# CenterForMedicalGeneticsGhent/WisecondorX

Measured on AMD Instinct MI355X. Metric: newref+predict throughput @15kb bins (bins x refs per second), higher is better.
Workload: dtype f64

## Files before the change

wisecondorx_amd/csrc/api.hip:

```cpp
#include "wcx_common.h"

#include <cstring>
#include <thread>

static thread_local char g_err[1024] = "";

void wcx_set_error(const char *fmt, ...) {
  va_list ap;
  va_start(ap, fmt);
  vsnprintf(g_err, sizeof(g_err), fmt, ap);
  va_end(ap);
}

int wcx_scratch(wcx_ctx *ctx, size_t bytes, void **out) {
  if (bytes > ctx->scratch_bytes) {
    if (ctx->scratch) {
      WCX_HIP(hipStreamSynchronize(ctx->stream));
      WCX_HIP(hipFree(ctx->scratch));
      ctx->scratch = nullptr;
      ctx->scratch_bytes = 0;
    }
    hipError_t e = hipMalloc(&ctx->scratch, bytes);
    if (e != hipSuccess) {
      wcx_set_error("hipMalloc(%zu bytes scratch) failed: %s", bytes, hipGetErrorString(e));
      return WCX_ERR_NOMEM;
    }
    ctx->scratch_bytes = bytes;
  }
  *out = ctx->scratch;
  return WCX_OK;
}

int wcx_host_scratch(wcx_ctx *ctx, size_t bytes, void **out) {
  if (bytes > ctx->host_scratch_bytes) {
    if (ctx->host_scratch) {
      WCX_HIP(hipStreamSynchronize(ctx->stream));
      WCX_HIP(hipHostFree(ctx->host_scratch));
      ctx->host_scratch = nullptr;
      ctx->host_scratch_bytes = 0;
    }
    const size_t grown = bytes + bytes / 4;
    hipError_t e = hipHostMalloc(&ctx->host_scratch, grown, hipHostMallocDefault);
    if (e != hipSuccess) {
      wcx_set_error("hipHostMalloc(%zu bytes) failed: %s", grown, hipGetErrorString(e));
      return WCX_ERR_NOMEM;
    }
    ctx->host_scratch_bytes = grown;
  }
  *out = ctx->host_scratch;
  return WCX_OK;
}

int wcx_scratch2(wcx_ctx *ctx, size_t bytes, void **out) {
  if (bytes > ctx->scratch2_bytes) {
    if (ctx->scratch2) {
      WCX_HIP(hipStreamSynchronize(ctx->stream));
      WCX_HIP(hipFree(ctx->scratch2));
      ctx->scratch2 = nullptr;
      ctx->scratch2_bytes = 0;
    }
    hipError_t e = hipMalloc(&ctx->scratch2, bytes);
    if (e != hipSuccess) {
      wcx_set_error("hipMalloc(%zu bytes scratch2) failed: %s", bytes, hipGetErrorString(e));
      return WCX_ERR_NOMEM;
    }
    ctx->scratch2_bytes = bytes;
  }
  *out = ctx->scratch2;
  return WCX_OK;
}

int wcx_upload_small(wcx_ctx *ctx, void *dst_dev, const void *src_host, size_t bytes) {
  if (ctx->stage.size() > 64) {
    WCX_HIP(hipStreamSynchronize(ctx->stream));
    ctx->stage.clear();
  }
  ctx->stage.emplace_back((const unsigned char *)src_host, (const unsigned char *)src_host + bytes);
  WCX_HIP(hipMemcpyAsync(dst_dev, ctx->stage.back().data(), bytes, hipMemcpyHostToDevice,
                         ctx->stream));
  return WCX_OK;
}

int wcx_timer_begin(wcx_ctx *ctx, const char *name) {
  KernelTimer &t = ctx->timers[ctx->timer_tag + name];
  if (!t.start) {
    WCX_HIP(hipEventCreate(&t.start));
    WCX_HIP(hipEventCreate(&t.stop));
  }
  WCX_HIP(hipEventRecord(t.start, ctx->stream));
  return WCX_OK;
}

int wcx_timer_end(wcx_ctx *ctx, const char *name) {
  KernelTimer &t = ctx->timers[ctx->timer_tag + name];
  WCX_HIP(hipEventRecord(t.stop, ctx->stream));
  t.used = true;
  return WCX_OK;
}

namespace {
constexpr size_t STAGED_MIN = (size_t)32 << 20;
constexpr size_t STAGED_CHUNK = (size_t)32 << 20;
constexpr int COPY_THREADS = 8;

void host_copy_mt(char *dst, const char *src, size_t n) {
  const size_t per = ((n + COPY_THREADS - 1) / COPY_THREADS + 4095) & ~(size_t)4095;
  std::thread th[COPY_THREADS];
  int used = 0;
  for (size_t o = per; o < n; o += per)
    th[used++] = std::thread([=] { memcpy(dst + o, src + o, o + per <= n ? per : n - o); });
  memcpy(dst, src, per <= n ? per : n);
  for (int i = 0; i < used; ++i) th[i].join();
}

int staged_copy(wcx_ctx *ctx, void *dst, const void *src, size_t bytes, bool to_host) {
  void *pin = nullptr;
  int rc = wcx_host_scratch(ctx, 2 * STAGED_CHUNK, &pin);
  if (rc) return rc;
  char *half[2] = {reinterpret_cast<char *>(pin), reinterpret_cast<char *>(pin) + STAGED_CHUNK};
  char *d = reinterpret_cast<char *>(dst);
  const char *s = reinterpret_cast<const char *>(src);
  hipStream_t st = ctx->stream;
  const size_t n_chunks = (bytes + STAGED_CHUNK - 1) / STAGED_CHUNK;
  auto len = [&](size_t i) { return i + 1 < n_chunks ? STAGED_CHUNK : bytes - i * STAGED_CHUNK; };
  if (to_host) {
    WCX_HIP(hipMemcpyAsync(half[0], s, len(0), hipMemcpyDeviceToHost, st));
    WCX_HIP(hipStreamSynchronize(st));
    for (size_t i = 0; i < n_chunks; ++i) {
      if (i + 1 < n_chunks)
        WCX_HIP(hipMemcpyAsync(half[(i + 1) & 1], s + (i + 1) * STAGED_CHUNK, len(i + 1),
                               hipMemcpyDeviceToHost, st));
      host_copy_mt(d + i * STAGED_CHUNK, half[i & 1], len(i));
      WCX_HIP(hipStreamSynchronize(st));
    }
  } else {
    host_copy_mt(half[0], s, len(0));
    for (size_t i = 0; i < n_chunks; ++i) {
      WCX_HIP(hipMemcpyAsync(d + i * STAGED_CHUNK, half[i & 1], len(i), hipMemcpyHostToDevice, st));
      if (i + 1 < n_chunks) host_copy_mt(half[(i + 1) & 1], s + (i + 1) * STAGED_CHUNK, len(i + 1));
      WCX_HIP(hipStreamSynchronize(st));
    }
  }
  return WCX_OK;
}
}

extern "C" {

int wcx_version(void) { return 100; }

int wcx_sweep_event(wcx_ctx *ctx, void **out_event) {
  WCX_ARG(ctx && out_event, "NULL argument");
  WCX_HIP(hipSetDevice(ctx->device));
  if (!ctx->ev_after_sweep) WCX_HIP(hipEventCreateWithFlags(&ctx->ev_after_sweep, hipEventDisableTiming));
  *out_event = ctx->ev_after_sweep;
  return WCX_OK;
}

int wcx_wait_event(wcx_ctx *ctx, void *event) {
  WCX_ARG(ctx && event, "NULL argument");
  WCX_HIP(hipSetDevice(ctx->device));
  WCX_HIP(hipStreamWaitEvent(ctx->stream, reinterpret_cast<hipEvent_t>(event), 0));
  return WCX_OK;
}

int wcx_debug_flags(wcx_ctx *ctx, int flags) {
  if (!ctx) return 0;
  const int old = ctx->debug_flags;
  ctx->debug_flags = flags;
  return old;
}

const char *wcx_last_error(void) { return g_err; }

int wcx_timer_tag(wcx_ctx *ctx, const char *tag) {
  WCX_ARG(ctx, "ctx is NULL");
  ctx->timer_tag = tag ? tag : "";
  return WCX_OK;
}

int wcx_ctx_create(int device, void *stream, wcx_ctx **out) {
  WCX_ARG(out != nullptr, "out is NULL");
  int n = 0;
  hipError_t e = hipGetDeviceCount(&n);
  if (e != hipSuccess || n <= 0) {
    wcx_set_error("no HIP device available (%s); libwcx_hip.so has no CPU fallback",
                  e != hipSuccess ? hipGetErrorString(e) : "device count 0");
    return WCX_ERR_HIP;
  }
  WCX_ARG(device >= 0 && device < n, "device index out of range");
  WCX_HIP(hipSetDevice(device));
  wcx_ctx *ctx = new wcx_ctx();
  ctx->device = device;
  if (stream == WCX_STREAM_DEFAULT) {
    ctx->stream = nullptr;
    ctx->own_stream = false;
  } else if (stream) {
    ctx->stream = reinterpret_cast<hipStream_t>(stream);
    ctx->own_stream = false;
  } else {
    WCX_HIP(hipStreamCreateWithFlags(&ctx->stream, hipStreamNonBlocking));
    ctx->own_stream = true;
  }
  WCX_HIP(hipMalloc(reinterpret_cast<void **>(&ctx->d_stats), 256));
  WCX_HIP(hipMemsetAsync(ctx->d_stats, 0, 256, ctx->stream));
  WCX_HIP(hipMalloc(&ctx->d_small, 8192));
  *out = ctx;
  return WCX_OK;
}

int wcx_ctx_destroy(wcx_ctx *ctx) {
  if (!ctx) return WCX_OK;
  hipSetDevice(ctx->device);
  hipStreamSynchronize(ctx->stream);
  for (auto &kv : ctx->timers) {
    if (kv.second.start) hipEventDestroy(kv.second.start);
    if (kv.second.stop) hipEventDestroy(kv.second.stop);
  }
  wcx_sym_state_free(ctx);
  if (ctx->scratch) hipFree(ctx->scratch);
  if (ctx->host_scratch) hipHostFree(ctx->host_scratch);
  for (auto &sl : ctx->sel_pool)
    if (sl.p) hipFree(sl.p);
  if (ctx->host_scratch2) hipHostFree(ctx->host_scratch2);
  if (ctx->scratch2) hipFree(ctx->scratch2);
  if (ctx->d_stats) hipFree(ctx->d_stats);
  if (ctx->d_small) hipFree(ctx->d_small);
  if (ctx->d_nullm) hipFree(ctx->d_nullm);
  if (ctx->d_nullsrc) hipFree(ctx->d_nullsrc);
  if (ctx->d_pca) hipFree(ctx->d_pca);
  if (ctx->sweep_stream) {
    hipStreamSynchronize(ctx->sweep_stream);
    hipStreamDestroy(ctx->sweep_stream);
    hipEventDestroy(ctx->ev_sweep0);
    hipEventDestroy(ctx->ev_sweep1);
  }
  if (ctx->ev_after_sweep) hipEventDestroy(ctx->ev_after_sweep);
  if (ctx->copy_stream) {
    hipStreamSynchronize(ctx->copy_stream);
    hipStreamDestroy(ctx->copy_stream);
    hipEventDestroy(ctx->ev_cbs_fill);
    hipEventDestroy(ctx->ev_cbs_xw);
  }
  if (ctx->aux_stream) {
    hipStreamSynchronize(ctx->aux_stream);
    hipStreamDestroy(ctx->aux_stream);
    hipEventDestroy(ctx->ev_main);
    hipEventDestroy(ctx->ev_rank);
  }
  if (ctx->d_rank) hipFree(ctx->d_rank);
  if (ctx->own_stream) hipStreamDestroy(ctx->stream);
  delete ctx;
  return WCX_OK;
}

int wcx_sync(wcx_ctx *ctx) {
  WCX_ARG(ctx, "ctx is NULL");
  WCX_HIP(hipStreamSynchronize(ctx->stream));
  return WCX_OK;
}

int wcx_malloc(wcx_ctx *ctx, size_t bytes, void **dptr) {
  WCX_ARG(ctx && dptr, "NULL argument");
  WCX_HIP(hipSetDevice(ctx->device));
  hipError_t e = hipMalloc(dptr, bytes ? bytes : 1);
  if (e != hipSuccess) {
    wcx_set_error("hipMalloc(%zu) failed: %s", bytes, hipGetErrorString(e));
    return WCX_ERR_NOMEM;
  }
  return WCX_OK;
}

int wcx_free(wcx_ctx *ctx, void *dptr) {
  WCX_ARG(ctx, "ctx is NULL");
  if (dptr) {
    WCX_HIP(hipStreamSynchronize(ctx->stream));
    WCX_HIP(hipFree(dptr));
  }
  return WCX_OK;
}

int wcx_memcpy_h2d(wcx_ctx *ctx, void *dst, const void *src, size_t bytes) {
  WCX_ARG(ctx && dst && src, "NULL argument");
  WCX_HIP(hipSetDevice(ctx->device));
  if (bytes >= STAGED_MIN) return staged_copy(ctx, dst, src, bytes, false);
  WCX_HIP(hipMemcpyAsync(dst, src, bytes, hipMemcpyHostToDevice, ctx->stream));
  WCX_HIP(hipStreamSynchronize(ctx->stream));
  return WCX_OK;
}

int wcx_memcpy_d2h(wcx_ctx *ctx, void *dst, const void *src, size_t bytes) {
  WCX_ARG(ctx && dst && src, "NULL argument");
  WCX_HIP(hipSetDevice(ctx->device));
  if (bytes >= STAGED_MIN) return staged_copy(ctx, dst, src, bytes, true);
  WCX_HIP(hipMemcpyAsync(dst, src, bytes, hipMemcpyDeviceToHost, ctx->stream));
  WCX_HIP(hipStreamSynchronize(ctx->stream));
  return WCX_OK;
}

double wcx_last_kernel_ms(wcx_ctx *ctx, const char *name) {
  if (!ctx || !name) return -1.0;
  auto it = ctx->timers.find(name);
  if (it == ctx->timers.end() || !it->second.used) return -1.0;
  if (hipEventSynchronize(it->second.stop) != hipSuccess) return -1.0;
  float ms = 0.f;
  if (hipEventElapsedTime(&ms, it->second.start, it->second.stop) != hipSuccess) return -1.0;
  return (double)ms;
}

int wcx_transpose_dev(wcx_ctx *ctx, const double *d_src, int64_t rows, int64_t cols,
                      double *d_dst) {
  WCX_ARG(ctx && d_src && d_dst, "NULL argument");
  WCX_ARG(rows > 0 && cols > 0 && rows < (1ll << 31) && (rows + 31) / 32 < 65536, "bad sizes");
  WCX_HIP(hipSetDevice(ctx->device));
  return wcx_transpose_launch(ctx, d_src, rows, cols, d_dst);
}

int wcx_last_topk_stats(wcx_ctx *ctx, int64_t out[24]) {
  WCX_ARG(ctx && out, "NULL argument");
  unsigned long long h[24] = {0};
  WCX_HIP(hipMemcpyAsync(h, ctx->d_stats, 24 * 8, hipMemcpyDeviceToHost, ctx->stream));
  WCX_HIP(hipStreamSynchronize(ctx->stream));
  out[0] = ctx->topk_stats[0];
  out[1] = ctx->topk_stats[1];
  out[2] = (int64_t)h[2];
  out[3] = (int64_t)h[3];
  for (int i = 4; i < 24; ++i) out[i] = (int64_t)h[i];
  return WCX_OK;
}

int wcx_newref_sym_sweep_dev(wcx_ctx *ctx, const double *dXs, int64_t B, int S, const int64_t *chr_cum,
                             int n_chr, int k, int part, int n_parts, const int64_t *row_bounds,
                             int64_t *counts_out) {
  WCX_ARG(ctx && dXs && chr_cum && row_bounds && counts_out, "NULL argument");
  WCX_ARG(B > 0 && S > 0 && n_chr > 0 && k > 0, "B, S, n_chr, k must be positive");
  WCX_ARG(chr_cum[n_chr - 1] == B, "chr_cum[n_chr-1] must equal B");
  WCX_ARG(n_parts >= 1 && part >= 0 && part < n_parts, "bad part");
  WCX_ARG(B < (int64_t)0x7fffffff, "B must fit in int32 (indices are int32)");
  if (n_chr > 22) {
    wcx_set_error("the sharded symmetric sweep searches every row: not a gonosomal pass (n_chr = %d)", n_chr);
    return WCX_ERR_UNSUPPORTED;
  }
  WCX_HIP(hipSetDevice(ctx->device));
  if (ctx->rank_X && !ctx->rank_pending) ctx->rank_X = nullptr;
  const int64_t r0 = row_bounds[part], r1 = row_bounds[part + 1];
  WCX_ARG(0 <= r0 && r0 <= r1 && r1 <= B, "bad row bounds");
  int64_t pairs = 0;
  for (int c = 0; c < n_chr; ++c) {
    const int64_t cs = c ? chr_cum[c - 1] : 0, ce = chr_cum[c];
    const int64_t lo = cs > r0 ? cs : r0, hi = ce < r1 ? ce : r1;
    if (lo < hi) pairs += (hi - lo) * (B - (ce - cs));
  }
  ctx->topk_stats[0] = r1 - r0;
  ctx->topk_stats[1] = pairs;
  wcx_aux_cancel_if_few_rows(ctx, B, r1 - r0);
  return wcx_sym_shard_sweep(ctx, dXs, B, S, chr_cum, n_chr, k, part, n_parts, row_bounds, counts_out);
}

int wcx_newref_sym_records_dev(wcx_ctx *ctx, void *d_send) {
// ... 103 lines not shown
```

wisecondorx_amd/csrc/cbs_seg.hip:

```cpp
#include <algorithm>
#include <chrono>
#include <cmath>
#include <cstdio>
#include <functional>
#include <map>
#include <mutex>
#include <thread>
#include <vector>

#include "wave_sort.h"
#include "wcx_common.h"

namespace {

constexpr int NTP = 1024;
constexpr int KMAXC = 25;
constexpr int QC_W = 32;
constexpr int PCHUNK = 256;
constexpr int NCH = 64;
constexpr int STAGE_A = 512;
typedef float f32x2 __attribute__((ext_vector_type(2)));

__host__ __device__ __forceinline__ unsigned long long mix64(unsigned long long z) {
  z += 0x9e3779b97f4a7c15ull;
// ... 1213 lines not shown
    std::vector<int> hc(nsc + 1);
    WCX_HIP(hipMemcpyAsync(hc.data(), d_cnt, (nsc + 1) * 4, hipMemcpyDeviceToHost, st));
    WCX_HIP(hipStreamSynchronize(st));
    for (size_t q = 0; q < nsc; ++q) cnt_sc[q] = hc[q];
    n_inf = hc[nsc];
  } else {
    for_samples([&](int s) {
      for (int c = 0; c < n_chr; ++c) {
        const double *rr = r + (int64_t)s * n_bins + chr_off[c];
        const int nall = (int)(chr_off[c + 1] - chr_off[c]);
        int64_t m = 0;
        for (int i = 0; i < nall; ++i) m += is_drop(rr[i]) ? 0 : 1;
        cnt_sc[(size_t)s * n_chr + c] = m;
      }
    });
  }
  int64_t total = 0;
  std::vector<int64_t> lo_sc(cnt_sc.size());
  for (size_t q = 0; q < cnt_sc.size(); ++q) { lo_sc[q] = total; total += cnt_sc[q]; }
  const int64_t totp = (total + 3) & ~(int64_t)3;
  void *hstage = nullptr;
  {
    const int rcs = wcx_host_scratch(ctx, (size_t)totp * 20 + 64, &hstage);
    if (rcs) return rcs;
  }
  double *hx = reinterpret_cast<double *>(hstage), *hw = hx + totp;
  int *hpos = reinterpret_cast<int *>(hw + totp);
  if (d_r && (ctx->debug_flags & 64)) {
    const double poison = __builtin_nan("");
    for (int64_t i = 0; i < 2 * totp; ++i) hx[i] = poison;
  }
  if (!d_r)
    for_samples([&](int s) {
      for (int c = 0; c < n_chr; ++c) {
        const int64_t o = (int64_t)s * n_bins + chr_off[c];
        const int nall = (int)(chr_off[c + 1] - chr_off[c]);
        int64_t at = lo_sc[(size_t)s * n_chr + c];
        for (int i = 0; i < nall; ++i) {
          const double v = r[o + i];
          if (is_drop(v)) continue;
          hx[at] = v;
          hw[at] = w[o + i] == 0.0 ? 1.0 : w[o + i];
          hpos[at] = i + 1;
          ++at;
        }
      }
    });
  for (int s = 0; s < n_samples; ++s)
    for (int c = 0; c < n_chr; ++c) {
      const size_t q = (size_t)s * n_chr + c;
      if (cnt_sc[q] == 0) continue;
      Series se;
      se.sample = s; se.chr = c; se.lo = lo_sc[q]; se.n = (int)cnt_sc[q];
      se.seg_end = {0, se.n};
      series.push_back(std::move(se));
    }
  const int64_t N = total;
  const double *dXs_all = nullptr, *dWs_all = nullptr;
  lap("series");
  int rc = wcx_timer_begin(ctx, "cbs");
  if (rc) return rc;
  if (N > 0) {
    int max_n = 0;
    for (const Series &se : series) max_n = std::max(max_n, se.n);
    const int max_segs = (int)series.size() + 8;
    const int max_jobs = max_segs * 2;
    const int npad_max = (max_n + NTP - 1) / NTP * NTP;
    const bool any_big = max_n > LDS_KEYS_MAX;
    const size_t max_items = (size_t)max_segs + (size_t)(N / 4) + 6144 + 64;
    const size_t max_blocks = (size_t)(N / PBS) + 2 * (size_t)max_segs + 64;
    const unsigned int work_cap = 1u << 22;
    const size_t qtab_floats = (size_t)(KMAXC - 1) * ((size_t)N + (size_t)NTP * max_segs) +
                               (size_t)max_segs * (KMAXC + 1) * QC_W;
    const size_t need = (size_t)N * (8 * 5 + 4 * 3) + 4096 + (series.size() + 8) * sizeof(RangeItem) + (size_t)max_segs * (sizeof(SegIn) + sizeof(SegOut) + 8) +
                        (size_t)max_segs * P.ngrid * 16 + max_items * (sizeof(ArcItem) + sizeof(ArcBest)) +
                        (size_t)max_jobs * (2 * sizeof(PermJob) + (size_t)(nw + NCH) * 4) +
                        (any_big ? (size_t)BIG_GRID * (npad_max + 64) * 4 : 0) +
                        (size_t)EXACT_GRID * npad_max * 8 + FLAG_CAP * sizeof(uint2) + qtab_floats * 4 +
                        max_blocks * (sizeof(BlkStat) + 4) + (size_t)work_cap * (sizeof(WorkItem) + sizeof(ArcBest)) +
                        (size_t)max_segs * 32 + (1 << 16);
    void *scr = nullptr;
    rc = wcx_scratch(ctx, need, &scr);
    if (rc) return rc;
    Arena A;
    A.base = reinterpret_cast<char *>(scr);
    double *dX = A.take<double>(N), *dW = A.take<double>(N), *dS = A.take<double>(N), *dWp = A.take<double>(N);
    double *dYd = A.take<double>(N);
    dXs_all = dX; dWs_all = dW;
    int *dpos = A.take<int>((size_t)N + 4);
    RangeItem *drng = A.take<RangeItem>(series.size() + 8);
    float *dy = A.take<float>(N), *drw = A.take<float>(N);
    SegIn *dseg = A.take<SegIn>(max_segs);
    SegOut *dso = A.take<SegOut>(max_segs);
    int *dfirst = A.take<int>(max_segs + 1);
    double *dtx = A.take<double>((size_t)max_segs * P.ngrid), *dnu = A.take<double>((size_t)max_segs * P.ngrid);
    ArcItem *ditems = A.take<ArcItem>(max_items);
    ArcBest *dbest = A.take<ArcBest>(max_items);
    PermJob *djobs = A.take<PermJob>((size_t)max_jobs * 2);
    unsigned int *dbits = A.take<unsigned int>((size_t)max_jobs * nw);
    unsigned int *dcnt = A.take<unsigned int>((size_t)max_jobs * NCH + 64);
    unsigned int *dnflag = dcnt + (size_t)max_jobs * NCH;
    float *dbig = any_big ? A.take<float>((size_t)BIG_GRID * (npad_max + 64)) : nullptr;
    double *dexact = A.take<double>((size_t)EXACT_GRID * npad_max);
    uint2 *dflags = A.take<uint2>(FLAG_CAP);
    float *dq = A.take<float>(qtab_floats);
    BlkStat *dbs = A.take<BlkStat>(max_blocks);
    WorkItem *dwork = A.take<WorkItem>(work_cap);
    ArcBest *dres = A.take<ArcBest>(work_cap);
    int *dboff = A.take<int>(max_segs + 1);
    int *dbseg = A.take<int>(max_blocks);
    unsigned int *dL = A.take<unsigned int>(max_segs + 2);
    unsigned long long *dbbits = A.take<unsigned long long>(max_segs);
    unsigned long long *dbij = A.take<unsigned long long>(max_segs);
    static const bool no_prune = getenv("WCX_CBS_NOPRUNE") && atoi(getenv("WCX_CBS_NOPRUNE"));
    if (d_r) {
      WCX_HIP(hipMemcpyAsync(d_lo, lo_sc.data(), lo_sc.size() * 8, hipMemcpyHostToDevice, st));
      k_cbs_fill<<<dim3((unsigned)n_chr, (unsigned)n_samples), 256, 0, st>>>(d_r, d_w, n_bins, co, n_chr, d_lo,
                                                                            dX, dW, dpos);
      WCX_HIP(hipGetLastError());
      WCX_HIP(hipEventRecord(ctx->ev_cbs_fill, st));
      WCX_HIP(hipStreamWaitEvent(aux, ctx->ev_cbs_fill, 0));
      k_cbs_export<<<16, 256, 0, aux>>>(reinterpret_cast<const uint4 *>(dpos), reinterpret_cast<uint4 *>(hpos),
                                        ((int64_t)N * 4 + 15) / 16);
      WCX_HIP(hipGetLastError());
      if (n_inf > 0) {
        const size_t rw_bytes = (size_t)n_samples * n_bins * 8;
        WCX_HIP(hipMemcpyAsync(const_cast<double *>(r), d_r, rw_bytes, hipMemcpyDeviceToHost, aux));
        WCX_HIP(hipMemcpyAsync(const_cast<double *>(w), d_w, rw_bytes, hipMemcpyDeviceToHost, aux));
      }
      copies_queued = true;
    } else {
      WCX_HIP(hipMemcpyAsync(dX, hx, (size_t)N * 8, hipMemcpyHostToDevice, st));
      WCX_HIP(hipMemcpyAsync(dW, hw, (size_t)N * 8, hipMemcpyHostToDevice, st));
    }
    const size_t lds_small = (size_t)(std::min(npad_max, LDS_KEYS_MAX) + 32) * 4;
    WCX_HIP(hipFuncSetAttribute(reinterpret_cast<const void *>(k_cbs_perm_hyb<false>),
                                hipFuncAttributeMaxDynamicSharedMemorySize, (int)lds_small));

    std::vector<JobResult> jres;
    std::vector<unsigned int> hbits;
    auto run_jobs = [&](std::vector<PermJob> &jobs, const std::vector<std::vector<int>> &seq) -> int {
      jres.assign(jobs.size(), JobResult());
      if (jobs.empty()) return WCX_OK;
      WCX_ARG(jobs.size() <= (size_t)max_jobs, "internal: permutation job table overflow");
      size_t qoff = 0;
      for (size_t q = 0; q < jobs.size(); ++q) {
        jobs[q].slot = (int)q;
        jobs[q].qoff = (int64_t)qoff;
        if (jobs[q].mode == 0)
          qoff += (size_t)(KMAXC - 1) * (size_t)((jobs[q].n + NTP - 1) / NTP * NTP) + (size_t)(KMAXC + 1) * QC_W;
      }
      WCX_ARG(qoff <= qtab_floats, "internal: arc-weight table overflow");
      WCX_HIP(hipMemcpyAsync(djobs, jobs.data(), jobs.size() * sizeof(PermJob), hipMemcpyHostToDevice, st));
      WCX_HIP(hipMemsetAsync(dbits, 0, jobs.size() * (size_t)nw * 4, st));
      WCX_HIP(hipMemsetAsync(dcnt, 0, jobs.size() * (size_t)NCH * 4, st));
      {
        int hyb_max_n = 0;
        for (const PermJob &jb : jobs) if (jb.mode == 0) hyb_max_n = std::max(hyb_max_n, jb.n);
        if (hyb_max_n > 0) {
          const int npad_sel = (hyb_max_n + NTP - 1) / NTP * NTP;
          k_cbs_arcweights<<<dim3((unsigned)(npad_sel / 256), (unsigned)jobs.size()), 256, 0, st>>>(
              dWp, djobs, P.minw, dq);
          WCX_HIP(hipGetLastError());
        }
      }
      hbits.resize(jobs.size() * (size_t)nw);
      std::vector<int> pending(jobs.size());
      for (size_t q = 0; q < jobs.size(); ++q) pending[q] = (int)q;
      const int stages[3] = {0, std::min(STAGE_A, P.nperm), P.nperm};
      for (int sg = 0; sg < 2 && !pending.empty(); ++sg) {
        const int p0 = stages[sg], p1 = stages[sg + 1];
        if (p1 <= p0) continue;
        std::vector<PermJob> sel[4];
        for (int q : pending) {
          const PermJob &jb = jobs[(size_t)q];
          const int kind = jb.mode == 0 ? (jb.n > LDS_KEYS_MAX ? 1 : 0) : jb.mode == 1 ? 2 : 3;
          sel[kind].push_back(jb);
        }
        size_t joff = 0;
        PermJob *dsel = djobs + jobs.size();
        WCX_ARG(pending.size() + jobs.size() <= (size_t)max_jobs * 2, "internal: job table overflow");
        for (int kind = 0; kind < 4; ++kind) {
          std::vector<PermJob> &sj = sel[kind];
          if (sj.empty()) continue;
          const size_t per_launch = kind <= 1 ? std::max<size_t>(1, FLAG_CAP / (size_t)(p1 - p0)) : sj.size();
          for (size_t j0 = 0; j0 < sj.size(); j0 += per_launch) {
            const size_t nj = std::min(per_launch, sj.size() - j0);
            PermJob *dj = dsel + joff;
            WCX_HIP(hipMemcpyAsync(dj, sj.data() + j0, nj * sizeof(PermJob), hipMemcpyHostToDevice, st));
            joff += nj;
            if (kind <= 1) {
              WCX_HIP(hipMemsetAsync(dnflag, 0, 4, st));
              if (kind == 1)
                k_cbs_perm_hyb<true><<<dim3((unsigned)std::min(BIG_GRID, p1 - p0), (unsigned)nj), NTP, 0, st>>>(
                    dy, drw, dj, p0, p1, npad_max + 64, dq, dbig, dbits, dcnt, nw, dflags, dnflag);
              else
                k_cbs_perm_hyb<false><<<dim3((unsigned)(p1 - p0), (unsigned)nj), NTP, lds_small, st>>>(
                    dy, drw, dj, p0, p1, 0, dq, nullptr, dbits, dcnt, nw, dflags, dnflag);
              WCX_HIP(hipGetLastError());
              k_cbs_perm_exact<<<EXACT_GRID, 256, 0, st>>>(dYd, dW, dWp, dj, dflags, dnflag, dexact, npad_max,
                                                           P.minw, dbits, dcnt, nw);
            } else if (kind == 2) {
              k_cbs_perm_full<<<dim3((unsigned)(p1 - p0), (unsigned)nj), 256, 0, st>>>(dYd, dW, dWp, dj, p0, p1,
                                                                                      P.minw, dbits, dcnt, nw);
            } else {
              k_cbs_perm_edge<<<dim3((unsigned)((p1 - p0 + 3) / 4), (unsigned)nj), 256, 0, st>>>(
                  dYd, dW, dj, p0, p1, dbits, dcnt, nw);
            }
            WCX_HIP(hipGetLastError());
          }
        }
        WCX_HIP(hipMemcpyAsync(hbits.data(), dbits, jobs.size() * (size_t)nw * 4, hipMemcpyDeviceToHost, st));
        WCX_HIP(hipStreamSynchronize(st));
        std::vector<int> still;
        for (int q : pending) {
          const PermJob &jb = jobs[(size_t)q];
          const unsigned int *b = hbits.data() + (size_t)q * nw;
          JobResult &res = jres[(size_t)q];
          if (jb.mode == 2) {
            int nrej = 0;
            for (int t = 0; t < nw; ++t) nrej += __builtin_popcount(b[t]);
            res.nrej = nrej; res.np = p1;
            if (nrej > jb.budget) { res.decided = 1; res.significant = 0; }
            else if (p1 >= P.nperm) { res.decided = 1; res.significant = 1; }
          } else {
            eval_sequential(b, p1, P.nperm, jb.budget, seq[(size_t)q], res);
          }
          if (!res.decided) still.push_back(q);
        }
        pending.swap(still);
      }
      return WCX_OK;
    };

    std::vector<char> resident(series.size(), d_r ? 0 : 1);
    auto ensure_resident = [&](const std::vector<int> &want) -> int {
      std::vector<RangeItem> items;
      for (int q : want)
        if (!resident[(size_t)q]) {
          resident[(size_t)q] = 1;
          items.push_back({series[(size_t)q].lo, series[(size_t)q].n, 0});
        }
      if (items.empty()) return WCX_OK;
      WCX_HIP(hipMemcpyAsync(drng, items.data(), items.size() * sizeof(RangeItem), hipMemcpyHostToDevice, st));
      k_cbs_export_ranges<<<(unsigned)items.size(), 256, 0, st>>>(dX, dW, drng, hx, hw);
      WCX_HIP(hipGetLastError());
      WCX_HIP(hipStreamSynchronize(st));
      return WCX_OK;
    };

    struct Active { int series, lo, hi; };
    for (;;) {
      std::vector<Active> act;
      for (size_t q = 0; q < series.size(); ++q) {
        Series &se = series[q];
        while (se.seg_end.size() > 1) {
          const int k = (int)se.seg_end.size();
          const int lo = se.seg_end[k - 2], hi = se.seg_end[k - 1];
          if (hi - lo >= 2 * P.minw) { act.push_back({(int)q, lo, hi}); break; }
          se.change_loc.push_back(hi);
          se.seg_end.pop_back();
        }
      }
      if (act.empty()) break;
      const int ns = (int)act.size();
      std::vector<SegIn> hseg(ns);
      double arc_total = 0;
      for (int a = 0; a < ns; ++a) { const double n = act[a].hi - act[a].lo; arc_total += 0.5 * n * n; }
      const double arc_budget = std::max(arc_total / 6144.0, 16384.0);
      std::vector<ArcItem> items;
      std::vector<int> first(ns + 1);
      for (int a = 0; a < ns; ++a) {
        const Series &se = series[act[a].series];
        hseg[a].lo = se.lo + act[a].lo;
        hseg[a].n = act[a].hi - act[a].lo;
        hseg[a].hybrid = hseg[a].n > P.nmin ? 1 : 0;
        first[a] = (int)items.size();
        const int n = hseg[a].n;
        for (int i0 = 0; i0 < n;) {
          const int rows = (int)std::min<double>(ARC_ROWS, std::max<double>(4.0, arc_budget / (double)(n - i0)));
          items.push_back({a, i0, std::min(i0 + rows, n), 0});
          i0 += rows;
        }
      }
      first[ns] = (int)items.size();
      WCX_ARG(items.size() <= max_items, "internal: arc stripe table overflow");
      WCX_HIP(hipMemcpyAsync(dseg, hseg.data(), (size_t)ns * sizeof(SegIn), hipMemcpyHostToDevice, st));
      WCX_HIP(hipMemcpyAsync(ditems, items.data(), items.size() * sizeof(ArcItem), hipMemcpyHostToDevice, st));
      WCX_HIP(hipMemcpyAsync(dfirst, first.data(), (size_t)(ns + 1) * 4, hipMemcpyHostToDevice, st));
      k_cbs_prepare<<<ns, NTP, 0, st>>>(dX, dW, dseg, dS, dWp, dYd, dy, drw, dso);
      std::vector<int> boff(ns + 1);
      boff[0] = 0;
      for (int a = 0; a < ns; ++a) boff[a + 1] = boff[a] + (hseg[a].n + 1 + PBS - 1) / PBS;
      const int total_blocks = boff[ns];
      bool pruned = !no_prune && (size_t)total_blocks <= max_blocks && arc_total > 4e9;
      unsigned int *dcount = dL + ns;
      if (pruned) {
        WCX_HIP(hipMemcpyAsync(dboff, boff.data(), (size_t)(ns + 1) * 4, hipMemcpyHostToDevice, st));
        WCX_HIP(hipMemsetAsync(dL, 0, (size_t)(ns + 1) * 4, st));
        WCX_HIP(hipMemsetAsync(dbbits, 0, (size_t)ns * 8, st));
        WCX_HIP(hipMemsetAsync(dbij, 0xff, (size_t)ns * 8, st));
        std::vector<int> bseg((size_t)total_blocks);
        for (int a = 0; a < ns; ++a) std::fill(bseg.begin() + boff[a], bseg.begin() + boff[a + 1], a);
        WCX_HIP(hipMemcpyAsync(dbseg, bseg.data(), (size_t)total_blocks * 4, hipMemcpyHostToDevice, st));
        const unsigned rows4 = (unsigned)((total_blocks + 3) / 4);
        k_cbs_blockstats<<<rows4, 256, 0, st>>>(dS, dWp, dseg, dso, dboff, dbseg, total_blocks, dbs);
        k_cbs_coarse<<<rows4, 256, 0, st>>>(dS, dWp, dseg, dso, dboff, dbseg, total_blocks, dbs, P.minw, dL);
        k_cbs_prune<<<(unsigned)((total_blocks + 4 * PRW - 1) / (4 * PRW)), 256, 0, st>>>(
            dso, dboff, dbseg, total_blocks, dbs, dL, dwork, work_cap, dcount);
        k_cbs_pairmax<<<8192, 256, 0, st>>>(dS, dWp, dseg, dso, dwork, work_cap, dcount, P.minw, dres, dbbits, dL);
        k_cbs_pairtie<<<2048, 256, 0, st>>>(dwork, work_cap, dcount, dres, dbbits, dbij);
        k_cbs_pairfinal<<<(unsigned)((ns + 256) / 256), 256, 0, st>>>(ns, dbbits, dbij, dbest, dfirst);
        WCX_HIP(hipGetLastError());
        unsigned int hcount = 0;
        WCX_HIP(hipMemcpyAsync(&hcount, dcount, 4, hipMemcpyDeviceToHost, st));
        WCX_HIP(hipStreamSynchronize(st));
        ctx->cbs_pairs_listed += hcount;
        ctx->cbs_pairs_total += [&] { long long t = 0; for (int a = 0; a < ns; ++a) { const long long nb = boff[a + 1] - boff[a]; t += nb * (nb + 1) / 2; } return t; }();
        if (hcount > work_cap) pruned = false;
      }
      if (!pruned) {
        WCX_HIP(hipMemcpyAsync(dfirst, first.data(), (size_t)(ns + 1) * 4, hipMemcpyHostToDevice, st));
        k_cbs_arcmax<<<(unsigned)items.size(), 256, 0, st>>>(dS, dWp, dseg, dso, ditems, P.minw, dbest);
      }
      const double alpha_skip = (ctx->debug_flags & 2) ? HUGE_VAL : 4.0 * P.alpha;
      k_cbs_arcfinish<<<ns, 128, 0, st>>>(dbest, dfirst, dseg, dWp, dso, P.kmax, P.ngrid, alpha_skip, dtx);
      k_nu_series<<<dim3(P.ngrid, ns), 256, 0, st>>>(dtx, dseg, dso, P.ngrid, alpha_skip, dnu);
      k_cbs_tailp<<<ns, 64, 0, st>>>(dnu, dseg, dso, P.ngrid, alpha_skip);
      WCX_HIP(hipGetLastError());
      std::vector<SegOut> hso(ns);
      WCX_HIP(hipMemcpyAsync(hso.data(), dso, (size_t)ns * sizeof(SegOut), hipMemcpyDeviceToHost, st));
      WCX_HIP(hipStreamSynchronize(st));
      lap("  stats");
      if (d_r) {
        std::vector<int> want;
        for (int a = 0; a < ns; ++a) {
          const SegOut &o = hso[a];
          if (!hseg[a].hybrid || !o.valid || o.range <= 1.4901161193847656e-08) continue;
          const double ostat1 = sqrt(o.ostat);
          const int arc = std::min(o.bj - o.bi, hseg[a].n - o.bj + o.bi);
          if (ostat1 <= 0.1 || (!strict && ostat1 >= 7.0 && arc >= 10)) continue;
          if (o.pval1 < 0.0 || o.pval1 > P.alpha) continue;
          want.push_back(act[a].series);
        }
        rc = ensure_resident(want);
        if (rc) return rc;
      }
      lap("  host copy");

      std::vector<PermJob> jobs;
      std::vector<std::vector<int>> seq;
      std::vector<int> job_of(ns, -1);
      std::vector<int> verdict(ns, 0);
      std::vector<int> why(ns, 0);
      int n_shortcut = 0;
      for (int a = 0; a < ns; ++a) {
        const SegOut &o = hso[a];
        const int n = hseg[a].n;
        if (!o.valid || o.range <= 1.4901161193847656e-08) { why[a] = 1; continue; }
        const double ostat1 = sqrt(o.ostat);
        if (ostat1 <= 0.1) { why[a] = 2; continue; }
        const int arc = std::min(o.bj - o.bi, n - o.bj + o.bi);
        if (!strict && ostat1 >= 7.0 && arc >= 10) { why[a] = 3; verdict[a] = 1; continue; }
        double pval2 = P.alpha;
        if (hseg[a].hybrid) {
          if (o.pval1 < 0.0 || o.pval1 > P.alpha) { why[a] = 4; continue; }
          pval2 = P.alpha - o.pval1;
        }
        PermJob jb;
        memset(&jb, 0, sizeof(jb));
        jb.lo = hseg[a].lo; jb.n = n; jb.mode = hseg[a].hybrid ? 0 : 1;
        jb.budget = (int)(pval2 * (double)P.nperm);
        jb.thr = 0.99999 * o.ostat;
        jb.tss = o.tss;
        jb.W = o.W;
        if (jb.mode == 0 && !(ctx->debug_flags & 32) &&
            short_arc_bound(hx + jb.lo, hw + jb.lo, jb.n, P.minw, P.kmax, o.tss) * 1.0001 < jb.thr) {
          why[a] = 6; verdict[a] = 1; ++n_shortcut;
          continue;
        }
        if (jb.mode == 0) {
          const double u = 5.9604644775390625e-08;
          const double vmax = sqrt(o.wmax) * o.ymax;
          const double wlo = P.minw * o.wmin;
          const double qmax = o.W / (wlo * (o.W - wlo));
          jb.cthr = jb.thr / ((n - 2.0) + jb.thr);
          jb.D = u * vmax * (2700.0 + 75.0 * n * o.wmax / o.W) * sqrt(qmax) * 1.001;
          jb.eT = 6.0 * u * n * vmax / o.W * 1.001;
          const double bthr = jb.cthr * o.tss;
          if (!(wlo > 0) || !(o.W > 2 * wlo) || !(bthr > 1e-30) || !(bthr < 1e30) || !std::isfinite(jb.D))
            jb.D = HUGE_VAL;
        }
        const Series &se = series[act[a].series];
        jb.key = test_key(P.seed, se.chr, act[a].lo, act[a].hi, 0);
        why[a] = 5;
        job_of[a] = (int)jobs.size();
        seq.push_back(cbs_boundary(P.alpha, P.nperm, jb.budget));
        jobs.push_back(jb);
      }
      rc = run_jobs(jobs, seq);
      if (rc) return rc;
      lap("  perms");
      std::vector<JobResult> seg_res(ns);
      for (int a = 0; a < ns; ++a)
        if (job_of[a] >= 0) { seg_res[a] = jres[(size_t)job_of[a]]; verdict[a] = seg_res[a].significant; }
      ctx->cbs_shortcuts += n_shortcut;

      std::vector<PermJob> ejobs;
      struct EdgeRef { int a, which, shortcut; };
      std::vector<EdgeRef> eref;
      if (d_r) {
        std::vector<int> want;
        for (int a = 0; a < ns; ++a)
          if (verdict[a] && hso[a].bi != 0 && hso[a].bj != hseg[a].n) want.push_back(act[a].series);
        rc = ensure_resident(want);
        if (rc) return rc;
      }
      for (int a = 0; a < ns; ++a) {
        if (!verdict[a]) continue;
        const int n = hseg[a].n, bi = hso[a].bi, bj = hso[a].bj;
        if (bi == 0 || bj == n) continue;
        const double mean = hso[a].mean;
        const double *x = hx + hseg[a].lo, *ww = hw + hseg[a].lo;
        for (int which = 0; which < 2; ++which) {
          const int l = which == 0 ? 0 : bi, n12 = which == 0 ? bj : n - bi;
          const int n1 = which == 0 ? bi : bj - bi, n2 = n12 - n1;
          EdgeRef er{a, which, -1};
          if (n1 == 1 || n2 == 1) { er.shortcut = 0; eref.push_back(er); continue; }
          double w1 = 0, w2 = 0, s1 = 0, s2 = 0, ssq = 0;
          for (int i = 0; i < n1; ++i) { const double c = x[l + i] - mean; w1 += ww[l + i]; s1 += ww[l + i] * c; ssq += ww[l + i] * c * c; }
          for (int i = n1; i < n12; ++i) { const double c = x[l + i] - mean; w2 += ww[l + i]; s2 += ww[l + i] * c; ssq += ww[l + i] * c * c; }
          const double rn = w1 + w2;
          const double xbar = (s1 + s2) / rn;
          const double tss = ssq - rn * xbar * xbar;
          const bool first_short = n1 <= n2;
          const int m1 = first_short ? n1 : n2;
          const double wm = first_short ? w1 : w2, wo = first_short ? w2 : w1;
          const double dm = fabs((first_short ? s1 / w1 : s2 / w2) - xbar);
          double tstat = dm * dm * wm * rn / wo;
          tstat = tstat / ((tss - tstat) / (n12 - 2.0));
          if (!strict && tstat > 25.0 && m1 >= 10) { er.shortcut = 1; eref.push_back(er); continue; }
          PermJob jb;
          memset(&jb, 0, sizeof(jb));
          jb.lo = hseg[a].lo + l; jb.n = n12; jb.mode = 2; jb.m1 = m1;
          int budget = (int)floor(P.alpha * P.nperm);
          while ((double)(budget + 1) / (double)P.nperm <= P.alpha) ++budget;
          while (budget >= 0 && (double)budget / (double)P.nperm > P.alpha) --budget;
          jb.budget = budget;
          jb.thr = 0.99999 * dm;
          jb.tss = xbar;
          jb.W = wm;
          const Series &se = series[act[a].series];
          jb.key = test_key(P.seed, se.chr, act[a].lo, act[a].hi, 1 + which);
          er.shortcut = -1 - (int)ejobs.size();
// ... 226 lines not shown
```

wisecondorx_amd/csrc/newref_topk_screen.hip:

```cpp
#include <cmath>
#include <cstdlib>

#include "screen_kernel.h"
#include "screen_common.h"
#include "screen_hub1.h"

namespace {

constexpr int CSPLIT = 16;

__device__ __forceinline__ unsigned long long dord(double x) {
  const unsigned long long u = (unsigned long long)__double_as_longlong(x);
  return (u >> 63) ? ~u : (u | 0x8000000000000000ull);
}
__device__ __forceinline__ double dord_inv(unsigned long long k) {
  return __longlong_as_double((long long)((k >> 63) ? (k & 0x7fffffffffffffffull) : ~k));
}

__global__ __launch_bounds__(NT) void k_col_sum(const double *__restrict__ Xs, int64_t B,
                                                double *__restrict__ psum,
                                                double *__restrict__ pcnt,
                                                unsigned long long *__restrict__ cmin,
                                                unsigned long long *__restrict__ cmax) {
  __shared__ double ws[NT / 64], wc[NT / 64];
// ... 925 lines not shown
  const int forced = kn.cut_r(0);
  if (forced > 0 && forced < k) r = forced;
  return r;
}

static std::vector<ScreenBlock> merge_blocks(const std::vector<TopkBlock> &exact_blocks, const int64_t *chr_cum,
                                             int n_chr, int max_rows) {
  std::vector<ScreenBlock> out;
  size_t i = 0;
  while (i < exact_blocks.size()) {
    ScreenBlock sb;
    sb.row0 = exact_blocks[i].row0;
    sb.nrows = exact_blocks[i].nrows;
    sb.chr = 0;
    for (int c = 0; c < n_chr; ++c)
      if (chr_cum[c] == exact_blocks[i].ce && (c ? chr_cum[c - 1] : 0) == exact_blocks[i].cs) sb.chr = c;
    sb.cs = exact_blocks[i].cs;
    sb.ce = exact_blocks[i].ce;
    size_t j = i + 1;
    while (j < exact_blocks.size() && exact_blocks[j].cs == sb.cs &&
           exact_blocks[j].row0 == sb.row0 + sb.nrows && sb.nrows + exact_blocks[j].nrows <= max_rows) {
      sb.nrows += exact_blocks[j].nrows;
      ++j;
    }
    out.push_back(sb);
    i = j;
  }
  return out;
}

enum class ScreenPath { sym, exact, one_dir };
struct ScreenPlan {
  ScreenCfg cfg;
  int hw_cus = 256, slots = 0;
  int hub_need = 0;
  int64_t hub_rows = 0;
  bool hub_ok = false;
  ScreenPath path = ScreenPath::one_dir;
  std::vector<ScreenBlock> blocks;
  std::vector<ScreenBlock> hub_blocks;
  bool use_hub1 = false;
  int SF = 0, n_seg = 1, cut_r = 0;
};
static ScreenPlan plan_shape(wcx_ctx *ctx, int64_t B, int k, const ScreenCfg &cfg, const Knobs &kn) {
  ScreenPlan p;
  p.cfg = cfg;
  hipDeviceProp_t prop;
  if (hipGetDeviceProperties(&prop, ctx->device) == hipSuccess && prop.multiProcessorCount > 0)
    p.hw_cus = prop.multiProcessorCount;
  p.slots = p.hw_cus * (cfg.lb * 4 / cfg.wpb > 0 ? cfg.lb * 4 / cfg.wpb : 1);
  const int need = (int)(1.18 * k) + 8;
  p.hub_need = kn.hub_test_fail(0) ? (1 << 28) : need;
  const int frac = kn.hub_frac(cfg.nk >= 16 ? 32 : 12);
  p.hub_rows = frac > 1 ? B / frac : 0;
  if (p.hub_rows < 8 * (int64_t)need + 512) p.hub_rows = 8 * (int64_t)need + 512;
  p.hub_ok = cfg.nk >= 5 && frac > 1 && p.hub_rows * 6 <= B;
  return p;
}

static ScreenPlan plan_search(wcx_ctx *ctx, int64_t B, int S, int k, bool all_rows, const Knobs &kn,
                              const std::vector<TopkBlock> &exact_blocks, const int64_t *chr_cum, int n_chr) {
  const int NK = screen_nk(S);
  ScreenCfg cfg = default_cfg(NK);
  cfg.prof = (ctx->debug_flags & DBG_PROF) && (NK == 7 || NK == 32) ? 1 : 0;
  int tl[5];
  if (kn.tile.set && sscanf(kn.tile.str, "%d,%d,%d,%d,%d", &tl[0], &tl[1], &tl[2], &tl[3], &tl[4]) == 5) {
    cfg.ctg = tl[0]; cfg.tt = tl[1]; cfg.wpb = tl[2]; cfg.lb = tl[3]; cfg.ring = tl[4];
  }
  ScreenPlan p = plan_shape(ctx, B, k, cfg, kn);
  const int TGT_WG = 32 * cfg.tt * cfg.wpb;
  p.blocks = merge_blocks(exact_blocks, chr_cum, n_chr, TGT_WG);
  int SF = kn.sample((B >= 32768) ? 16 : ((B >= 8192 && NK < 16) ? 8 : 0));
  if (SF < 2 || SF > 64) SF = 0;
  const int64_t n_s = SF ? (B + SF - 1) / SF : 0;
  const int64_t P_s = (n_s + CT - 1) / CT * CT;
  const bool hub1 = kn.screen_hub(kn.sample.set || kn.cut_r.set ? 0 : 1) != 0 && p.hub_ok && cfg.wpb == 4 &&
                    cfg.ring >= 2;
  int n_seg = 1;
  if ((int)p.blocks.size() * (hub1 ? 2 : 4) <= p.slots) {
    int fill = p.slots / (int)p.blocks.size();
    if (fill > 8) fill = 8;
    n_seg = kn.segments_small(fill);
  }
  n_seg = kn.segments(n_seg);
  if (n_seg < 1) n_seg = 1;
  if (n_seg > 8) n_seg = 8;
  p.n_seg = n_seg;
  int64_t covered = 0;
  for (const ScreenBlock &sb : p.blocks) covered += sb.nrows;
  const int cut_r1 = sample_rank(k, SF, P_s, 1, kn);
  const int sym_mode = kn.sym(1);
  if (cut_r1 && all_rows && covered == B && cfg.tt == 1 && cfg.wpb == 4 && cfg.ring >= 2 &&
      (sym_mode == 2 || (sym_mode == 1 && NK >= 16))) {
    p.path = ScreenPath::sym;
    p.SF = SF;
    p.cut_r = cut_r1;
    return p;
  }
  if (k > KMAX_ONE_DIR) {
    p.path = ScreenPath::exact;
    return p;
  }
  p.use_hub1 = hub1;
  if (hub1) {
    if (TGT_WG != 128) p.hub_blocks = merge_blocks(exact_blocks, chr_cum, n_chr, 128);
  } else {
    p.SF = SF;
    p.cut_r = sample_rank(k, SF, P_s, n_seg, kn);
  }
  return p;
}

template <class Unit, size_t N, class... Args>
static int launch_unit(Unit (&units)[N], const Args &...args) {
  int rc = -1;
  for (Unit u : units)
    if ((rc = u(args...)) >= 0) break;
  return rc;
}
static const decltype(&wcx_screen_launch_k1) screen_units[] = {
    wcx_screen_launch_k1, wcx_screen_launch_k2, wcx_screen_launch_k3, wcx_screen_launch_k4,
    wcx_screen_launch_k5, wcx_screen_launch_k6, wcx_screen_launch_k7, wcx_screen_launch_k8};
static const decltype(&wcx_sym_launch_k1) sym_units[] = {wcx_sym_launch_k1, wcx_sym_launch_k2, wcx_sym_launch_k3,
                                                         wcx_sym_launch_k4, wcx_sym_launch_k5};
static const decltype(&wcx_count_launch_k1) count_units[] = {wcx_count_launch_k1, wcx_count_launch_k2,
                                                             wcx_count_launch_k3, wcx_count_launch_k4};
static const decltype(&wcx_hub1_launch_k1) hub1_units[] = {wcx_hub1_launch_k1, wcx_hub1_launch_k2,
                                                           wcx_hub1_launch_k3, wcx_hub1_launch_k4};

static int unit_status(int e, const char *family, const ScreenCfg &c, int trials = 0) {
  if (e == 0) return WCX_OK;
  char what[128];
  const int n = snprintf(what, sizeof what, "nk=%d ctg=%d tt=%d wpb=%d lb=%d ring=%d", c.nk, c.ctg, c.tt, c.wpb,
                         c.lb, c.ring);
  if (trials) snprintf(what + n, sizeof what - n, " trials=%d", trials);
  if (e < 0) {
    wcx_set_error("%s kernel %s is not instantiated", family, what);
    return (int)WCX_ERR_UNSUPPORTED;
  }
  wcx_set_error("%s kernel %s: launch failed: %s", family, what, hipGetErrorString((hipError_t)e));
  return (int)WCX_ERR_HIP;
}

struct Carve {
  uintptr_t at;
  template <class T> void operator()(T *&p, size_t bytes) {
    p = reinterpret_cast<T *>(at);
    at += (bytes + 255) / 256 * 256;
  }
};

static float screen_gamma(int NK) { return (float)(16 * NK + 12) * 1.1920929e-7f; }

static int col_stats(const double *dXs, int64_t B, int S, double *cmean, ScreenGlobals *glob,
                     const int64_t *chr_cum, int n_chr, ChrTab &tab, hipStream_t st) {
  unsigned long long *cmin = reinterpret_cast<unsigned long long *>(cmean + S);
  unsigned long long *cmax = cmin + S;
  double *psum = cmean + 3 * S, *pcnt = psum + (size_t)S * CSPLIT;
  WCX_HIP(hipMemsetAsync(cmin, 0xff, (size_t)S * 8, st));
  WCX_HIP(hipMemsetAsync(cmax, 0, (size_t)S * 8, st));
  k_col_sum<<<dim3((unsigned)S, CSPLIT), NT, 0, st>>>(dXs, B, psum, pcnt, cmin, cmax);
  k_col_stats<<<(unsigned)((S + 63) / 64), 64, 0, st>>>(S, psum, pcnt, cmin, cmax, cmean, glob);
  tab.n_chr = n_chr;
  for (int c = 0; c < 32; ++c) tab.cum[c] = c < n_chr ? chr_cum[c] : B;
  return WCX_OK;
}

static void screen_prep(int NK, const double *Xr, int64_t n_pos, int S, int Sp, const double *cmean,
                        const int *perm, ScreenGlobals *glob, half8 *F, RowInfo *info, const unsigned int *gate,
                        hipStream_t st) {
  const unsigned g = (unsigned)((n_pos + 31) / 32);
  switch (NK) {
#define WCX_PREP_CASE(N) case N: k_screen_prep<N><<<g, NT, 0, st>>>(Xr, n_pos, S, Sp, cmean, perm, glob, F, info, gate); break;
    WCX_PREP_CASE(1) WCX_PREP_CASE(2) WCX_PREP_CASE(3) WCX_PREP_CASE(4) WCX_PREP_CASE(5)
    WCX_PREP_CASE(6) WCX_PREP_CASE(7) WCX_PREP_CASE(8) WCX_PREP_CASE(10) WCX_PREP_CASE(12)
    WCX_PREP_CASE(14) WCX_PREP_CASE(16) WCX_PREP_CASE(20) WCX_PREP_CASE(24) WCX_PREP_CASE(28)
    WCX_PREP_CASE(40) WCX_PREP_CASE(48) WCX_PREP_CASE(56) WCX_PREP_CASE(64)
    default: k_screen_prep<32><<<g, NT, 0, st>>>(Xr, n_pos, S, Sp, cmean, perm, glob, F, info, gate); break;
#undef WCX_PREP_CASE
  }
}

struct ScreenChunk { int64_t groups; size_t lds; };
static ScreenChunk screen_chunk(const ScreenCfg &cfg, int kb) {
  int64_t g = ((int64_t)kb << 10) / ((int64_t)cfg.ctg * 32 * cfg.nk * 32);
  if (g < 16) g = 16;
  if (g > 4096) g = 4096;
  return {g, (size_t)(cfg.ring >= 2 ? cfg.ring : 2) * (size_t)(cfg.ctg * cfg.nk * 64) * 16 + (size_t)(g + 64) * 4};
}

static int sym_final(int NK, int cap2, const RowInfo *info, const ScreenGlobals *glob, const int *rowpos, int64_t n,
                     uint2 *sl, int *cnt, unsigned int *flags, const float *Dest, int k, const unsigned int *gate,
                     hipStream_t st) {
  const float gamma = screen_gamma(NK);
  const unsigned gf = (unsigned)((n + 3) / 4 < 65536 ? (n + 3) / 4 : 65536);
  if (cap2 == CAP2)
    k_sym_final<CAP2 / 64><<<gf, NT, 0, st>>>(info, glob, rowpos, n, sl, cnt, flags, Dest, k, gamma, CAP, gate);
  else
    k_sym_final<CAP2_BIG / 64><<<gf, NT, 0, st>>>(info, glob, rowpos, n, sl, cnt, flags, Dest, k, gamma,
                                                  REFINE_MAX, gate);
  WCX_HIP(hipGetLastError());
  return WCX_OK;
}

static bool kick_after_sweep(int S) { return S >= 256; }
static int end_prep(wcx_ctx *ctx, int S) {
  WCX_HIP(hipGetLastError());
  int rc = wcx_timer_end(ctx, "topk_prep");
  if (rc) return rc;
  if (!kick_after_sweep(S) && (rc = wcx_aux_kick(ctx))) return rc;
  return wcx_timer_begin(ctx, "topk_screen");
}

struct TopkTail {
  const double *dXs = nullptr;
  int64_t B = 0;
  int S = 0, Sp = 0, k = 0;
  int cap2 = CAP;
  ChrTab tab;
  double *Xr = nullptr;
  ScreenGlobals *glob = nullptr;
  int *perm = nullptr, *cnt = nullptr;
  unsigned int *flags = nullptr, *d_nredo = nullptr;
  unsigned char *searched = nullptr;
  uint2 *sl = nullptr;
  TopkBlock *d_redo = nullptr, *d_rtile = nullptr;
  int32_t *d_rlist = nullptr;
  void *rscr = nullptr;
};
static int finish_topk(wcx_ctx *ctx, const TopkTail &t, int64_t r0, int64_t n, bool kick, int32_t *d_out_idx,
                       double *d_out_dist) {
  hipStream_t st = ctx->stream;
  if (ctx->ev_after_sweep) WCX_HIP(hipEventRecord(ctx->ev_after_sweep, st));
  int rc = kick ? wcx_aux_kick(ctx) : (int)WCX_OK;
  if (rc) return rc;
  rc = wcx_timer_begin(ctx, "topk_refine");
  if (rc) return rc;
  rc = wcx_refine_launch(ctx, t.Xr, t.S, t.Sp, t.tab, r0, n, t.searched, t.sl, t.cnt, t.flags, t.perm, t.k,
                         d_out_idx, d_out_dist, t.glob, t.cap2);
  if (rc) return rc;
  rc = wcx_timer_end(ctx, "topk_refine");
  if (rc) return rc;
  const unsigned g = (unsigned)((n + NT - 1) / NT);
  k_collect_redo<<<g, NT, 0, st>>>(r0, n, t.searched, t.flags, t.tab, t.d_redo, t.d_nredo, ctx->d_stats);
  k_redo_plan<<<1, 64, 0, st>>>(t.tab, t.d_nredo, t.d_rtile);
  k_redo_fill<<<g, NT, 0, st>>>(r0, n, t.searched, t.flags, t.tab, t.d_nredo, t.d_rlist);
  WCX_HIP(hipGetLastError());
  rc = wcx_topk_exact_redo_launch(ctx, t.dXs, t.B, t.S, t.d_redo, t.d_nredo, t.d_rtile, t.d_nredo + 1, t.d_rlist,
                                  t.rscr, r0, t.k, d_out_idx, d_out_dist);
  if (rc) return rc;
  return wcx_timer_end(ctx, "topk");
}

struct SymShardState {
  bool valid = false;
  int64_t row_begin = 0, row_end = 0;
  int NK = 0, n_parts = 0, part = 0;
  RowBounds rb;
  TopkTail tail;
  RowInfo *info = nullptr;
  int *rowpos = nullptr;
  float *Dest = nullptr;
  unsigned int *pool_head = nullptr;
  uint4 *pool = nullptr;
  unsigned int pool_cap = 0;
  unsigned long long *d_counts = nullptr;
  unsigned long long counts[32] = {0};
  bool overflow = false;
};
struct SymShardCall { int part, n_parts; RowBounds rb; SymShardState *state; };

static int screen_sym_path(wcx_ctx *ctx, const Knobs &kn, const ScreenPlan &p, const double *dXs, int64_t B, int S,
                           const int64_t *chr_cum, int n_chr, int k, int32_t *d_out_idx, double *d_out_dist,
                           SymShardCall *sh = nullptr) {
  const ScreenCfg &cfg = p.cfg;
  const std::vector<ScreenBlock> &blocks = p.blocks;
  const int NK = cfg.nk, CTG = cfg.ctg, SF = p.SF;
  const int Sp = row_pitch(S);
  const int64_t n_rows = B;
  const int64_t n_own = sh ? sh->rb.b[sh->part + 1] - sh->rb.b[sh->part] : B;
  const int cap2 = k <= 448 ? CAP2 : CAP2_BIG;
  const bool use_hub = kn.sym_hub(1) != 0 && p.hub_ok;
  if (sh && !use_hub) {
    wcx_set_error("the row-sharded symmetric sweep needs the hub-count thresholds (K >= 256, B >= %lld)",
                  (long long)(36 * (int64_t)p.hub_need));
    return (int)WCX_ERR_UNSUPPORTED;
  }
  const int64_t n_s = (B + SF - 1) / SF;
  const int64_t P_s = (n_s + CT - 1) / CT * CT;
  const int64_t Bpad2 = P_s + ((B - n_s) + CT - 1) / CT * CT;
  const int64_t NTb = (((B + 31) / 32 + (int64_t)2 * SYM_NCLS * n_chr + 4) + 7) / 8 * 8;
  const int64_t PB = NTb * 32;
  const int64_t pool_want = sh ? n_rows * (int64_t)(cap2 / 2) / sh->n_parts * 2 : n_rows * (int64_t)(cap2 / 2);
  const unsigned int pool_cap = (unsigned int)(pool_want < 200000000ll ? pool_want : 200000000ll);
  const int n_wg_det = (int)((B + NT - 1) / NT);
  TopkTail t;
  ScreenGlobals *glob;
  double *cmean;
  half8 *F, *Fs;
  RowInfo *info, *infs;
  int *perm2, *rowpos, *rowpos2, *hubhist, *rchr, *rkey, *cellcnt, *cursor, *d_seq, *dett;
  unsigned int *rbits, *rfine, *gmask, *tinfo, *pool_head;
  float *tmin, *Dest, *g_state;
  unsigned char *tchr;
  unsigned short *detl;
  uint4 *pool;
  SymDesc *d_desc;
  unsigned long long *d_counts;
  ScreenBlock *d_blocks;
  auto layout = [&](uintptr_t base) {
    Carve take{base};
    take(glob, sizeof(ScreenGlobals));
    take(cmean, (size_t)S * 8 * (3 + 2 * CSPLIT));
    take(t.Xr, (size_t)B * Sp * 8 + 256);
    take(F, (size_t)PB * NK * 32);
    take(Fs, (size_t)P_s * NK * 32);
    take(info, (size_t)PB * sizeof(RowInfo));
    take(infs, (size_t)P_s * sizeof(RowInfo));
    take(t.perm, (size_t)PB * 4);
    take(perm2, (size_t)Bpad2 * 4);
    take(rowpos, (size_t)B * 4);
    take(rowpos2, (size_t)B * 4);
    take(rbits, (size_t)B * 4);
    take(rfine, (size_t)B * 4);
    take(hubhist, (size_t)HUB_BINS * 4);
    take(rchr, (size_t)B * 4);
    take(rkey, (size_t)B * 4);
    take(cellcnt, (size_t)2 * NCELL * 4);
    take(cursor, (size_t)2 * NCELL * 4);
    take(gmask, (size_t)(P_s / CT) * 4);
    take(tinfo, (size_t)NTb * 64 * 4);
    take(tmin, (size_t)NTb * 4);
    take(tchr, (size_t)NTb);
    take(Dest, (size_t)n_rows * 4);
    take(pool, (size_t)pool_cap * 16);
    take(pool_head, 256);
    take(d_desc, 256 * sizeof(SymDesc));
    take(d_seq, (size_t)(NTb / 4 + 1) * 4);
    take(t.sl, (size_t)n_own * cap2 * 8);
    take(dett, sh ? (size_t)DET_KEYS * n_wg_det * 4 : 0);
    take(detl, sh ? (size_t)B * 2 : 0);
    take(d_counts, 64 * 8);
    take(t.cnt, (size_t)n_rows * 4);
    take(g_state, (size_t)n_rows * 4);
    take(t.flags, (size_t)n_rows * 4);
    take(t.searched, (size_t)n_rows);
    take(d_blocks, blocks.size() * sizeof(ScreenBlock));
    take(t.d_redo, (size_t)n_rows * sizeof(TopkBlock));
    take(t.d_nredo, 512);
    take(t.d_rtile, ((size_t)n_rows / 64 + 64) * sizeof(TopkBlock));
    take(t.d_rlist, (size_t)n_rows * 4);
    take(t.rscr, wcx_topk_redo_scratch_bytes(k, B));
    return (size_t)(take.at - base);
  };
  void *scr = nullptr;
  int rc = wcx_scratch(ctx, layout(0), &scr);
  if (rc) return rc;
  layout(reinterpret_cast<uintptr_t>(scr));
  t.dXs = dXs; t.B = B; t.S = S; t.Sp = Sp; t.k = k; t.cap2 = cap2; t.glob = glob;
  unsigned int *d_gate = pool_head + 3, *d_failed = pool_head + 4;
  const unsigned int *gate2 = use_hub ? d_gate : nullptr;

  hipStream_t st = ctx->stream;
  WCX_HIP(hipMemsetAsync(glob, 0, sizeof(ScreenGlobals), st));
  WCX_HIP(hipMemsetAsync(t.cnt, 0, (size_t)n_rows * 4, st));
  WCX_HIP(hipMemsetAsync(t.flags, 0, (size_t)n_rows * 4, st));
  WCX_HIP(hipMemsetAsync(t.searched, 1, (size_t)n_rows, st));
  WCX_HIP(hipMemsetAsync(pool_head, 0, 256, st));
  WCX_HIP(hipMemsetAsync(t.d_nredo, 0, 512, st));
  WCX_HIP(hipMemsetAsync(ctx->d_stats, 0, 256, st));
  rc = wcx_upload_small(ctx, d_blocks, blocks.data(), blocks.size() * sizeof(ScreenBlock));
  if (rc) return rc;

  rc = wcx_timer_begin(ctx, "topk");
  if (rc) return rc;
  rc = wcx_timer_begin(ctx, "topk_prep");
  if (rc) return rc;
  rc = col_stats(dXs, B, S, cmean, glob, chr_cum, n_chr, t.tab, st);
  if (rc) return rc;
  const ChrTab &tab = t.tab;
  const unsigned gb = (unsigned)((B + NT - 1) / NT);
  if (use_hub) {
    WCX_HIP(hipMemsetAsync(hubhist, 0, (size_t)HUB_BINS * 4, st));
    k_transpose_norm<<<(unsigned)((B + 31) / 32), 256, 0, st>>>(dXs, B, S, Sp, t.Xr, cmean, tab, glob, rbits, rchr,
                                                                rfine, hubhist);
    k_hub_cut<<<1, 1024, 0, st>>>(hubhist, (int)p.hub_rows, glob);
  } else {
    k_transpose_norm<<<(unsigned)((B + 31) / 32), 256, 0, st>>>(dXs, B, S, Sp, t.Xr, cmean, tab, glob, rbits, rchr,
                                                                nullptr, nullptr);
  }
  WCX_HIP(hipMemsetAsync(cellcnt, 0, (size_t)2 * NCELL * 4, st));
  WCX_HIP(hipMemsetAsync(cursor, 0, (size_t)2 * NCELL * 4, st));
  WCX_HIP(hipMemsetAsync(t.perm, 0xff, (size_t)PB * 4, st));
  WCX_HIP(hipMemsetAsync(tchr, 0xff, (size_t)NTb, st));
  static_assert(2 * SYM_NCELL * SYM_NSUB <= 2 * NCELL, "cell tables");
  k_sym_hist<<<gb, NT, 0, st>>>(rbits, rchr, B, glob, rkey, cellcnt, 1, use_hub ? rfine : nullptr);
  k_sym_scan<<<1, SYM_NCELL, 0, st>>>(cellcnt, cursor, tchr, glob);
  if (sh) {
    WCX_HIP(hipMemsetAsync(dett, 0, (size_t)DET_KEYS * n_wg_det * 4, st));
    k_det_local<<<gb, NT, 0, st>>>(rkey, B, n_wg_det, dett, detl);
    k_det_scan<<<(unsigned)((DET_KEYS * 64 + NT - 1) / NT), NT, 0, st>>>(dett, n_wg_det, cursor);
    k_det_place<<<gb, NT, 0, st>>>(rkey, B, n_wg_det, dett, detl, t.perm, rowpos);
  } else {
    k_scatter<<<gb, NT, 0, st>>>(rkey, B, cursor, t.perm, rowpos);
  }
  screen_prep(NK, t.Xr, PB, S, Sp, cmean, t.perm, glob, F, info, nullptr, st);
  rc = end_prep(ctx, S);
  if (rc) return rc;

  int64_t Cz = ((int64_t)kn.sym_chunk_kb(3072) << 10) / ((int64_t)NK * 1024);
  Cz = Cz / 8 * 8;
  if (Cz < 32) Cz = 32;
  if (Cz > 8192) Cz = 8192;
  while ((NTb + Cz - 1) / Cz > 256) Cz *= 2;
  const int glist_cap = (int)((Cz / CTG + 64 + 3) / 4 * 4);
  const size_t lds_sym = (size_t)cfg.ring * (size_t)(CTG * NK * 64) * 16 + (size_t)cfg.ring * CTG * 256 +
                         (size_t)glist_cap * 4 + (size_t)4 * 64 * 16;
  const int NQb = (int)(NTb / 4);
  SymArgs sa;
  int sym_grid = 0;
  {
    const int fill = kn.sym_fill(1) * p.slots;
    std::vector<SymDesc> descs;
    int total = 0;
    for (int64_t c0 = 0; c0 < NTb; c0 += Cz) {
      SymDesc d;
      d.c0 = (int)c0;
      d.c1 = (int)(c0 + Cz < NTb ? c0 + Cz : NTb);
      d.q_first = (int)(c0 / 4);
      d.n_q = NQb - d.q_first;
      int n_split = d.n_q >= fill ? 1 : (fill + d.n_q - 1) / d.n_q;
      const int max_split = (d.c1 - d.c0) / CTG / 8 > 1 ? (d.c1 - d.c0) / CTG / 8 : 1;
      if (n_split > max_split) n_split = max_split;
      const int split = kn.sym_split(0);
      if (split > 0) n_split = split < max_split ? split : max_split;
      if (n_split < 1) n_split = 1;
      if (!descs.empty() && n_split < descs.back().n_split) n_split = descs.back().n_split;
      d.n_split = n_split;
      d.item_base = total;
      d.index = (int)descs.size();
      d.pad = 0;
      total += d.n_q * d.n_split;
      descs.push_back(d);
    }
    rc = wcx_upload_small(ctx, d_desc, descs.data(), descs.size() * sizeof(SymDesc));
    if (rc) return rc;
    WCX_HIP(hipMemsetAsync(d_seq, 0, (size_t)(NQb + 1) * 4, st));
    sa.F = F; sa.tinfo = tinfo; sa.tmin = tmin; sa.tchr = tchr; sa.glob = glob; sa.sl = t.sl; sa.cnt = t.cnt;
    sa.flags = t.flags; sa.stats = ctx->d_stats; sa.dbg = ctx->debug_flags; sa.cap2 = cap2;
    sa.pool = pool; sa.pool_head = pool_head; sa.pool_ovf = pool_head + 1; sa.pool_cap = pool_cap;
    sa.queue_head = pool_head + 2;
    sa.desc = d_desc; sa.n_desc = (int)descs.size(); sa.total_items = total; sa.seq = d_seq;
    sa.glist_cap = glist_cap;
    sa.gate = nullptr;
    if (sh) { sa.force_records = 1; sa.part = sh->part; sa.n_parts = sh->n_parts; }
    sym_grid = total < p.slots ? total : p.slots;
  }
  auto sweep = [&]() {
    return unit_status(launch_unit(sym_units, NK, CTG, cfg.lb, cfg.ring, sa, (unsigned)sym_grid, lds_sym, st),
                       "symmetric screen", cfg);
  };
  auto sweep_and_cut = [&](const unsigned int *gate) -> int {
    sa.gate = gate;
    const int e = sweep();
    if (e) return e;
    k_sym_regroup<<<2048, NT, 0, st>>>(pool, pool_head, pool_head + 1, pool_cap, n_rows, t.sl, t.cnt, t.flags,
                                       cap2, gate);
    return sym_final(NK, cap2, info, glob, rowpos, n_rows, t.sl, t.cnt, t.flags, Dest, k, gate, st);
  };

  if (use_hub) {
    rc = wcx_timer_begin(ctx, "topk_pre");
    if (rc) return rc;
    CountArgs ca;
    ca.F = F; ca.tchr = tchr; ca.glob = glob; ca.perm = t.perm; ca.tinfo = tinfo; ca.tmin = tmin;
    ca.Dest = Dest; ca.cnt = t.cnt; ca.flags = t.flags; ca.stats = ctx->d_stats;
    ca.need = p.hub_need; ca.n1 = kn.hub_n1(16); ca.gate = nullptr;
    ca.sl = nullptr; ca.cap2 = cap2;
    const int64_t hub_t = (p.hub_rows * 2 + 31) / 32 + (int64_t)SYM_NCLS * n_chr + 8;
    const int64_t cap_t = hub_t < NTb ? hub_t : NTb;
    ca.glist_cap = (int)(cap_t / CTG + 64);
    const size_t lds_cnt = (size_t)cfg.ring * (size_t)(CTG * NK * 64) * 16 + (size_t)ca.glist_cap * 4;
    rc = unit_status(launch_unit(count_units, NK, CTG, cfg.lb, cfg.ring, ca, (unsigned)NQb, lds_cnt, st),
                     "hub-count", cfg);
    if (rc) return rc;
    rc = wcx_timer_end(ctx, "topk_pre");
    if (rc) return rc;
    if (sh) {
      rc = sweep();
      if (rc) return rc;
      WCX_HIP(hipMemsetAsync(d_counts, 0, 64 * 8, st));
      k_rec_hist<<<1024, NT, 0, st>>>(pool, pool_head, pool_cap, sh->rb, d_counts);
      WCX_HIP(hipGetLastError());
      rc = wcx_timer_end(ctx, "topk_screen");
      if (rc) return rc;
      SymShardState &Z = *sh->state;
      unsigned int head2[2] = {0, 0};
      WCX_HIP(hipMemcpyAsync(Z.counts, d_counts, 32 * 8, hipMemcpyDeviceToHost, st));
      WCX_HIP(hipMemcpyAsync(head2, pool_head, 8, hipMemcpyDeviceToHost, st));
      WCX_HIP(hipStreamSynchronize(st));
      Z.overflow = head2[1] || head2[0] > pool_cap || kn.pool_ovf(0) != 0;
      if (Z.overflow)
        for (int r = 0; r < 32; ++r) Z.counts[r] = 0;
      Z.valid = true;
      Z.row_begin = sh->rb.b[sh->part]; Z.row_end = sh->rb.b[sh->part + 1];
      Z.NK = NK; Z.n_parts = sh->n_parts; Z.part = sh->part; Z.rb = sh->rb;
      Z.tail = t; Z.info = info; Z.rowpos = rowpos; Z.Dest = Dest;
      Z.pool_head = pool_head; Z.pool = pool; Z.pool_cap = pool_cap; Z.d_counts = d_counts;
      return (int)WCX_OK;
    }
    rc = sweep_and_cut(nullptr);
    if (rc) return rc;
    if (!(ctx->debug_flags & DBG_ABLATIONS)) {
      k_hub_count_failed<<<512, NT, 0, st>>>(t.flags, n_rows, d_failed);
      k_hub_verdict<<<1, 64, 0, st>>>(d_failed, d_gate, ctx->d_stats);
    }
    k_gate_reset<<<1024, NT, 0, st>>>(d_gate, n_rows, t.cnt, t.flags, pool_head, d_seq, NQb + 1);
  } else {
    rc = wcx_timer_begin(ctx, "topk_pre");
    if (rc) return rc;
  }

  {
    WCX_HIP(hipMemsetAsync(cellcnt, 0, (size_t)2 * NCELL * 4, st));
    WCX_HIP(hipMemsetAsync(perm2, 0xff, (size_t)Bpad2 * 4, st));
    k_row_hist<<<gb, NT, 0, st>>>(rbits, rchr, B, SF, 0, glob, rkey, cellcnt, gate2);
    k_scan_cells<<<1, 1024, 0, st>>>(cellcnt, cursor, (int)(P_s - n_s), gate2);
    k_scatter<<<gb, NT, 0, st>>>(rkey, B, cursor, perm2, rowpos2, gate2);
    k_group_mask<<<(unsigned)((P_s / CT + NT - 1) / NT), NT, 0, st>>>(perm2, rchr, P_s / CT, gmask, gate2);
    screen_prep(NK, t.Xr, P_s, S, Sp, cmean, perm2, glob, Fs, infs, gate2, st);
    WCX_HIP(hipGetLastError());
    const ScreenChunk ch = screen_chunk(cfg, kn.chunk_kb(NK > 16 ? 16384 : 3072));
    ScreenArgs a;
    a.F = Fs; a.Ft = F; a.info = info; a.glob = glob; a.perm = perm2; a.rowpos = rowpos; a.gmask = gmask;
    a.blocks = d_blocks; a.sl = t.sl; a.cnt = t.cnt; a.flags = t.flags; a.g_state = g_state;
    a.stats = ctx->d_stats; a.row_begin = 0; a.n_rows_all = n_rows;
    a.k = k; a.dbg = ctx->debug_flags & ~DBG_SWEEP; a.n_seg = 1; a.n_blocks = (int)blocks.size();
    a.raw_est = 1;
    a.gate = gate2;
    int trig_a = 4 * p.cut_r + 64;
    if (trig_a > 256 && 2 * p.cut_r + 32 <= 256) trig_a = 256;
    if (trig_a > LIM) trig_a = LIM;
    const int64_t g_end = P_s / (CTG * 32);
    bool first = true;
    for (int64_t g0 = 0; g0 < g_end; g0 += ch.groups) {
      const int64_t g1 = g0 + ch.groups < g_end ? g0 + ch.groups : g_end;
      a.g_start = g0; a.g_count = (int)(g1 - g0);
      a.cut_k = p.cut_r; a.cut_mode = 1; a.trig = trig_a; a.end_cut = g1 == g_end ? 1 : 0;
      a.first = first ? 1 : 0;
      first = false;
      rc = unit_status(launch_unit(screen_units, cfg, a, (unsigned)blocks.size(), ch.lds, st), "screen", cfg);
      if (rc) return rc;
    }
    k_sym_setup<<<(unsigned)((PB + NT - 1) / NT), NT, 0, st>>>(t.perm, info, glob, g_state, t.cnt, t.flags, Dest,
                                                              tinfo, tmin, gate2);
    WCX_HIP(hipGetLastError());
    if (!use_hub) {
      rc = wcx_timer_end(ctx, "topk_pre");
      if (rc) return rc;
    }
    rc = sweep_and_cut(gate2);
    if (rc) return rc;
  }
  rc = wcx_timer_end(ctx, "topk_screen");
  if (rc) return rc;
  return finish_topk(ctx, t, 0, n_rows, kick_after_sweep(S), d_out_idx, d_out_dist);
}

static int screen_one_dir_path(wcx_ctx *ctx, const Knobs &kn, const ScreenPlan &p, const double *dXs, int64_t B,
                               int S, const int64_t *chr_cum, int n_chr, int64_t row_begin, int64_t n_rows, int k,
                               int32_t *d_out_idx, double *d_out_dist) {
  const ScreenCfg &cfg = p.cfg;
  const std::vector<ScreenBlock> &blocks = p.blocks, &hub_blocks = p.hub_blocks;
  const int NK = cfg.nk, GRr = cfg.ctg * 32, SF = p.SF, n_seg = p.n_seg, cut_r = p.cut_r;
  const bool use_hub1 = p.use_hub1;
  const int64_t n_s = SF ? (B + SF - 1) / SF : 0;
  const int64_t P_s = (n_s + CT - 1) / CT * CT;
  const int64_t Bpad = P_s + ((B - n_s) + CT - 1) / CT * CT + (use_hub1 ? CT : 0);
  const int64_t n_iter_groups = Bpad / GRr;
  const int64_t n_groups = Bpad / CT;
  const int Sp = row_pitch(S);
  TopkTail t;
  ScreenGlobals *glob;
  double *cmean;
  half8 *F;
  RowInfo *info;
  int *rowpos, *hubhist, *rchr, *rkey, *cellcnt, *cursor;
  unsigned int *rbits, *rfine, *gmask;
  float *g_state;
  ScreenBlock *d_blocks, *d_hblocks;
  auto layout = [&](uintptr_t base) {
    Carve take{base};
    take(glob, sizeof(ScreenGlobals));
    take(cmean, (size_t)S * 8 * (3 + 2 * CSPLIT));
    take(t.Xr, (size_t)B * Sp * 8 + 256);
    take(F, (size_t)Bpad * NK * 32);
    take(info, (size_t)Bpad * sizeof(RowInfo));
    take(t.perm, (size_t)Bpad * 4);
    take(rowpos, (size_t)B * 4);
    take(rbits, (size_t)B * 4);
    take(rfine, use_hub1 ? (size_t)B * 4 : 0);
    take(hubhist, use_hub1 ? (size_t)HUB_BINS * 4 : 0);
    take(rchr, (size_t)B * 4);
    take(rkey, (size_t)B * 4);
    take(cellcnt, (size_t)2 * NCELL * 4);
    take(cursor, (size_t)2 * NCELL * 4);
    take(gmask, (size_t)n_groups * 4);
    take(t.sl, (size_t)n_seg * n_rows * CAP * 8);
    take(t.cnt, (size_t)n_seg * n_rows * 4);
    take(g_state, (size_t)n_seg * n_rows * 4);
    take(t.flags, (size_t)n_seg * n_rows * 4);
    take(t.searched, (size_t)n_rows);
    take(d_blocks, blocks.size() * sizeof(ScreenBlock));
    take(d_hblocks, hub_blocks.size() * sizeof(ScreenBlock));
    take(t.d_redo, (size_t)n_rows * sizeof(TopkBlock));
    take(t.d_nredo, 512);
    take(t.d_rtile, ((size_t)n_rows / 64 + 64) * sizeof(TopkBlock));
    take(t.d_rlist, (size_t)n_rows * 4);
    take(t.rscr, wcx_topk_redo_scratch_bytes(k, B));
    return (size_t)(take.at - base);
  };
  void *scr = nullptr;
  int rc = wcx_scratch(ctx, layout(0), &scr);
  if (rc) return rc;
  layout(reinterpret_cast<uintptr_t>(scr));
  t.dXs = dXs; t.B = B; t.S = S; t.Sp = Sp; t.k = k; t.cap2 = CAP; t.glob = glob;
  hipStream_t st = ctx->stream;
  WCX_HIP(hipMemsetAsync(glob, 0, sizeof(ScreenGlobals), st));
  WCX_HIP(hipMemsetAsync(t.cnt, 0, (size_t)n_seg * n_rows * 4, st));
  WCX_HIP(hipMemsetAsync(t.flags, 0, (size_t)n_seg * n_rows * 4, st));
  WCX_HIP(hipMemsetAsync(t.searched, 0, (size_t)n_rows, st));
  WCX_HIP(hipMemsetAsync(t.d_nredo, 0, 512, st));
  WCX_HIP(hipMemsetAsync(ctx->d_stats, 0, 256, st));
  rc = wcx_upload_small(ctx, d_blocks, blocks.data(), blocks.size() * sizeof(ScreenBlock));
  if (rc) return rc;
  k_mark<<<(unsigned)blocks.size(), 256, 0, st>>>(t.searched, d_blocks, row_begin);

  rc = wcx_timer_begin(ctx, "topk");
  if (rc) return rc;
  rc = wcx_timer_begin(ctx, "topk_prep");
  if (rc) return rc;
  rc = col_stats(dXs, B, S, cmean, glob, chr_cum, n_chr, t.tab, st);
  if (rc) return rc;
  const ChrTab &tab = t.tab;
  {
    const unsigned gb = (unsigned)((B + NT - 1) / NT);
    const unsigned gtn = (unsigned)((B + 31) / 32);
    WCX_HIP(hipMemsetAsync(cellcnt, 0, (size_t)2 * NCELL * 4, st));
    WCX_HIP(hipMemsetAsync(t.perm, 0xff, (size_t)Bpad * 4, st));
    if (use_hub1) {
      WCX_HIP(hipMemsetAsync(hubhist, 0, (size_t)HUB_BINS * 4, st));
      k_transpose_norm<<<gtn, 256, 0, st>>>(dXs, B, S, Sp, t.Xr, cmean, tab, glob, rbits, rchr, rfine, hubhist);
      k_hub_cut<<<1, 1024, 0, st>>>(hubhist, (int)p.hub_rows, glob);
      k_row_hist<<<gb, NT, 0, st>>>(rbits, rchr, B, 0, 0, glob, rkey, cellcnt, nullptr, rfine);
      k_scan_cells<<<1, 1024, 0, st>>>(cellcnt, cursor, 0, nullptr, glob);
    } else {
      k_transpose_norm<<<gtn, 256, 0, st>>>(dXs, B, S, Sp, t.Xr, cmean, tab, glob, rbits, rchr, nullptr, nullptr);
      k_row_hist<<<gb, NT, 0, st>>>(rbits, rchr, B, SF, n_seg > 1 ? 1 : 0, glob, rkey, cellcnt);
      k_scan_cells<<<1, 1024, 0, st>>>(cellcnt, cursor, (int)(P_s - n_s));
    }
    k_scatter<<<gb, NT, 0, st>>>(rkey, B, cursor, t.perm, rowpos);
    k_group_mask<<<(unsigned)((n_groups + NT - 1) / NT), NT, 0, st>>>(t.perm, rchr, n_groups, gmask);
  }
  screen_prep(NK, t.Xr, Bpad, S, Sp, cmean, t.perm, glob, F, info, nullptr, st);
  rc = end_prep(ctx, S);
  if (rc) return rc;

  const ScreenChunk ch =
      screen_chunk(cfg, n_seg > 1 ? kn.chunk_kb_small(24576) : kn.chunk_kb(NK > 16 ? 16384 : 3072));
  ScreenArgs a;
  a.F = F; a.Ft = F; a.info = info; a.glob = glob; a.perm = t.perm; a.rowpos = rowpos; a.gmask = gmask;
  a.blocks = d_blocks; a.sl = t.sl; a.cnt = t.cnt; a.flags = t.flags; a.g_state = g_state;
  a.stats = ctx->d_stats; a.row_begin = row_begin; a.n_rows_all = n_rows;
  a.k = k; a.dbg = ctx->debug_flags; a.n_seg = n_seg; a.n_blocks = (int)blocks.size();
  a.raw_est = 1;
  if (use_hub1) {
    rc = wcx_timer_begin(ctx, "topk_pre");
    if (rc) return rc;
    const ScreenCfg hc = default_cfg(NK);
    size_t n_hblocks = blocks.size();
    if (!hub_blocks.empty()) {
      rc = wcx_upload_small(ctx, d_hblocks, hub_blocks.data(), hub_blocks.size() * sizeof(ScreenBlock));
      if (rc) return rc;
      n_hblocks = hub_blocks.size();
    } else {
      d_hblocks = d_blocks;
    }
    Hub1Args ha;
    ha.F = F; ha.glob = glob; ha.perm = t.perm; ha.rowpos = rowpos; ha.gmask = gmask; ha.blocks = d_hblocks;
    ha.g_state = g_state; ha.cnt = t.cnt; ha.stats = ctx->d_stats; ha.row_begin = row_begin;
    ha.n_rows_all = n_rows; ha.n_seg = n_seg; ha.need = p.hub_need;
    ha.n1 = kn.hub_n1(16);
    const int hGR = hc.ctg * 32;
    int64_t cap_g = (p.hub_rows * 2 + hGR - 1) / hGR + 2;
    if (cap_g > Bpad / hGR) cap_g = Bpad / hGR;
    if (cap_g > 8192) cap_g = 8192;
    ha.glist_cap = (int)cap_g + 64;
    const size_t lds_h = (size_t)hc.ring * (size_t)(hc.ctg * NK * 64) * 16 + (size_t)ha.glist_cap * 4;
    const int trials = kn.hub1_trials((NK >= 16 || (int)n_hblocks <= p.hw_cus * hc.lb) ? 8 : 4);
    rc = unit_status(launch_unit(hub1_units, NK, hc.ctg, hc.lb, hc.ring, trials, ha, (unsigned)n_hblocks, lds_h, st),
                     "hub-count (one-directional)", hc, trials);
    if (rc) return rc;
    rc = wcx_timer_end(ctx, "topk_pre");
    if (rc) return rc;
  }
  const int n_streams = ((int)blocks.size() > p.slots && n_seg == 1) ? 2 : 1;
  hipStream_t st2 = st;
  if (n_streams == 2) {
    if (!ctx->sweep_stream) {
      WCX_HIP(hipStreamCreateWithFlags(&ctx->sweep_stream, hipStreamNonBlocking));
      WCX_HIP(hipEventCreateWithFlags(&ctx->ev_sweep0, hipEventDisableTiming));
      WCX_HIP(hipEventCreateWithFlags(&ctx->ev_sweep1, hipEventDisableTiming));
    }
    st2 = ctx->sweep_stream;
    WCX_HIP(hipEventRecord(ctx->ev_sweep0, st));
    WCX_HIP(hipStreamWaitEvent(st2, ctx->ev_sweep0, 0));
  }
  const int half0 = n_streams == 2 ? (int)(blocks.size() + 1) / 2 : (int)blocks.size();
  bool first = !use_hub1;
  auto launch = [&](int64_t g0, int64_t g1, int cut_k, int cut_mode, int trig, int end_cut) {
    a.g_start = g0; a.g_count = (int)(g1 - g0);
    a.cut_k = cut_k; a.cut_mode = cut_mode; a.trig = trig; a.end_cut = end_cut;
    a.first = first ? 1 : 0;
    first = false;
    for (int h = 0; h < n_streams; ++h) {
      a.blocks = d_blocks + (h ? half0 : 0);
      a.n_blocks = h ? (int)blocks.size() - half0 : half0;
      const int e = unit_status(launch_unit(screen_units, cfg, a, (unsigned)(a.n_blocks * n_seg), ch.lds,
                                            h ? st2 : st), "screen", cfg);
      if (e) return e;
    }
    return (int)WCX_OK;
  };
  const int trig_main = (ctx->debug_flags >> DBG_TRIG_SHIFT) ? (ctx->debug_flags >> DBG_TRIG_SHIFT) : LIM;
  int64_t g_main = 0;
  if (cut_r) {
    g_main = P_s / GRr;
    int trig_a = n_seg > 1 ? 2 * cut_r + 32 : 4 * cut_r + 64;
    if (trig_a > LIM) trig_a = LIM;
    for (int64_t g0 = 0; g0 < g_main; g0 += ch.groups) {
      const int64_t g1 = g0 + ch.groups < g_main ? g0 + ch.groups : g_main;
      rc = launch(g0, g1, cut_r, 1, trig_a, g1 == g_main ? 1 : 0);
      if (rc) return rc;
    }
    if (n_seg > 1)
      k_share_thresholds<<<(unsigned)((n_rows + NT - 1) / NT), NT, 0, st>>>(n_rows, n_seg, t.searched,
                                                                            g_state, t.cnt);
  }
  for (int64_t g0 = g_main; g0 < n_iter_groups; g0 += ch.groups) {
    const int64_t g1 = g0 + ch.groups < n_iter_groups ? g0 + ch.groups : n_iter_groups;
    rc = launch(g0, g1, k, 0, trig_main, g1 == n_iter_groups ? 2 : 0);
    if (rc) return rc;
  }
  if (n_seg > 1) {
    const unsigned gm = (unsigned)((n_rows + 3) / 4 < 65536 ? (n_rows + 3) / 4 : 65536);
    for (int step = 1; step < n_seg; step *= 2) {
      const unsigned pairs = (unsigned)((n_seg - step + 2 * step - 1) / (2 * step));
      k_merge_segments<<<dim3(gm, pairs), NT, 0, st>>>(info, glob, rowpos, row_begin, n_rows, t.searched, t.sl,
                                                       t.cnt, t.flags, g_state, step, n_seg, k, screen_gamma(NK),
                                                       step * 2 >= n_seg ? 1 : 0);
    }
  }
  if (n_streams == 2) {
    WCX_HIP(hipEventRecord(ctx->ev_sweep1, st2));
    WCX_HIP(hipStreamWaitEvent(st, ctx->ev_sweep1, 0));
  }
  WCX_HIP(hipGetLastError());
  rc = wcx_timer_end(ctx, "topk_screen");
  if (rc) return rc;
  return finish_topk(ctx, t, row_begin, n_rows, kick_after_sweep(S), d_out_idx, d_out_dist);
}

int wcx_topk_screen_launch(wcx_ctx *ctx, const double *dXs, int64_t B, int S,
                           const int64_t *chr_cum, int n_chr,
                           const std::vector<TopkBlock> &exact_blocks, int64_t row_begin,
                           int64_t n_rows, int k, int32_t *d_out_idx, double *d_out_dist) {
  if (exact_blocks.empty()) return WCX_OK;
  const Knobs kn;
  const ScreenPlan p = plan_search(ctx, B, S, k, row_begin == 0 && n_rows == B, kn, exact_blocks, chr_cum, n_chr);
  switch (p.path) {
    case ScreenPath::sym:
      return screen_sym_path(ctx, kn, p, dXs, B, S, chr_cum, n_chr, k, d_out_idx, d_out_dist);
    case ScreenPath::exact:
      return wcx_topk_exact_launch(ctx, dXs, B, S, exact_blocks, row_begin, n_rows, k, d_out_idx, d_out_dist);
    default:
      return screen_one_dir_path(ctx, kn, p, dXs, B, S, chr_cum, n_chr, row_begin, n_rows, k, d_out_idx,
                                 d_out_dist);
  }
}

void wcx_sym_state_free(wcx_ctx *ctx) {
  delete reinterpret_cast<SymShardState *>(ctx->sym_state);
  ctx->sym_state = nullptr;
}

int wcx_sym_shard_sweep(wcx_ctx *ctx, const double *dXs, int64_t B, int S, const int64_t *chr_cum, int n_chr,
                        int k, int part, int n_parts, const int64_t *row_bounds, int64_t *counts_out) {
  if (!wcx_screen_supported(B, S, k) || n_parts < 1 || n_parts > 32 || B < 32768) {
    wcx_set_error("sharded symmetric sweep: unsupported shape (B=%lld S=%d k=%d parts=%d)", (long long)B, S, k,
                  n_parts);
    return WCX_ERR_UNSUPPORTED;
  }
  const Knobs kn;
  ScreenPlan p = plan_shape(ctx, B, k, default_cfg(screen_nk(S)), kn);
// ... 67 lines not shown
```

wisecondorx_amd/csrc/null_ratios.hip:

```cpp
#include <algorithm>

#include "wave_sort.h"
#include "wcx_common.h"


namespace {

constexpr int NT = 256;
constexpr int BIN_BITS = 25;

__device__ __forceinline__ unsigned long long dkey(double x) {
  if (x != x) return ~0ull;
  x = x + 0.0;
  const unsigned long long u = (unsigned long long)__double_as_longlong(x);
  return (u >> 63) ? ~u : (u | 0x8000000000000000ull);
}

constexpr int RK_NS = 4096;
constexpr int RK_NB = 1024;
constexpr int RK_WMAX = 1024;
constexpr int RK_TILE = 4096;

__device__ __forceinline__ bool rk_less(unsigned long long ka, unsigned int ba, unsigned long long kb,
                                        unsigned int bb) {
// ... 602 lines not shown
  }
  const int r0 = (k - 1) >> 1, r1 = k >> 1;
  int my_c0 = 0, my_c1 = 0;
  double my_v0 = 0.0, my_v1 = 0.0;
  bool my_slow = false, my_nan = false;
#pragma unroll
  for (int s = 0; s < 8; ++s) {
    const int m = sg * 8 + s;
    if (m >= n_ids) break;
    unsigned int a0, a1, hi;
    wave_middle_u32<IPL>(v[s], act, k, s_hist[wave], s_slots[wave], a0, a1, hi);
    int below = 0, t0 = 0, t1 = 0, c0 = 0, c1 = 0;
#pragma unroll
    for (int q = 0; q < IPL; ++q) {
      const bool on = q < NFull<IPL>::value || q * 64 + lane < k;
      below += __popcll(__ballot(on && v[s][q] < a0));
      const unsigned long long e0 = __ballot(on && v[s][q] == a0);
      if (e0) {
        t0 += __popcll(e0);
        c0 = __builtin_amdgcn_readlane(cc[q], __builtin_amdgcn_readfirstlane(__ffsll((long long)e0) - 1));
      }
      if (a1 != a0) {
        const unsigned long long e1 = __ballot(on && v[s][q] == a1);
        if (e1) {
          t1 += __popcll(e1);
          c1 = __builtin_amdgcn_readlane(cc[q], __builtin_amdgcn_readfirstlane(__ffsll((long long)e1) - 1));
        }
      }
    }
    const bool fast = t0 == 1 && (r1 == r0 || (a1 != a0 && t1 == 1));
    if (fast) {
      if (lane == s) { my_c0 = c0; my_c1 = r1 == r0 ? c0 : c1; }
    } else {
      const double *x = Xs + (int64_t)sids[m] * B;
      const double v0 = pick_among_ties<IPL>(v[s], cc, act, a0, r0 - below, x, s_cand[wave]);
      double v1 = v0;
      if (r1 != r0)
        v1 = pick_among_ties<IPL>(v[s], cc, act, a1, a1 == a0 ? r1 - below : 0, x, s_cand[wave]);
      if (lane == s) { my_v0 = v0; my_v1 = v1; my_slow = true; }
    }
    if (lane == s) my_nan = hi == 0xffffffffu;
  }
  const int m = sg * 8 + lane;
  if (lane < 8 && m < n_ids) {
    const double *x = Xs + (int64_t)sids[m] * B;
    if (!my_slow) { my_v0 = x[my_c0]; my_v1 = x[my_c1]; }
    double med = (my_v0 + my_v1) / 2.0 + 0.0;
    if (my_nan) med = __builtin_nan("");
    out[r * (int64_t)n_ids + m] = log2(x[row_begin + r] / med);
  }
}

template <int IPL>
__global__ __launch_bounds__(NT) void k_null_ratios(
    const unsigned int *__restrict__ Rg, const double *__restrict__ V,
    const int *__restrict__ n_nan, const double *__restrict__ Xs,
    const int32_t *__restrict__ sids, int64_t B, const int32_t *__restrict__ idx,
    int64_t row_begin, int64_t n_rows, int k, int n_ids, double *__restrict__ out, int dbg) {
  const int lane = wcx::lane_id();
  const int wave = threadIdx.x >> 6;
  __shared__ int s_hist[NT / 64][64];
  __shared__ unsigned int s_slots[NT / 64][64];
  const int64_t r = (int64_t)blockIdx.x * (NT / 64) + wave;
  if (r >= n_rows) return;
  const int sg = blockIdx.y;
  const uint4 *slab = reinterpret_cast<const uint4 *>(Rg + (int64_t)sg * B * 8);
  unsigned int v[8][IPL];
  unsigned int act = 0;
#pragma unroll
  for (int q = 0; q < IPL; ++q) {
    const int t = q * 64 + lane;
    const bool valid = q < NFull<IPL>::value || t < k;
    int64_t c = valid ? (int64_t)idx[r * (int64_t)k + t] : 0;
    if (c < 0) c += B;
    act |= valid ? (1u << q) : 0u;
    uint4 a0, a1;
    if (dbg & 16) {
      a0 = make_uint4((unsigned)c, (unsigned)c * 3u, (unsigned)c ^ 0x55u, (unsigned)c + 7u);
      a1 = make_uint4((unsigned)c * 5u, (unsigned)c + 1u, (unsigned)c ^ 0x33u, (unsigned)c + 9u);
    } else { a0 = slab[c * 2]; a1 = slab[c * 2 + 1]; }
    v[0][q] = a0.x; v[1][q] = a0.y; v[2][q] = a0.z; v[3][q] = a0.w;
    v[4][q] = a1.x; v[5][q] = a1.y; v[6][q] = a1.z; v[7][q] = a1.w;
  }
  unsigned int my_a0 = 0, my_a1 = 0, my_hi = 0;
#pragma unroll
  for (int s = 0; s < 8; ++s) {
    unsigned int a0, a1, hi;
    if (dbg & 64) {
      a0 = 0;
#pragma unroll
      for (int q = 0; q < IPL; ++q) a0 ^= v[s][q];
      a0 = (unsigned int)__builtin_amdgcn_readfirstlane((int)a0) % (unsigned int)B; a1 = a0; hi = 0;
    } else
    wave_middle_u32<IPL>(v[s], act, k, s_hist[wave], s_slots[wave], a0, a1, hi);
    if (lane == s) { my_a0 = a0; my_a1 = a1; my_hi = hi; }
  }
  const int m = sg * 8 + lane;
  if (lane < 8 && m < n_ids) {
    const double *Vm = V + (int64_t)m * B;
    if (dbg & 16) { my_a0 %= (unsigned int)B; my_a1 %= (unsigned int)B; }
    double med = (Vm[my_a0] + Vm[my_a1]) / 2.0 + 0.0;
    if ((int64_t)my_hi >= B - n_nan[m]) med = __builtin_nan("");
    const double xr = Xs[(int64_t)sids[m] * B + row_begin + r];
    out[r * (int64_t)n_ids + m] = log2(xr / med);
  }
}

}

extern "C" {

struct RankLayout {
  size_t o_sid, o_nan, o_cnt, o_start, o_cursor, o_spk, o_spb, o_bkt, o_tk, o_tb, o_r, o_rg, o_v, total;
  int n_sg;
};

static int rank_layout(int64_t B, int n_ids, hipStream_t, RankLayout &L) {
  const int64_t n = (int64_t)n_ids * B;
  L.n_sg = (n_ids + 7) / 8;
  size_t off = 0;
  auto carve = [&](size_t bytes) { size_t o = off; off += (bytes + 255) / 256 * 256; return o; };
  L.o_sid = carve((size_t)n_ids * 4);
  L.o_nan = carve((size_t)n_ids * 4);
  L.o_cnt = carve((size_t)n_ids * RK_NB * 4);
  L.o_start = carve((size_t)n_ids * RK_NB * 4);
  L.o_cursor = carve((size_t)n_ids * RK_NB * 4);
  L.o_spk = carve((size_t)n_ids * RK_NB * 8);
  L.o_spb = carve((size_t)n_ids * RK_NB * 4);
  L.o_bkt = carve((size_t)n * 2);
  L.o_tk = carve((size_t)n * 8);
  L.o_tb = carve((size_t)n * 4);
  L.o_r = carve((size_t)n * 4);
  L.o_rg = carve((size_t)L.n_sg * B * 32);
  L.o_v = carve((size_t)n * 8);
  L.total = off;
  return WCX_OK;
}

static int rank_run(const double *dXs, int64_t B, int n_ids, const RankLayout &L, char *base,
                    hipStream_t st) {
  int32_t *d_sids = reinterpret_cast<int32_t *>(base + L.o_sid);
  int *d_nan = reinterpret_cast<int *>(base + L.o_nan);
  int *cnt = reinterpret_cast<int *>(base + L.o_cnt);
  int *start = reinterpret_cast<int *>(base + L.o_start);
  int *cursor = reinterpret_cast<int *>(base + L.o_cursor);
  unsigned long long *spk = reinterpret_cast<unsigned long long *>(base + L.o_spk);
  unsigned int *spb = reinterpret_cast<unsigned int *>(base + L.o_spb);
  unsigned short *bkt = reinterpret_cast<unsigned short *>(base + L.o_bkt);
  unsigned long long *tk = reinterpret_cast<unsigned long long *>(base + L.o_tk);
  unsigned int *tb = reinterpret_cast<unsigned int *>(base + L.o_tb);
  unsigned int *R = reinterpret_cast<unsigned int *>(base + L.o_r);
  unsigned int *Rg = reinterpret_cast<unsigned int *>(base + L.o_rg);
  double *V = reinterpret_cast<double *>(base + L.o_v);
  WCX_HIP(hipMemsetAsync(d_nan, 0, (size_t)n_ids * 4, st));
  WCX_HIP(hipMemsetAsync(cnt, 0, (size_t)n_ids * RK_NB * 4, st));
  const unsigned gb = (unsigned)((B + RK_TILE - 1) / RK_TILE);
  k_rank_splitters<<<(unsigned)n_ids, 1024, 0, st>>>(dXs, B, d_sids, spk, spb);
  k_rank_bucket<<<dim3((unsigned)n_ids, gb), NT, 0, st>>>(dXs, B, d_sids, spk, spb, bkt, cnt, d_nan);
  k_rank_scan<<<(unsigned)n_ids, RK_NB, 0, st>>>(cnt, start, cursor);
  k_rank_scatter<<<dim3((unsigned)n_ids, gb), NT, 0, st>>>(dXs, B, d_sids, bkt, cursor, tk, tb);
  k_rank_sort<<<(unsigned)(L.n_sg * 8 * (RK_NB / (NT / 64))), NT, 0, st>>>(B, n_ids, start, cnt, tk, tb, R, V);
  k_rank_pieces<<<dim3((unsigned)((B + NT - 1) / NT), (unsigned)L.n_sg), NT, 0, st>>>(R, B, n_ids, Rg);
  WCX_HIP(hipGetLastError());
  return WCX_OK;
}

}

size_t wcx_rank_bytes(int64_t B, int n) {
  RankLayout L;
  rank_layout(B, n, nullptr, L);
  return L.total;
}

int wcx_rank_rows_launch(const double *d_x, int64_t B, int n, char *base, hipStream_t st, WcxRankView *out) {
  WCX_ARG(n > 0 && n <= 128 && B < (1ll << BIN_BITS) && (int64_t)n * B < (1ll << 31), "too many rows / bins to rank");
  RankLayout L;
  rank_layout(B, n, st, L);
  k_iota_i32<<<1, 128, 0, st>>>(reinterpret_cast<int32_t *>(base + L.o_sid), n);
  const int rc = rank_run(d_x, B, n, L, base, st);
  if (rc) return rc;
  out->Rg = reinterpret_cast<unsigned int *>(base + L.o_rg);
  out->V = reinterpret_cast<const double *>(base + L.o_v);
  out->n_sg = L.n_sg;
  return WCX_OK;
}

int wcx_norm_rank_mark_launch(const WcxRankView &rk, const double *copyT, int64_t B, int NS, int n_samples,
                              hipStream_t st) {
  k_norm_rank_mark<<<dim3((unsigned)((B + NT - 1) / NT), (unsigned)rk.n_sg), NT, 0, st>>>(rk.Rg, copyT, B, NS,
                                                                                          n_samples);
  WCX_HIP(hipGetLastError());
  return WCX_OK;
}

int wcx_norm_median_rank_launch(const WcxRankView &rk, const int32_t *d_idx, const unsigned long long *d_sel,
                                const double *xT, int64_t B, int k, int ipl, int NS, int n_samples, int64_t ct,
                                const WcxChrCum &chr, double *rT, double *lrT, hipStream_t st) {
  const int64_t n_rows = B - ct;
  if (n_rows <= 0) return WCX_OK;
  const dim3 grid((unsigned)((n_rows + NT / 64 - 1) / (NT / 64)), (unsigned)rk.n_sg);
#define WCX_NMR_LAUNCH(IPL)                                                                            \
  k_norm_median_rank<IPL><<<grid, NT, 0, st>>>(rk.Rg, rk.V, d_idx, d_sel, xT, B, k, NS, n_samples, ct, chr, rT, lrT)
  switch (ipl) {
    case 1: WCX_NMR_LAUNCH(1); break;
    case 2: WCX_NMR_LAUNCH(2); break;
    case 3: WCX_NMR_LAUNCH(3); break;
    case 4: WCX_NMR_LAUNCH(4); break;
    case 5: WCX_NMR_LAUNCH(5); break;
    case 6: WCX_NMR_LAUNCH(6); break;
    case 7: WCX_NMR_LAUNCH(7); break;
    case 8: WCX_NMR_LAUNCH(8); break;
    default:
      wcx_set_error("rank medians: %d values per lane are not instantiated", ipl);
      return WCX_ERR_UNSUPPORTED;
  }
#undef WCX_NMR_LAUNCH
  WCX_HIP(hipGetLastError());
  return WCX_OK;
}

extern "C" {

static int check_ids(const int32_t *sample_ids, int n_ids, int S) {
  for (int i = 0; i < n_ids; ++i)
    WCX_ARG(sample_ids[i] >= 0 && sample_ids[i] < S, "sample id out of range");
  return WCX_OK;
}

int wcx_null_rank_prepare_dev(wcx_ctx *ctx, const double *dXs, int64_t B, int S,
                              const int32_t *sample_ids, int n_ids) {
  WCX_ARG(ctx && dXs && sample_ids, "NULL argument");
  WCX_ARG(B > 0 && S > 0 && n_ids > 0, "bad sizes");
  WCX_ARG(B < (1ll << BIN_BITS) && n_ids <= 128, "too many bins / null samples");
  WCX_ARG((int64_t)n_ids * B < (1ll << 31), "null samples x bins exceeds 2^31");
  int rc = check_ids(sample_ids, n_ids, S);
  if (rc) return rc;
  WCX_HIP(hipSetDevice(ctx->device));
  if (!ctx->aux_stream) {
    WCX_HIP(hipStreamCreateWithFlags(&ctx->aux_stream, hipStreamNonBlocking));
    WCX_HIP(hipEventCreateWithFlags(&ctx->ev_main, hipEventDisableTiming));
    WCX_HIP(hipEventCreateWithFlags(&ctx->ev_rank, hipEventDisableTiming));
  }
  RankLayout L;
  rc = rank_layout(B, n_ids, ctx->aux_stream, L);
  if (rc) return rc;
  if (ctx->rank_bytes < L.total) {
    WCX_HIP(hipStreamSynchronize(ctx->aux_stream));
    WCX_HIP(hipStreamSynchronize(ctx->stream));
    if (ctx->d_rank) { WCX_HIP(hipFree(ctx->d_rank)); ctx->d_rank = nullptr; ctx->rank_bytes = 0; }
    if (hipMalloc(&ctx->d_rank, L.total) != hipSuccess) {
      wcx_set_error("hipMalloc(%zu) for the null-sample ranks failed", L.total);
      return WCX_ERR_NOMEM;
    }
    ctx->rank_bytes = L.total;
  }
  ctx->rank_ids.assign(sample_ids, sample_ids + n_ids);
  ctx->rank_X = dXs;
  ctx->rank_B = B;
  ctx->rank_pending = true;
  return WCX_OK;
}

}

constexpr int ND_ROWS = 32;
__global__ __launch_bounds__(256) void k_null_dummy(const double *__restrict__ Xs, int64_t B,
                                                    const int32_t *__restrict__ sids, int n_ids,
                                                    int64_t row_begin, int64_t n_rows,
                                                    double *__restrict__ out) {
  __shared__ double tile[ND_ROWS][129];
  const int64_t r0 = (int64_t)blockIdx.x * ND_ROWS;
  const int rl = threadIdx.x & (ND_ROWS - 1), part = threadIdx.x / ND_ROWS;
  const int64_t r = r0 + rl;
  for (int m = part; m < n_ids; m += 256 / ND_ROWS) {
    const double *x = Xs + (int64_t)sids[m] * B;
    if (r < n_rows) tile[rl][m] = log2(x[row_begin + r] / x[0]);
  }
  __syncthreads();
  const int64_t rows_here = n_rows - r0 < ND_ROWS ? n_rows - r0 : ND_ROWS;
  const int64_t total = rows_here * n_ids;
  double *dst = out + r0 * n_ids;
  for (int64_t e = threadIdx.x; e < total; e += 256) {
    const int rr = (int)(e / n_ids), mm = (int)(e - (int64_t)rr * n_ids);
    dst[e] = tile[rr][mm];
  }
}

bool wcx_null_ratios_direct_pays(int64_t B, int64_t n_rows) {
  static const int ratio = [] {
    const char *e = getenv("WCX_NR_DIRECT_RATIO");
    return e && *e ? atoi(e) : 4;
  }();
  return ratio > 0 && n_rows * ratio <= B + B / 64;
}

void wcx_aux_cancel_if_few_rows(wcx_ctx *ctx, int64_t B, int64_t n_rows) {
  if (ctx->rank_pending && wcx_null_ratios_direct_pays(B, n_rows)) {
    ctx->rank_pending = false;
    ctx->rank_X = nullptr;
  }
}

int wcx_aux_kick(wcx_ctx *ctx) {
  if (!ctx->rank_pending) return WCX_OK;
  ctx->rank_pending = false;
  const int n_ids = (int)ctx->rank_ids.size();
  RankLayout L;
// ... 162 lines not shown
```

wisecondorx_amd/csrc/predict.hip:

```cpp
#include "wave_sort.h"
#include "wcx_common.h"

namespace {

constexpr int NT = 256;
constexpr double Z_MASK = 2.3263478740408408;

__global__ __launch_bounds__(NT) void k_cut_partial(const double *__restrict__ d, int64_t n,
                                                    const double *__restrict__ state, int phase,
                                                    double *__restrict__ part_sum,
                                                    double *__restrict__ part_cnt) {
  const double cutoff = state[0];
  const double mean = state[1];
  double s = 0.0, c = 0.0;
  const int64_t stride = (int64_t)gridDim.x * NT * 2;
  for (int64_t i = ((int64_t)blockIdx.x * NT + threadIdx.x) * 2; i < n; i += stride) {
    double2 v;
    if (i + 1 < n) v = *reinterpret_cast<const double2 *>(d + i);
    else { v.x = d[i]; v.y = __builtin_nan(""); }
    if (v.x < cutoff) { if (phase == 0) { s += v.x; c += 1.0; } else { double e = v.x - mean; s += e * e; } }
    if (v.y < cutoff) { if (phase == 0) { s += v.y; c += 1.0; } else { double e = v.y - mean; s += e * e; } }
  }
  __shared__ double sh_s[NT / 64], sh_c[NT / 64];
  s = wcx::wave_sum(s);
  c = wcx::wave_sum(c);
  if ((threadIdx.x & 63) == 0) { sh_s[threadIdx.x >> 6] = s; sh_c[threadIdx.x >> 6] = c; }
  __syncthreads();
  if (threadIdx.x == 0) {
    double ts = 0.0, tc = 0.0;
    for (int w = 0; w < NT / 64; ++w) { ts += sh_s[w]; tc += sh_c[w]; }
    part_sum[blockIdx.x] = ts;
    part_cnt[blockIdx.x] = tc;
  }
}

__global__ __launch_bounds__(NT) void k_cut_final(double *__restrict__ state, int phase,
                                                  const double *__restrict__ part_sum,
                                                  const double *__restrict__ part_cnt, int nparts) {
  double s = 0.0, c = 0.0;
  for (int i = threadIdx.x; i < nparts; i += NT) { s += part_sum[i]; c += part_cnt[i]; }
  __shared__ double sh_s[NT / 64], sh_c[NT / 64];
  s = wcx::wave_sum(s);
  c = wcx::wave_sum(c);
  if ((threadIdx.x & 63) == 0) { sh_s[threadIdx.x >> 6] = s; sh_c[threadIdx.x >> 6] = c; }
  __syncthreads();
  if (threadIdx.x == 0) {
    double ts = 0.0, tc = 0.0;
    for (int w = 0; w < NT / 64; ++w) { ts += sh_s[w]; tc += sh_c[w]; }
    if (phase == 0) {
      state[2] = tc;
      state[1] = ts / tc;
    } else {
      const double sd = sqrt(ts / state[2]);
      state[0] = state[1] + 3.0 * sd;
    }
  }
}

__global__ __launch_bounds__(NT) void k_sum_parts(const double *__restrict__ part_sum,
                                                  const double *__restrict__ part_cnt, int nparts,
                                                  double *__restrict__ out) {
  double s = 0.0, c = 0.0;
  for (int i = threadIdx.x; i < nparts; i += NT) { s += part_sum[i]; c += part_cnt[i]; }
  __shared__ double sh_s[NT / 64], sh_c[NT / 64];
  s = wcx::wave_sum(s);
  c = wcx::wave_sum(c);
  if ((threadIdx.x & 63) == 0) { sh_s[threadIdx.x >> 6] = s; sh_c[threadIdx.x >> 6] = c; }
  __syncthreads();
  if (threadIdx.x == 0) {
    double ts = 0.0, tc = 0.0;
    for (int w = 0; w < NT / 64; ++w) { ts += sh_s[w]; tc += sh_c[w]; }
    out[0] = ts;
    out[1] = tc;
  }
}

__global__ __launch_bounds__(NT) void k_weights(const double *__restrict__ dist, int64_t B, int k,
                                                double *__restrict__ out) {
  const int lane = wcx::lane_id();
  const int64_t w0 = ((int64_t)blockIdx.x * NT + threadIdx.x) >> 6;
  const int64_t nw = ((int64_t)gridDim.x * NT) >> 6;
  for (int64_t i = w0; i < B; i += nw) {
    double s = 0.0;
    for (int t = lane; t < k; t += 64) s += sqrt(dist[i * (int64_t)k + t]);
    s = wcx::wave_sum(s);
    if (lane == 0) out[i] = 1.0 / (s / (double)k);
  }
}

__global__ __launch_bounds__(NT) void k_select_mask(const double *__restrict__ dist, int k, int ipl,
                                                    double cutoff, int64_t lo, int64_t hi,
                                                    int64_t row0,
                                                    unsigned long long *__restrict__ sel) {
  const int lane = wcx::lane_id();
  const int64_t w0 = ((int64_t)blockIdx.x * NT + threadIdx.x) >> 6;
  const int64_t nw = ((int64_t)gridDim.x * NT) >> 6;
  for (int64_t i = lo + w0; i < hi; i += nw) {
    const int64_t li = i - row0;
    for (int q = 0; q < ipl; ++q) {
      const int t = q * 64 + lane;
      const bool s = (t < k) && (dist[li * (int64_t)k + t] < cutoff);
      const unsigned long long m = __ballot(s);
      if (lane == 0) sel[li * ipl + q] = m;
    }
  }
}

struct ChrTable {
  int n_chr;
  int64_t cum[32];
};

template <int IPL>
__global__ __launch_bounds__(NT) void k_normalize_pass(
    const double *__restrict__ x, const double *__restrict__ copy_in,
    double *__restrict__ copy_out, const int32_t *__restrict__ idx,
    const unsigned long long *__restrict__ sel, int64_t B, int k, int64_t ct, int64_t lo,
    int64_t hi, int64_t row0, ChrTable chr, double *__restrict__ out_z,
    double *__restrict__ out_r, double *__restrict__ out_n, double *__restrict__ out_lr,
    int last_pass) {
  const int lane = wcx::lane_id();
  __shared__ int s_hist[NT / 64][64];
  __shared__ double s_slots[NT / 64][64];
  const int s = blockIdx.y;
  const double *xs = x + (int64_t)s * B;
  const double *cin = copy_in + (int64_t)s * B;
  double *cout = copy_out + (int64_t)s * B;
  const int64_t Bp = B - ct;
  const int64_t w0 = ((int64_t)blockIdx.x * NT + threadIdx.x) >> 6;
  const int64_t nw = ((int64_t)gridDim.x * NT) >> 6;
  for (int64_t i = lo + w0; i < hi; i += nw) {
    const int64_t li = i - row0;
    int64_t cs = 0, ce = chr.cum[0];
    for (int c = 1; c < chr.n_chr && i >= ce; ++c) { cs = ce; ce = chr.cum[c]; }
    const int64_t own = ce - cs;
    const int64_t len_cd = B - own;
    double v[IPL];
    int nloc = 0;
    unsigned int keepmask = 0;
    double sloc = 0.0;
#pragma unroll
    for (int q = 0; q < IPL; ++q) {
      const int t = q * 64 + lane;
      const bool selq = (t < k) && ((sel[li * IPL + q] >> lane) & 1ull);
      double val = HUGE_VAL;
      bool keep = false;
      if (selq) {
        int64_t c = idx[li * (int64_t)k + t];
        if (c < 0) c += len_cd;
        const int64_t g = c < cs ? c : c + own;
        const double cv = cin[g];
        keep = cv >= 0.0;
        if (keep) val = cv;
      }
      v[q] = val;
      if (keep) { nloc += 1; sloc += val; keepmask |= 1u << q; }
    }
    const int n = wcx::wave_sum_i(nloc);
    const double mean = wcx::wave_sum(sloc) / (double)n;
    double ssl = 0.0;
#pragma unroll
    for (int q = 0; q < IPL; ++q) {
      if ((keepmask >> q) & 1u) { const double e = v[q] - mean; ssl += e * e; }
    }
    const double sd = sqrt(wcx::wave_sum(ssl) / (double)n);
    double med = 1.0;
    if (last_pass)
      med = wcx::wave_median_bucket<IPL>(v, keepmask, n, s_hist[threadIdx.x >> 6],
                                         s_slots[threadIdx.x >> 6], mean, sd);
    if (lane == 0) {
      const double xi = xs[i];
      const double z = (xi - mean) / sd;
      const double r = xi / med;
      const int64_t o = (int64_t)s * Bp + (i - ct);
      out_z[o] = z;
      out_r[o] = r;
      out_n[o] = (double)n;
      if (last_pass) out_lr[o] = log2(r);
      cout[i] = (fabs(z) >= Z_MASK) ? -1.0 : cin[i];
    }
  }
}

template <int IPL, int T>
__global__ __launch_bounds__(NT) void k_normalize_pass_tile(
    const double *__restrict__ x, const double *__restrict__ copy_in,
    double *__restrict__ copy_out, const int32_t *__restrict__ idx,
    const unsigned long long *__restrict__ sel, int64_t B, int k, int NS, int n_samples, int64_t ct,
    int64_t lo, int64_t hi, ChrTable chr, double *__restrict__ out_z, double *__restrict__ out_r,
    double *__restrict__ out_n, double *__restrict__ out_lr, int last_pass) {
  const int lane = wcx::lane_id();
  __shared__ int s_hist[NT / 64][64];
  __shared__ double s_slots[NT / 64][64];
  const int s0 = blockIdx.y * T;
  const int64_t Bp = B - ct;
  const int64_t w0 = ((int64_t)blockIdx.x * NT + threadIdx.x) >> 6;
  const int64_t nw = ((int64_t)gridDim.x * NT) >> 6;
  for (int64_t i = lo + w0; i < hi; i += nw) {
    int64_t cs = 0, ce = chr.cum[0];
    for (int c = 1; c < chr.n_chr && i >= ce; ++c) { cs = ce; ce = chr.cum[c]; }
    const int64_t own = ce - cs;
    const int64_t len_cd = B - own;
    double v[T][IPL];
    unsigned int selmask = 0;
#pragma unroll
    for (int q = 0; q < IPL; ++q) {
      const int t = q * 64 + lane;
      const bool selq = (t < k) && ((sel[i * IPL + q] >> lane) & 1ull);
      if (selq) {
        int64_t c = idx[i * (int64_t)k + t];
        if (c < 0) c += len_cd;
        const int64_t g = c < cs ? c : c + own;
        const double *src = copy_in + g * NS + s0;
#pragma unroll
        for (int s = 0; s < T; ++s) v[s][q] = src[s];
        selmask |= 1u << q;
      } else {
#pragma unroll
        for (int s = 0; s < T; ++s) v[s][q] = -1.0;
      }
    }
    double st_n = 0.0, st_mean = 0.0, st_q = 0.0, st_med = 1.0;
#pragma unroll
    for (int s = 0; s < T; ++s) {
// ... 243 lines not shown
    }
    const bool was = ((st_was ? st_was : st_mask)[i * n_tiles + blockIdx.y] >> lane) & 1ull;
    copy_out[i * NS + s] = (was || fabs(z) >= Z_MASK) ? -1.0 : c0;
    if (st_mask_new) {
      st_S1[i * NS + s] = S1;
      st_S2[i * NS + s] = S2;
      st_n[i * NS + s] = n | (s2_tag << 16);
      const unsigned long long m = __ballot(!was && fabs(z) >= Z_MASK && c0 >= 0.0);
      if (lane == 0) st_mask_new[i * n_tiles + blockIdx.y] = m;
    }
  }
}

__global__ __launch_bounds__(256) void k_from_sample_minor(const double *__restrict__ aT, int64_t ct, int64_t Bp,
                                                           int NS, int n_samples, double *__restrict__ out) {
  __shared__ double tile[32][33];
  const int64_t b0 = (int64_t)blockIdx.x * 32;
  const int s0 = blockIdx.y * 32;
  const int tx = threadIdx.x & 31, ty = threadIdx.x >> 5;
  for (int r = ty; r < 32; r += 8) {
    const int64_t bb = b0 + r;
    const int sx = s0 + tx;
    tile[r][tx] = (bb < Bp && sx < NS) ? aT[(ct + bb) * NS + sx] : 0.0;
  }
  __syncthreads();
  for (int r = ty; r < 32; r += 8) {
    const int sx = s0 + r;
    const int64_t bb = b0 + tx;
    if (sx < n_samples && bb < Bp) out[(int64_t)sx * Bp + bb] = tile[tx][r];
  }
}

__global__ __launch_bounds__(256) void k_to_sample_minor(const double *__restrict__ x, int64_t B,
                                                         int n_samples, int NS, double *__restrict__ a,
                                                         double *__restrict__ b) {
  __shared__ double tile[32][33];
  const int64_t b0 = (int64_t)blockIdx.x * 32;
  const int s0 = blockIdx.y * 32;
  const int tx = threadIdx.x & 31, ty = threadIdx.x >> 5;
  for (int r = ty; r < 32; r += 8) {
    const int s = s0 + r;
    const int64_t bb = b0 + tx;
    tile[r][tx] = (s < n_samples && bb < B) ? x[(int64_t)s * B + bb] : 0.0;
  }
  __syncthreads();
  for (int r = ty; r < 32; r += 8) {
    const int64_t bb = b0 + r;
    const int s = s0 + tx;
    if (bb < B && s < NS) { const double v = tile[tx][r]; a[bb * NS + s] = v; b[bb * NS + s] = v; }
  }
}

__device__ __forceinline__ unsigned long long f64_key(double x) {
  unsigned long long b = (unsigned long long)__double_as_longlong(x);
  return (b >> 63) ? ~b : (b | 0x8000000000000000ull);
}
__device__ __forceinline__ double key_f64(unsigned long long kx) {
  unsigned long long b = (kx >> 63) ? (kx & 0x7fffffffffffffffull) : ~kx;
  return __longlong_as_double((long long)b);
}

constexpr int NTM = 1024;

__global__ __launch_bounds__(NTM) void k_nanmedian(const double *__restrict__ a0,
                                                   const double *__restrict__ a1, int64_t n,
                                                   int64_t array_stride, double *__restrict__ out0,
                                                   double *__restrict__ out1) {
  const double *a = (blockIdx.y ? a1 : a0) + (int64_t)blockIdx.x * array_stride;
  double *out = blockIdx.y ? out1 : out0;
  __shared__ unsigned int hist[2][256];
  __shared__ unsigned long long prefix[2];
  __shared__ long long rank[2];
  __shared__ long long nvalid;
  const int tid = threadIdx.x;
  if (tid == 0) nvalid = 0;
  __syncthreads();
  constexpr int NMU = 8;
  long long loc = 0;
  for (int64_t i0 = 0; i0 < n; i0 += (int64_t)NTM * NMU) {
    double xs[NMU];
#pragma unroll
    for (int u = 0; u < NMU; ++u) {
      const int64_t i = i0 + (int64_t)u * NTM + tid;
      xs[u] = i < n ? a[i] : __builtin_nan("");
    }
#pragma unroll
    for (int u = 0; u < NMU; ++u) loc += (xs[u] == xs[u]);
    if (i0 + NTM >= n) break;
  }
  loc = (long long)wcx::wave_sum_i((int)loc);
  if ((tid & 63) == 0) atomicAdd((unsigned long long *)&nvalid, (unsigned long long)loc);
  __syncthreads();
  const long long nv = nvalid;
  if (nv == 0) { if (tid == 0) out[blockIdx.x] = __builtin_nan(""); return; }
  if (tid == 0) { rank[0] = (nv - 1) / 2; rank[1] = nv / 2; prefix[0] = 0; prefix[1] = 0; }
  unsigned long long himask = 0;
  for (int shift = 56; shift >= 0; shift -= 8) {
    if (tid < 256) { hist[0][tid] = 0; hist[1][tid] = 0; }
    __syncthreads();
    const unsigned long long p0 = prefix[0], p1 = prefix[1];
    const bool two = p1 != p0;
    auto count = [&](bool on, unsigned int dg, unsigned int *h) {
      const unsigned long long m = __ballot(on);
      if (m == 0ull) return;
      const int first = __ffsll((long long)m) - 1;
      const unsigned int dgf = (unsigned int)__builtin_amdgcn_readlane((int)dg, first);
      if (__ballot(on && dg == dgf) == m) {
        if ((tid & 63) == first) atomicAdd(&h[dgf], (unsigned int)__popcll(m));
      } else if (on) {
        atomicAdd(&h[dg], 1u);
      }
    };
    for (int64_t i0 = 0; i0 < n; i0 += (int64_t)NTM * NMU) {
      double xs[NMU];
#pragma unroll
      for (int u = 0; u < NMU; ++u) {
        const int64_t i = i0 + (int64_t)u * NTM + tid;
        xs[u] = i < n ? a[i] : __builtin_nan("");
      }
#pragma unroll
      for (int u = 0; u < NMU; ++u) {
        if (i0 + (int64_t)u * NTM >= n) break;
        const double x = xs[u];
        const bool ok = x == x;
        const unsigned long long kx = f64_key(x);
        const unsigned int dg = (unsigned int)((kx >> shift) & 255ull);
        count(ok && (kx & himask) == p0, dg, hist[0]);
        if (two) count(ok && (kx & himask) == p1, dg, hist[1]);
      }
    }
    __syncthreads();
    if (!two && tid < 256) hist[1][tid] = hist[0][tid];
    __syncthreads();
    if (tid < 2) {
      long long rk = rank[tid];
      int dg = 0;
      for (; dg < 256; ++dg) {
        const long long h = hist[tid][dg];
        if (rk < h) break;
        rk -= h;
      }
      rank[tid] = rk;
      prefix[tid] |= ((unsigned long long)dg) << shift;
    }
    himask |= 255ull << shift;
    __syncthreads();
  }
  if (tid == 0) {
    const double lo = key_f64(prefix[0]), hi = key_f64(prefix[1]);
    out[blockIdx.x] = (nv & 1) ? lo : (lo + hi) / 2.0;
  }
}

struct NmState { unsigned long long prefix[2]; long long rank[2]; unsigned long long himask; long long nvalid; };

__global__ __launch_bounds__(256) void k_nm_count(const double *__restrict__ a0,
                                                  const double *__restrict__ a1, int64_t n,
                                                  NmState *__restrict__ st) {
  const double *a = blockIdx.y ? a1 : a0;
  long long loc = 0;
  for (int64_t i = (int64_t)blockIdx.x * 256 + threadIdx.x; i < n; i += (int64_t)gridDim.x * 256) {
    const double x = a[i];
    loc += (x == x);
  }
  loc = (long long)wcx::wave_sum_i((int)loc);
  if ((threadIdx.x & 63) == 0 && loc) atomicAdd((unsigned long long *)&st[blockIdx.y].nvalid, (unsigned long long)loc);
}

__global__ void k_nm_init(NmState *__restrict__ st, unsigned int *__restrict__ hist) {
  const int a = blockIdx.x;
  if (threadIdx.x == 0) {
    const long long nv = st[a].nvalid;
    st[a].rank[0] = nv > 0 ? (nv - 1) / 2 : 0;
    st[a].rank[1] = nv / 2;
    st[a].prefix[0] = st[a].prefix[1] = 0;
    st[a].himask = 0;
  }
  for (int i = threadIdx.x; i < 512; i += blockDim.x) hist[a * 512 + i] = 0;
}

__global__ __launch_bounds__(256) void k_nm_hist(const double *__restrict__ a0,
                                                 const double *__restrict__ a1, int64_t n, int shift,
                                                 const NmState *__restrict__ st,
                                                 unsigned int *__restrict__ hist) {
  const int arr = blockIdx.y;
  const double *a = arr ? a1 : a0;
  __shared__ unsigned int lh[2][256];
  lh[0][threadIdx.x] = 0;
  lh[1][threadIdx.x] = 0;
  __syncthreads();
  const unsigned long long p0 = st[arr].prefix[0], p1 = st[arr].prefix[1], himask = st[arr].himask;
  const bool two = p1 != p0;
  for (int64_t i = (int64_t)blockIdx.x * 256 + threadIdx.x; i < n; i += (int64_t)gridDim.x * 256) {
    const double x = a[i];
    if (x == x) {
      const unsigned long long kx = f64_key(x);
      const unsigned int dg = (unsigned int)((kx >> shift) & 255ull);
      if ((kx & himask) == p0) atomicAdd(&lh[0][dg], 1u);
      if (two && (kx & himask) == p1) atomicAdd(&lh[1][dg], 1u);
    }
  }
  __syncthreads();
  if (lh[0][threadIdx.x]) atomicAdd(&hist[arr * 512 + threadIdx.x], lh[0][threadIdx.x]);
  if (two && lh[1][threadIdx.x]) atomicAdd(&hist[arr * 512 + 256 + threadIdx.x], lh[1][threadIdx.x]);
}

__global__ __launch_bounds__(512) void k_nm_decide(NmState *__restrict__ st,
                                                    unsigned int *__restrict__ hist, int shift,
                                                    double *__restrict__ out0,
                                                    double *__restrict__ out1) {
  const int a = blockIdx.x;
  const int t = threadIdx.x >> 8, d = threadIdx.x & 255;
  const bool two = st[a].prefix[1] != st[a].prefix[0];
  __shared__ long long cum[2][256];
  const long long rk = st[a].rank[t];
  const long long mine = hist[a * 512 + ((t == 1 && two) ? 256 : 0) + d];
  cum[t][d] = mine;
  __syncthreads();
  for (int off = 1; off < 256; off <<= 1) {
    const long long v = d >= off ? cum[t][d - off] : 0;
    __syncthreads();
    cum[t][d] += v;
    __syncthreads();
  }
  const long long incl = cum[t][d], excl = incl - mine;
  __syncthreads();
  if (rk >= excl && rk < incl) {
    st[a].rank[t] = rk - excl;
    st[a].prefix[t] |= ((unsigned long long)d) << shift;
  }
  hist[a * 512 + threadIdx.x] = 0;
  __syncthreads();
  if (threadIdx.x == 0) {
    __threadfence();
    st[a].himask |= 255ull << shift;
    if (shift == 0) {
      double *out = a ? out1 : out0;
      const long long nv = st[a].nvalid;
      const double lo = key_f64(st[a].prefix[0]), hi = key_f64(st[a].prefix[1]);
      out[0] = nv == 0 ? __builtin_nan("") : ((nv & 1) ? lo : (lo + hi) / 2.0);
    }
  }
}

__global__ void k_copy2(const double *__restrict__ src, double *__restrict__ a,
                        double *__restrict__ b, int64_t n) {
  int64_t i = (int64_t)blockIdx.x * blockDim.x + threadIdx.x;
  if (i < n) { const double v = src[i]; a[i] = v; b[i] = v; }
}

}

static int launch_nanmedian_wide(wcx_ctx *ctx, const double *a0, const double *a1, int64_t n,
                                 double *out0, double *out1) {
  void *scr = ctx->d_small;
  NmState *st = reinterpret_cast<NmState *>(scr);
  unsigned int *hist = reinterpret_cast<unsigned int *>(reinterpret_cast<char *>(scr) + 256);
  hipStream_t s = ctx->stream;
  WCX_HIP(hipMemsetAsync(st, 0, 2 * sizeof(NmState), s));
  const unsigned g = (unsigned)std::min<int64_t>(256, (n + 255) / 256 > 0 ? (n + 255) / 256 : 1);
  k_nm_count<<<dim3(g, 2), 256, 0, s>>>(a0, a1, n, st);
  k_nm_init<<<2, 256, 0, s>>>(st, hist);
  for (int shift = 56; shift >= 0; shift -= 8) {
    k_nm_hist<<<dim3(g, 2), 256, 0, s>>>(a0, a1, n, shift, st, hist);
    k_nm_decide<<<2, 512, 0, s>>>(st, hist, shift, out0, out1);
  }
  WCX_HIP(hipGetLastError());
  return WCX_OK;
}

int wcx_nanmedian_rows_launch(wcx_ctx *ctx, const double *d_a, int64_t n, int64_t stride, int count,
                              double *d_out) {
  k_nanmedian<<<dim3((unsigned)count, 1), NTM, 0, ctx->stream>>>(d_a, d_a, n, stride, d_out, d_out);
  WCX_HIP(hipGetLastError());
  return WCX_OK;
}

namespace {

__global__ __launch_bounds__(1024) void k_nanmean1(const double *__restrict__ w, int64_t n,
                                                   double *__restrict__ out) {
  __shared__ double ss[16];
  __shared__ double sc[16];
  __shared__ double sb[16];
  double s = 0.0, c = 0.0, bad = 0.0;
  for (int64_t i = threadIdx.x; i < n; i += 1024) {
    const double v = w[i];
    if (v == v) { s += v; c += 1.0; }
    if (!(v - v == 0.0)) bad += 1.0;
  }
  s = wcx::wave_sum(s);
  c = wcx::wave_sum(c);
  bad = wcx::wave_sum(bad);
  if ((threadIdx.x & 63) == 0) { ss[threadIdx.x >> 6] = s; sc[threadIdx.x >> 6] = c; sb[threadIdx.x >> 6] = bad; }
  __syncthreads();
  if (threadIdx.x == 0) {
    double a = 0.0, b = 0.0, nb = 0.0;
    for (int q = 0; q < 16; ++q) { a += ss[q]; b += sc[q]; nb += sb[q]; }
    const double m = a / b;
    out[0] = m;
    out[1] = (nb > 0.0 || !(m - m == 0.0) || m == 0.0) ? 1.0 : 0.0;
  }
}

__global__ __launch_bounds__(256) void k_post_process(
    const double *__restrict__ z, const double *__restrict__ r, const double *__restrict__ nref,
    const double *__restrict__ w, int64_t B, const double *__restrict__ m_lr,
    const double *__restrict__ m_z, const double *__restrict__ wmean, double minrefbins,
    const int32_t *__restrict__ pos, int64_t n_bins, double *__restrict__ full) {
  const int64_t i = (int64_t)blockIdx.x * 256 + threadIdx.x;
  if (i >= B) return;
  const bool keep = nref[i] >= minrefbins;
  double lr = log2(keep ? r[i] : 0.0);
  const bool good = (lr - lr == 0.0);
  lr = good ? lr : 0.0;
  if (lr != 0.0) lr -= m_lr[0];
  const int64_t p = pos[i];
  full[p] = lr;
  full[n_bins + p] = good ? z[i] - m_z[0] : 0.0;
  full[2 * n_bins + p] = good ? (wmean[1] != 0.0 ? 1.0 : w[i] / wmean[0]) : 0.0;
}

__global__ __launch_bounds__(1024) void k_prep_total(const int32_t *__restrict__ counts, int64_t n_bins,
                                                     double *__restrict__ total) {
  __shared__ double red[16];
  const int32_t *c = counts + (int64_t)blockIdx.x * n_bins;
  double s = 0.0;
  for (int64_t i = threadIdx.x; i < n_bins; i += 1024) s += (double)c[i];
  s = wcx::wave_sum(s);
  if ((threadIdx.x & 63) == 0) red[threadIdx.x >> 6] = s;
  __syncthreads();
  if (threadIdx.x == 0) {
    double t = 0.0;
    for (int q = 0; q < 16; ++q) t += red[q];
    total[blockIdx.x] = t;
  }
}

constexpr int PSL = 64;
template <int NC>
__global__ __launch_bounds__(256) void k_prep_depth(const int32_t *__restrict__ counts, int64_t n_bins,
                                                    const double *__restrict__ total,
                                                    const int32_t *__restrict__ pos, int64_t B,
                                                    const double *__restrict__ mean,
                                                    const double *__restrict__ comps,
                                                    double *__restrict__ x, double *__restrict__ part) {
  __shared__ double red[NC][4];
  const int s = blockIdx.y, sl = blockIdx.x;
  const int64_t per = (B + PSL - 1) / PSL, lo = sl * per, hi = lo + per < B ? lo + per : B;
  const int32_t *c = counts + (int64_t)s * n_bins;
  const double tot = total[s];
  double acc[NC];
#pragma unroll
  for (int q = 0; q < NC; ++q) acc[q] = 0.0;
  for (int64_t i = lo + threadIdx.x; i < hi; i += 256) {
    const double v = (double)c[pos[i]] / tot;
    x[(int64_t)s * B + i] = v;
    const double e = v - mean[i];
#pragma unroll
    for (int q = 0; q < NC; ++q) acc[q] += comps[(int64_t)q * B + i] * e;
  }
#pragma unroll
  for (int q = 0; q < NC; ++q) {
    const double t = wcx::wave_sum(acc[q]);
    if ((threadIdx.x & 63) == 0) red[q][threadIdx.x >> 6] = t;
  }
  __syncthreads();
  if (threadIdx.x < NC)
    part[((int64_t)s * PSL + sl) * NC + threadIdx.x] =
        red[threadIdx.x][0] + red[threadIdx.x][1] + red[threadIdx.x][2] + red[threadIdx.x][3];
}

template <int NC>
__global__ __launch_bounds__(256) void k_prep_project(const double *__restrict__ part, int64_t B,
                                                      const double *__restrict__ mean,
                                                      const double *__restrict__ comps,
                                                      double *__restrict__ x) {
  const int s = blockIdx.y;
  double t[NC];
#pragma unroll
  for (int q = 0; q < NC; ++q) {
    double a = 0.0;
    for (int sl = 0; sl < PSL; ++sl) a += part[((int64_t)s * PSL + sl) * NC + q];
    t[q] = a;
  }
  const int64_t i = (int64_t)blockIdx.x * 256 + threadIdx.x;
  if (i >= B) return;
  double rec = mean[i];
#pragma unroll
  for (int q = 0; q < NC; ++q) rec += t[q] * comps[(int64_t)q * B + i];
  x[(int64_t)s * B + i] = x[(int64_t)s * B + i] / rec;
}

__global__ __launch_bounds__(1024) void k_wstats(const double *__restrict__ w, int64_t n,
                                                 double *__restrict__ out) {
  __shared__ double ss[16], sc[16], sb[16];
  double s = 0.0, c = 0.0, bad = 0.0;
  for (int64_t i = threadIdx.x; i < n; i += 1024) {
    const double v = w[i];
    if (v == v) { s += v; c += 1.0; }
    if (!(v - v == 0.0)) bad += 1.0;
  }
  s = wcx::wave_sum(s); c = wcx::wave_sum(c); bad = wcx::wave_sum(bad);
  if ((threadIdx.x & 63) == 0) { ss[threadIdx.x >> 6] = s; sc[threadIdx.x >> 6] = c; sb[threadIdx.x >> 6] = bad; }
  __syncthreads();
  if (threadIdx.x == 0) {
    double a = 0.0, b = 0.0, nb = 0.0;
    for (int q = 0; q < 16; ++q) { a += ss[q]; b += sc[q]; nb += sb[q]; }
    out[0] = a / b; out[1] = b; out[2] = nb;
  }
}

__global__ __launch_bounds__(1024) void k_wmerge(const double *__restrict__ wA, int64_t BA,
                                                 const double *__restrict__ wG, int64_t BG,
                                                 const double *__restrict__ stA,
                                                 const double *__restrict__ stG,
                                                 double *__restrict__ wout, int *__restrict__ fallback) {
  __shared__ double ss[16], sc[16];
  __shared__ double s_mean;
  __shared__ int s_bad;
  const double mA = stA[0], mG = BG ? stG[0] : 1.0;
  const double fa = BG ? mG : 1.0, fg = mA;
  double s = 0.0, c = 0.0;
  for (int64_t i = threadIdx.x; i < BA + BG; i += 1024) {
    const double v = i < BA ? wA[i] * fa : wG[i - BA] * fg;
    if (v == v) { s += v; c += 1.0; }
  }
  s = wcx::wave_sum(s); c = wcx::wave_sum(c);
  if ((threadIdx.x & 63) == 0) { ss[threadIdx.x >> 6] = s; sc[threadIdx.x >> 6] = c; }
  __syncthreads();
  if (threadIdx.x == 0) {
    double a = 0.0, b = 0.0;
    for (int q = 0; q < 16; ++q) { a += ss[q]; b += sc[q]; }
    const double m = a / b;
    s_mean = m;
    const bool bad = stA[2] > 0.0 || (BG && stG[2] > 0.0) || !(m - m == 0.0) || m == 0.0 ||
                     !(fa - fa == 0.0) || !(fg - fg == 0.0);
    s_bad = bad ? 1 : 0;
    *fallback = s_bad;
  }
  __syncthreads();
  const double m = s_mean;
  const bool bad = s_bad != 0;
  for (int64_t i = threadIdx.x; i < BA + BG; i += 1024) {
    const double v = i < BA ? wA[i] * fa : wG[i - BA] * fg;
    wout[i] = bad ? 1.0 : v / m;
  }
}

__global__ __launch_bounds__(256) void k_post_merge(
    const double *__restrict__ zA, const double *__restrict__ rA, const double *__restrict__ nA,
    int64_t BA, const double *__restrict__ zG, const double *__restrict__ rG,
    const double *__restrict__ nG, int64_t BG, const double *__restrict__ wfin,
    const double *__restrict__ m_lr, const double *__restrict__ m_z, double minrefbins,
    const int32_t *__restrict__ pos, int64_t n_bins, double *__restrict__ out_r,
    double *__restrict__ out_z, double *__restrict__ out_w) {
  const int64_t i = (int64_t)blockIdx.x * 256 + threadIdx.x;
  const int s = blockIdx.y;
  if (i >= BA + BG) return;
  const bool aut = i < BA;
  const int64_t j = aut ? (int64_t)s * BA + i : (int64_t)s * BG + (i - BA);
  const double nref = aut ? nA[j] : nG[j], rr = aut ? rA[j] : rG[j], zz = aut ? zA[j] : zG[j];
  const bool keep = nref >= minrefbins;
  double lr = log2(keep ? rr : 0.0);
  const bool good = (lr - lr == 0.0);
  lr = good ? lr : 0.0;
  if (lr != 0.0) lr -= m_lr[s];
  const int64_t p = (int64_t)s * n_bins + pos[i];
  out_r[p] = lr;
  out_z[p] = good && keep ? zz - m_z[s] : 0.0;
  out_w[p] = good && keep ? wfin[i] : 0.0;
}

}

void wcx_ref_release_sel(wcx_ctx *ctx, wcx_ref *ref);

extern "C" {

int wcx_ref_wrap_dev(wcx_ctx *ctx, const int32_t *d_idx, const double *d_dist, int64_t B, int k,
                     const int64_t *chr_cum, int n_chr, wcx_ref **out) {
  WCX_ARG(ctx && d_idx && d_dist && chr_cum && out, "NULL argument");
  WCX_ARG(B > 0 && k > 0 && n_chr > 0 && n_chr <= 32, "bad sizes (n_chr <= 32)");
  WCX_ARG(chr_cum[n_chr - 1] == B, "chr_cum[n_chr-1] must equal B");
  wcx_ref *r = new wcx_ref();
  r->d_idx = d_idx;
  r->d_dist = d_dist;
  r->owned = false;
  r->B = B;
  r->k = k;
  r->row0 = 0;
  r->nrows = B;
  r->chr_cum.assign(chr_cum, chr_cum + n_chr);
  *out = r;
  return WCX_OK;
}

int wcx_ref_upload(wcx_ctx *ctx, const int32_t *idx, const double *dist, int64_t B, int k,
                   const int64_t *chr_cum, int n_chr, wcx_ref **out) {
  WCX_ARG(ctx && idx && dist && chr_cum && out, "NULL argument");
  WCX_ARG(B > 0 && k > 0, "bad sizes");
  WCX_HIP(hipSetDevice(ctx->device));
  void *di = nullptr, *dd = nullptr;
  const size_t ib = (size_t)B * k * 4, db = (size_t)B * k * 8;
  if (hipMalloc(&di, ib) != hipSuccess || hipMalloc(&dd, db) != hipSuccess) {
    if (di) hipFree(di);
    wcx_set_error("hipMalloc failed for a %lld x %d reference", (long long)B, k);
    return WCX_ERR_NOMEM;
  }
  WCX_HIP(hipMemcpyAsync(di, idx, ib, hipMemcpyHostToDevice, ctx->stream));
  WCX_HIP(hipMemcpyAsync(dd, dist, db, hipMemcpyHostToDevice, ctx->stream));
  WCX_HIP(hipStreamSynchronize(ctx->stream));
  int rc = wcx_ref_wrap_dev(ctx, (const int32_t *)di, (const double *)dd, B, k, chr_cum, n_chr, out);
  if (rc) { hipFree(di); hipFree(dd); return rc; }
  (*out)->owned = true;
  return WCX_OK;
}

int wcx_ref_free(wcx_ctx *ctx, wcx_ref *ref) {
  if (!ref) return WCX_OK;
  if (ctx) wcx_ref_release_sel(ctx, ref);
  else if (ref->d_sel) hipFree(ref->d_sel);
  if (ref->owned) {
    if (ctx) hipStreamSynchronize(ctx->stream);
    hipFree(const_cast<int32_t *>(ref->d_idx));
    hipFree(const_cast<double *>(ref->d_dist));
  }
  delete ref;
  return WCX_OK;
}

int wcx_cutoff(wcx_ctx *ctx, const wcx_ref *ref, int repeats, double *cutoff) {
  WCX_ARG(ctx && ref && cutoff, "NULL argument");
  WCX_ARG(repeats >= 0, "repeats must be >= 0");
  WCX_HIP(hipSetDevice(ctx->device));
  const int64_t n = ref->nrows * (int64_t)ref->k;
  const int nparts = 2048;
  void *scr = nullptr;
  int rc = wcx_scratch(ctx, (size_t)(2 * nparts + 8) * 8, &scr);
  if (rc) return rc;
  double *state = reinterpret_cast<double *>(scr);
  double *ps = state + 8, *pc = ps + nparts;
  const double init[3] = {HUGE_VAL, 0.0, 0.0};
  rc = wcx_upload_small(ctx, state, init, sizeof(init));
  if (rc) return rc;
  rc = wcx_timer_begin(ctx, "cutoff");
  if (rc) return rc;
  for (int rep = 0; rep < repeats; ++rep) {
    for (int phase = 0; phase < 2; ++phase) {
      k_cut_partial<<<nparts, NT, 0, ctx->stream>>>(ref->d_dist, n, state, phase, ps, pc);
      k_cut_final<<<1, NT, 0, ctx->stream>>>(state, phase, ps, pc, nparts);
    }
  }
  WCX_HIP(hipGetLastError());
  rc = wcx_timer_end(ctx, "cutoff");
  if (rc) return rc;
  WCX_HIP(hipMemcpyAsync(cutoff, state, 8, hipMemcpyDeviceToHost, ctx->stream));
  WCX_HIP(hipStreamSynchronize(ctx->stream));
  return WCX_OK;
}

int wcx_weights_dev(wcx_ctx *ctx, const wcx_ref *ref, double *d_out) {
  WCX_ARG(ctx && ref && d_out, "NULL argument");
  WCX_HIP(hipSetDevice(ctx->device));
  int rc = wcx_timer_begin(ctx, "weights");
  if (rc) return rc;
  const unsigned grid = (unsigned)((ref->nrows + 3) / 4 < 8192 ? (ref->nrows + 3) / 4 + 1 : 8192);
  k_weights<<<grid, NT, 0, ctx->stream>>>(ref->d_dist, ref->nrows, ref->k, d_out);
  WCX_HIP(hipGetLastError());
  return wcx_timer_end(ctx, "weights");
}

int wcx_post_process_dev(wcx_ctx *ctx, const double *d_z, const double *d_r, const double *d_n,
                         const double *d_w, int64_t B, const double *d_m_lr, const double *d_m_z,
                         double minrefbins, const int32_t *d_pos, int64_t n_bins, double *out_r,
                         double *out_z, double *out_w) {
  WCX_ARG(ctx && d_z && d_r && d_n && d_w && d_m_lr && d_m_z && d_pos && out_r && out_z && out_w,
          "NULL argument");
  WCX_ARG(B > 0 && n_bins >= B, "bad sizes");
  WCX_HIP(hipSetDevice(ctx->device));
  void *scr = nullptr;
  int rc = wcx_scratch2(ctx, (size_t)n_bins * 24 + 256, &scr);
  if (rc) return rc;
  double *full = reinterpret_cast<double *>(scr);
  double *d_wmean = full + 3 * n_bins;
  hipStream_t st = ctx->stream;
  WCX_HIP(hipMemsetAsync(full, 0, (size_t)n_bins * 24, st));
  k_nanmean1<<<1, 1024, 0, st>>>(d_w, B, d_wmean);
  k_post_process<<<(unsigned)((B + 255) / 256), 256, 0, st>>>(d_z, d_r, d_n, d_w, B, d_m_lr, d_m_z,
                                                             d_wmean, minrefbins, d_pos, n_bins, full);
  WCX_HIP(hipGetLastError());
  WCX_HIP(hipMemcpyAsync(out_r, full, (size_t)n_bins * 8, hipMemcpyDeviceToHost, st));
  WCX_HIP(hipMemcpyAsync(out_z, full + n_bins, (size_t)n_bins * 8, hipMemcpyDeviceToHost, st));
  WCX_HIP(hipMemcpyAsync(out_w, full + 2 * n_bins, (size_t)n_bins * 8, hipMemcpyDeviceToHost, st));
  WCX_HIP(hipStreamSynchronize(st));
  return WCX_OK;
}

int wcx_predict_prep_dev(wcx_ctx *ctx, const int32_t *d_counts, int n_samples, int64_t n_bins,
                         const int32_t *d_pos, int64_t B, const double *d_mean, const double *d_comps,
                         int n_comp, double *d_x) {
  WCX_ARG(ctx && d_counts && d_pos && d_mean && d_comps && d_x, "NULL argument");
  WCX_ARG(n_samples > 0 && n_bins >= B && B > 0, "bad sizes");
  WCX_ARG(n_comp == 5, "this build instantiates 5 components (newref_tools.py:138: pcacomp=5)");
  WCX_HIP(hipSetDevice(ctx->device));
  void *scr = nullptr;
  int rc = wcx_scratch2(ctx, (size_t)n_samples * (8 + (size_t)PSL * 5 * 8) + 256, &scr);
  if (rc) return rc;
  double *d_total = reinterpret_cast<double *>(scr);
  double *d_part = d_total + n_samples;
  hipStream_t st = ctx->stream;
  k_prep_total<<<(unsigned)n_samples, 1024, 0, st>>>(d_counts, n_bins, d_total);
  k_prep_depth<5><<<dim3(PSL, (unsigned)n_samples), 256, 0, st>>>(d_counts, n_bins, d_total, d_pos, B,
                                                                  d_mean, d_comps, d_x, d_part);
  k_prep_project<5><<<dim3((unsigned)((B + 255) / 256), (unsigned)n_samples), 256, 0, st>>>(
      d_part, B, d_mean, d_comps, d_x);
  WCX_HIP(hipGetLastError());
  return WCX_OK;
}

int wcx_post_process_merge_dev(wcx_ctx *ctx, const double *d_zA, const double *d_rA,
                               const double *d_nA, const double *d_wA, int64_t BA,
                               const double *d_zG, const double *d_rG, const double *d_nG,
                               const double *d_wG, int64_t BG, int n_samples, const double *d_m_lr,
                               const double *d_m_z, double minrefbins, const int32_t *d_pos,
                               int64_t n_bins, double *d_out_r, double *d_out_z, double *d_out_w,
                               int *weights_fallback) {
  WCX_ARG(ctx && d_zA && d_rA && d_nA && d_wA && d_m_lr && d_m_z && d_pos && d_out_r && d_out_z && d_out_w,
          "NULL argument");
  WCX_ARG(BG == 0 || (d_zG && d_rG && d_nG && d_wG), "gonosomal part incomplete");
  WCX_ARG(BA > 0 && BG >= 0 && n_samples > 0 && n_bins >= BA + BG, "bad sizes");
  WCX_HIP(hipSetDevice(ctx->device));
  void *scr = nullptr;
  int rc = wcx_scratch2(ctx, (size_t)(BA + BG) * 8 + 512, &scr);
  if (rc) return rc;
  double *d_wfin = reinterpret_cast<double *>(scr);
  double *d_st = d_wfin + (BA + BG);
  int *d_fb = reinterpret_cast<int *>(d_st + 8);
  hipStream_t st = ctx->stream;
  WCX_HIP(hipMemsetAsync(d_out_r, 0, (size_t)n_samples * n_bins * 8, st));
  WCX_HIP(hipMemsetAsync(d_out_z, 0, (size_t)n_samples * n_bins * 8, st));
  WCX_HIP(hipMemsetAsync(d_out_w, 0, (size_t)n_samples * n_bins * 8, st));
  k_wstats<<<1, 1024, 0, st>>>(d_wA, BA, d_st);
  if (BG) k_wstats<<<1, 1024, 0, st>>>(d_wG, BG, d_st + 3);
  k_wmerge<<<1, 1024, 0, st>>>(d_wA, BA, d_wG, BG, d_st, d_st + 3, d_wfin, d_fb);
  k_post_merge<<<dim3((unsigned)((BA + BG + 255) / 256), (unsigned)n_samples), 256, 0, st>>>(
      d_zA, d_rA, d_nA, BA, d_zG, d_rG, d_nG, BG, d_wfin, d_m_lr, d_m_z, minrefbins, d_pos, n_bins,
      d_out_r, d_out_z, d_out_w);
  WCX_HIP(hipGetLastError());
  if (weights_fallback) {
    WCX_HIP(hipMemcpyAsync(weights_fallback, d_fb, 4, hipMemcpyDeviceToHost, st));
    WCX_HIP(hipStreamSynchronize(st));
  }
  return WCX_OK;
}

int wcx_weights(wcx_ctx *ctx, const wcx_ref *ref, double *out) {
  WCX_ARG(ctx && ref && out, "NULL argument");
  WCX_HIP(hipSetDevice(ctx->device));
  void *scr = nullptr;
  int rc = wcx_scratch(ctx, (size_t)ref->nrows * 8 + 8, &scr);
  if (rc) return rc;
  rc = wcx_timer_begin(ctx, "weights");
  if (rc) return rc;
  const unsigned grid = (unsigned)((ref->nrows + 3) / 4 < 8192 ? (ref->nrows + 3) / 4 + 1 : 8192);
  k_weights<<<grid, NT, 0, ctx->stream>>>(ref->d_dist, ref->nrows, ref->k, (double *)scr);
  WCX_HIP(hipGetLastError());
  rc = wcx_timer_end(ctx, "weights");
  if (rc) return rc;
  if (ref->nrows)
    WCX_HIP(hipMemcpyAsync(out, scr, (size_t)ref->nrows * 8, hipMemcpyDeviceToHost, ctx->stream));
  WCX_HIP(hipStreamSynchronize(ctx->stream));
  return WCX_OK;
}

}

namespace {

int ipl_for(int k) {
  int ipl = (k + 63) / 64;
  if (ipl > 8) ipl = ipl <= 16 ? 16 : 32;
  return ipl;
}

void sel_release(wcx_ctx *ctx, wcx_ref *ref) {
  if (!ref->d_sel) return;
  for (auto &sl : ctx->sel_pool)
    if (sl.p == ref->d_sel) sl.used = false;
  ref->d_sel = nullptr;
  ref->sel_bytes = 0;
}

int ensure_sel(wcx_ctx *ctx, wcx_ref *ref, int ipl) {
  const size_t need = (size_t)ref->nrows * ipl * 8;
  if (ref->d_sel && ref->sel_bytes >= need) return WCX_OK;
  sel_release(ctx, ref);
  int best = -1;
  for (size_t i = 0; i < ctx->sel_pool.size(); ++i) {
    const auto &sl = ctx->sel_pool[i];
    if (!sl.used && sl.bytes >= need && (best < 0 || sl.bytes < ctx->sel_pool[best].bytes)) best = (int)i;
  }
  if (best < 0) {
    wcx_ctx::SelSlot sl{nullptr, need ? need : 8, false};
    if (hipMalloc(&sl.p, sl.bytes) != hipSuccess) {
      wcx_set_error("hipMalloc(%zu) for the selection mask failed", need);
      return WCX_ERR_NOMEM;
    }
    ctx->sel_pool.push_back(sl);
    best = (int)ctx->sel_pool.size() - 1;
  }
  ctx->sel_pool[best].used = true;
  ref->d_sel = reinterpret_cast<unsigned long long *>(ctx->sel_pool[best].p);
  ref->sel_bytes = ctx->sel_pool[best].bytes;
  return WCX_OK;
}

int launch_pass(wcx_ctx *ctx, const wcx_ref *ref, const double *d_x, const double *cin, double *cout,
                int n_samples, int64_t ct, bool last, double *d_z, double *d_r, double *d_n,
                double *d_lr) {
  const int64_t B = ref->B;
  const int k = ref->k;
  const int ipl = ipl_for(k);
  const int64_t lo = ct > ref->row0 ? ct : ref->row0, hi = ref->row0 + ref->nrows;
  if (lo >= hi) return WCX_OK;
  ChrTable tab;
  tab.n_chr = (int)ref->chr_cum.size();
  for (int c = 0; c < 32; ++c) tab.cum[c] = c < tab.n_chr ? ref->chr_cum[c] : B;
  const int64_t nl = hi - lo;
  dim3 grid((unsigned)((nl + 3) / 4 < 16384 ? (nl + 3) / 4 : 16384), (unsigned)n_samples);
#define WCX_NORM_LAUNCH(IPL)                                                                  \
  k_normalize_pass<IPL><<<grid, NT, 0, ctx->stream>>>(d_x, cin, cout, ref->d_idx, ref->d_sel, B, k, \
                                                      ct, lo, hi, ref->row0, tab, d_z, d_r, d_n,    \
                                                      d_lr, last ? 1 : 0)
  switch (ipl) {
    case 1: WCX_NORM_LAUNCH(1); break;
    case 2: WCX_NORM_LAUNCH(2); break;
    case 3: WCX_NORM_LAUNCH(3); break;
    case 4: WCX_NORM_LAUNCH(4); break;
    case 5: WCX_NORM_LAUNCH(5); break;
    case 6: WCX_NORM_LAUNCH(6); break;
    case 7: WCX_NORM_LAUNCH(7); break;
    case 8: WCX_NORM_LAUNCH(8); break;
    case 16: WCX_NORM_LAUNCH(16); break;
    default: WCX_NORM_LAUNCH(32); break;
  }
#undef WCX_NORM_LAUNCH
  WCX_HIP(hipGetLastError());
  return WCX_OK;
}

template <int T>
int launch_pass_tile(wcx_ctx *ctx, const wcx_ref *ref, const double *d_x, const double *cin,
                     double *cout, int n_samples, int NS, int64_t ct, bool last, double *d_z,
                     double *d_r, double *d_n, double *d_lr) {
  const int64_t B = ref->B;
  const int k = ref->k;
  const int ipl = ipl_for(k);
  const int64_t lo = ct, hi = B;
  if (lo >= hi) return WCX_OK;
  ChrTable tab;
  tab.n_chr = (int)ref->chr_cum.size();
  for (int c = 0; c < 32; ++c) tab.cum[c] = c < tab.n_chr ? ref->chr_cum[c] : B;
  const int64_t nl = hi - lo;
  dim3 grid((unsigned)((nl + 3) / 4 < 16384 ? (nl + 3) / 4 : 16384), (unsigned)((n_samples + T - 1) / T));
#define WCX_NORMT_LAUNCH(IPL)                                                                     \
  k_normalize_pass_tile<IPL, T><<<grid, NT, 0, ctx->stream>>>(d_x, cin, cout, ref->d_idx, ref->d_sel, \
                                                               B, k, NS, n_samples, ct, lo, hi, tab, \
                                                               d_z, d_r, d_n, d_lr, last ? 1 : 0)
  switch (ipl) {
    case 1: WCX_NORMT_LAUNCH(1); break;
    case 2: WCX_NORMT_LAUNCH(2); break;
    case 3: WCX_NORMT_LAUNCH(3); break;
    case 4: WCX_NORMT_LAUNCH(4); break;
    case 5: WCX_NORMT_LAUNCH(5); break;
    case 6: WCX_NORMT_LAUNCH(6); break;
    case 7: WCX_NORMT_LAUNCH(7); break;
    default: WCX_NORMT_LAUNCH(8); break;
  }
#undef WCX_NORMT_LAUNCH
  WCX_HIP(hipGetLastError());
  return WCX_OK;
}

int launch_select_mask(wcx_ctx *ctx, wcx_ref *ref, double cutoff, int64_t ct) {
  const int ipl = ipl_for(ref->k);
  int rc = ensure_sel(ctx, ref, ipl);
  if (rc) return rc;
  const int64_t lo = ct > ref->row0 ? ct : ref->row0, hi = ref->row0 + ref->nrows;
  if (lo >= hi) return WCX_OK;
  const int64_t nl = hi - lo;
  const unsigned gsel = (unsigned)((nl + 3) / 4 < 16384 ? (nl + 3) / 4 : 16384);
  k_select_mask<<<gsel, NT, 0, ctx->stream>>>(ref->d_dist, ref->k, ipl, cutoff, lo, hi, ref->row0,
                                              ref->d_sel);
  WCX_HIP(hipGetLastError());
// ... 19 lines not shown
  const int n_chr = (int)ref->chr_cum.size();
  WCX_ARG(cp >= 0 && cp < n_chr, "cp out of range");
  WCX_ARG(ct == (cp ? ref->chr_cum[cp - 1] : 0), "ct must be the first row of chromosome cp");
  WCX_HIP(hipSetDevice(ctx->device));
  if (ref->k > 64 * 32) {
    wcx_set_error("refsize %d too large for the normalise kernel (max 2048)", ref->k);
    return WCX_ERR_UNSUPPORTED;
  }
  const int64_t Bp = B - ct;
  if (Bp <= 0) return WCX_OK;
  constexpr int TILE = 8;
  const bool tiled = n_samples >= 2 && ipl_for(ref->k) <= 8;
  static const int lanes_min = [] { const char *e = getenv("WCX_NORM_LANES_MIN"); return e && *e ? atoi(e) : 16; }();
  const bool lanes = tiled && n_samples >= lanes_min;
  const int NS = lanes ? (n_samples + 63) / 64 * 64 : tiled ? (n_samples + TILE - 1) / TILE * TILE : n_samples;
  const size_t cp_b = (size_t)NS * B * 8;
  const size_t lr_b = (size_t)n_samples * Bp * 8;
  static const int incr_on = [] { const char *e = getenv("WCX_NORM_INCR"); return e && *e ? atoi(e) : 1; }();
  const bool incr = lanes && incr_on;
  const size_t st_b = incr ? 2 * cp_b + (size_t)NS * B * 4 + (size_t)B * (NS / 64) * 8 + 256 : 0;
  static const int rankmed_on = [] { const char *e = getenv("WCX_NORM_RANKMED"); return e && *e ? atoi(e) : 1; }();
  const bool rankmed = incr && rankmed_on && n_samples <= 128 && B < (1ll << 25) &&
                       (int64_t)n_samples * B < (1ll << 31) && Bp * 4 >= B;
  const size_t mw_b = (size_t)B * (NS / 64) * 8 + 256;
  const size_t rk_b = rankmed ? 2 * mw_b + 4 * cp_b + wcx_rank_bytes(B, n_samples) + 1024 : 0;
  void *scr = nullptr;
  int rc = wcx_scratch(ctx, (lanes ? 3 : 2) * cp_b + lr_b + st_b + rk_b, &scr);
  if (rc) return rc;
  double *cA = reinterpret_cast<double *>(scr);
  double *cB = cA + (size_t)NS * B;
  double *lr = cB + (size_t)NS * B;
  double *xT = lanes ? lr + (size_t)n_samples * Bp : nullptr;
  double *stS1 = incr ? xT + (size_t)NS * B : nullptr;
  double *stS2 = incr ? stS1 + (size_t)NS * B : nullptr;
  unsigned long long *stM = incr ? reinterpret_cast<unsigned long long *>(stS2 + (size_t)NS * B) : nullptr;
  int *stN = incr ? reinterpret_cast<int *>(stM + (size_t)B * (NS / 64) + 8) : nullptr;
  char *rkp = rankmed ? reinterpret_cast<char *>(stN) + ((size_t)NS * B * 4 + 255) / 256 * 256 : nullptr;
  unsigned long long *stM1 = reinterpret_cast<unsigned long long *>(rkp);
  unsigned long long *stM01 = reinterpret_cast<unsigned long long *>(rkp + mw_b);
  double *zT = reinterpret_cast<double *>(rkp + 2 * mw_b);
  double *nT = rankmed ? zT + (size_t)NS * B : nullptr;
  double *rT = rankmed ? nT + (size_t)NS * B : nullptr;
  double *lrT = rankmed ? rT + (size_t)NS * B : nullptr;
  char *rank_base = rankmed ? reinterpret_cast<char *>(lrT + (size_t)NS * B) : nullptr;
  (void)stM01;
  rc = wcx_timer_begin(ctx, "normalize");
  if (rc) return rc;
  WcxRankView rkv{nullptr, nullptr, 0};
  if (rankmed) {
    rc = wcx_rank_rows_launch(d_x, B, n_samples, rank_base, ctx->stream, &rkv);
    if (rc) return rc;
  }
  if (tiled) {
    k_to_sample_minor<<<dim3((unsigned)((B + 31) / 32), (unsigned)((NS + 31) / 32)), 256, 0,
                        ctx->stream>>>(d_x, B, n_samples, NS, cA, cB);
    if (lanes)
      k_to_sample_minor<<<dim3((unsigned)((B + 31) / 32), (unsigned)((NS + 31) / 32)), 256, 0,
                          ctx->stream>>>(d_x, B, n_samples, NS, xT, xT);
  } else {
    const int64_t ntot = (int64_t)n_samples * B;
    k_copy2<<<(unsigned)((ntot + 255) / 256), 256, 0, ctx->stream>>>(d_x, cA, cB, ntot);
  }
  rc = launch_select_mask(ctx, ref, cutoff, ct);
  if (rc) return rc;
  for (int pass = 0; pass < 3; ++pass) {
    const double *cin = (pass & 1) ? cB : cA;
    double *cout = (pass & 1) ? cA : cB;
    if (lanes && pass < 2) {
      ChrTable tab;
      tab.n_chr = (int)ref->chr_cum.size();
      for (int c = 0; c < 32; ++c) tab.cum[c] = c < tab.n_chr ? ref->chr_cum[c] : B;
      const dim3 grid((unsigned)((Bp + 3) / 4 < 16384 ? (Bp + 3) / 4 : 16384), (unsigned)(NS / 64));
      if (incr && pass == 0) {
        if (ct > 0) WCX_HIP(hipMemsetAsync(stM, 0, (size_t)ct * (NS / 64) * 8, ctx->stream));
        k_normalize_mask_lanes<<<grid, NT, 0, ctx->stream>>>(xT, cin, cout, ref->d_idx, ref->d_sel, B, ref->k,
                                                             ipl_for(ref->k), NS, ct, B, tab, stS1, stS2, stN, stM);
      } else if (incr) {
        if (rankmed && ct > 0) WCX_HIP(hipMemsetAsync(stM1, 0, (size_t)ct * (NS / 64) * 8, ctx->stream));
        k_normalize_mask_incr<<<grid, NT, 0, ctx->stream>>>(xT, cout, ref->d_idx, ref->d_sel, B, ref->k,
                                                            ipl_for(ref->k), NS, ct, B, tab, stS1, stS2, stN, stM,
                                                            nullptr, rankmed ? stM1 : nullptr);
      } else {
        k_normalize_mask_lanes<<<grid, NT, 0, ctx->stream>>>(xT, cin, cout, ref->d_idx, ref->d_sel, B, ref->k,
                                                             ipl_for(ref->k), NS, ct, B, tab);
      }
      WCX_HIP(hipGetLastError());
    } else if (rankmed) {
      ChrTable tab;
      tab.n_chr = (int)ref->chr_cum.size();
      for (int c = 0; c < 32; ++c) tab.cum[c] = c < tab.n_chr ? ref->chr_cum[c] : B;
      WcxChrCum cc;
      cc.n_chr = tab.n_chr;
      for (int c = 0; c < 32; ++c) cc.cum[c] = tab.cum[c];
      const dim3 grid((unsigned)((Bp + 3) / 4 < 16384 ? (Bp + 3) / 4 : 16384), (unsigned)(NS / 64));
      k_normalize_mask_incr<<<grid, NT, 0, ctx->stream>>>(xT, const_cast<double *>(cin), ref->d_idx, ref->d_sel, B,
                                                          ref->k, ipl_for(ref->k), NS, ct, B, tab, stS1, stS2, stN,
                                                          stM1, nullptr, nullptr, zT, nT);
      WCX_HIP(hipGetLastError());
      rc = wcx_norm_rank_mark_launch(rkv, cin, B, NS, n_samples, ctx->stream);
      if (rc) return rc;
      rc = wcx_norm_median_rank_launch(rkv, ref->d_idx, ref->d_sel, xT, B, ref->k, ipl_for(ref->k), NS, n_samples,
                                       ct, cc, rT, lrT, ctx->stream);
      if (rc) return rc;
      const dim3 gt((unsigned)((Bp + 31) / 32), (unsigned)((n_samples + 31) / 32));
      k_from_sample_minor<<<gt, 256, 0, ctx->stream>>>(zT, ct, Bp, NS, n_samples, d_out_z);
      k_from_sample_minor<<<gt, 256, 0, ctx->stream>>>(nT, ct, Bp, NS, n_samples, d_out_n);
      k_from_sample_minor<<<gt, 256, 0, ctx->stream>>>(rT, ct, Bp, NS, n_samples, d_out_r);
      k_from_sample_minor<<<gt, 256, 0, ctx->stream>>>(lrT, ct, Bp, NS, n_samples, lr);
      WCX_HIP(hipGetLastError());
    } else if (tiled)
      rc = launch_pass_tile<TILE>(ctx, ref, d_x, cin, cout, n_samples, NS, ct, pass == 2, d_out_z,
                                  d_out_r, d_out_n, lr);
    else
      rc = launch_pass(ctx, ref, d_x, cin, cout, n_samples, ct, pass == 2, d_out_z, d_out_r, d_out_n,
                       lr);
    if (rc) return rc;
  }
  if (n_samples == 1) {
    rc = launch_nanmedian_wide(ctx, lr, d_out_z, Bp, d_out_mlr, d_out_mz);
    if (rc) return rc;
  } else {
    k_nanmedian<<<dim3((unsigned)n_samples, 2), NTM, 0, ctx->stream>>>(lr, d_out_z, Bp, Bp,
                                                                        d_out_mlr, d_out_mz);
  }
  WCX_HIP(hipGetLastError());
  return wcx_timer_end(ctx, "normalize");
}

int wcx_ref_wrap_rows_dev(wcx_ctx *ctx, const int32_t *d_idx, const double *d_dist, int64_t B, int k,
                          const int64_t *chr_cum, int n_chr, int64_t row0, int64_t nrows,
                          wcx_ref **out) {
  WCX_ARG(row0 >= 0 && nrows >= 0 && row0 + nrows <= B, "bad row range");
  int rc = wcx_ref_wrap_dev(ctx, d_idx, d_dist, B, k, chr_cum, n_chr, out);
  if (rc) return rc;
  (*out)->row0 = row0;
  (*out)->nrows = nrows;
  return WCX_OK;
}

int wcx_cutoff_moments_dev(wcx_ctx *ctx, const wcx_ref *ref, double cutoff, double mean, int phase,
                           double *out2) {
  WCX_ARG(ctx && ref && out2 && (phase == 0 || phase == 1), "bad argument");
  WCX_HIP(hipSetDevice(ctx->device));
  const int64_t n = ref->nrows * (int64_t)ref->k;
  const int nparts = 2048;
  void *scr = nullptr;
  int rc = wcx_scratch(ctx, (size_t)(2 * nparts + 16) * 8, &scr);
  if (rc) return rc;
  double *state = reinterpret_cast<double *>(scr);
  double *ps = state + 16, *pc = ps + nparts;
  const double init[3] = {cutoff, mean, 0.0};
  rc = wcx_upload_small(ctx, state, init, sizeof(init));
  if (rc) return rc;
  if (n > 0) k_cut_partial<<<nparts, NT, 0, ctx->stream>>>(ref->d_dist, n, state, phase, ps, pc);
  else WCX_HIP(hipMemsetAsync(ps, 0, (size_t)2 * nparts * 8, ctx->stream));
  k_sum_parts<<<1, NT, 0, ctx->stream>>>(ps, pc, nparts, state + 8);
  WCX_HIP(hipGetLastError());
  WCX_HIP(hipMemcpyAsync(out2, state + 8, 16, hipMemcpyDeviceToHost, ctx->stream));
  WCX_HIP(hipStreamSynchronize(ctx->stream));
  return WCX_OK;
}

int wcx_predict_pass_dev(wcx_ctx *ctx, wcx_ref *ref, const double *d_x, const double *d_copy_in,
                         double *d_copy_out, double cutoff, int64_t ct, int build_mask, int last,
                         double *d_z, double *d_r, double *d_n, double *d_lr) {
  WCX_ARG(ctx && ref && d_x && d_copy_in && d_copy_out && d_z && d_r && d_n && d_lr, "NULL argument");
  WCX_HIP(hipSetDevice(ctx->device));
  if (ref->k > 64 * 32) {
    wcx_set_error("refsize %d too large for the normalise kernel (max 2048)", ref->k);
    return WCX_ERR_UNSUPPORTED;
  }
  int rc = WCX_OK;
  if (build_mask) {
    rc = wcx_timer_begin(ctx, "normalize");
    if (rc) return rc;
    rc = launch_select_mask(ctx, ref, cutoff, ct);
    if (rc) return rc;
  }
  WCX_ARG(ref->d_sel != nullptr || ref->nrows == 0, "first pass must build the selection mask");
  rc = launch_pass(ctx, ref, d_x, d_copy_in, d_copy_out, 1, ct, last != 0, d_z, d_r, d_n, d_lr);
  if (rc) return rc;
  if (last) rc = wcx_timer_end(ctx, "normalize");
  return rc;
}

int wcx_nanmedian2_dev(wcx_ctx *ctx, const double *d_a0, const double *d_a1, int64_t n,
                       double *d_out0, double *d_out1) {
  WCX_ARG(ctx && d_a0 && d_a1 && d_out0 && d_out1 && n >= 0, "bad argument");
  WCX_HIP(hipSetDevice(ctx->device));
  return launch_nanmedian_wide(ctx, d_a0, d_a1, n, d_out0, d_out1);
}

int wcx_predict_normalize(wcx_ctx *ctx, const wcx_ref *ref, const double *x, int n_samples,
                          double cutoff, int64_t ct, int cp, double *out_z, double *out_r,
                          double *out_n, double *out_mlr, double *out_mz) {
  WCX_ARG(ctx && ref && x && out_z && out_r && out_n && out_mlr && out_mz, "NULL argument");
  WCX_ARG(n_samples > 0, "n_samples must be positive");
  WCX_HIP(hipSetDevice(ctx->device));
  const int64_t B = ref->B, Bp = B - ct;
  WCX_ARG(Bp >= 0, "ct beyond the last row");
  const size_t xb = (size_t)n_samples * B * 8, ob = (size_t)n_samples * (Bp > 0 ? Bp : 0) * 8;
  void *buf = nullptr;
  int rc = wcx_scratch2(ctx, xb + 3 * ob + (size_t)n_samples * 16 + 64, &buf);
  if (rc) return rc;
  double *dx = reinterpret_cast<double *>(buf);
  double *dz = dx + (size_t)n_samples * B;
  double *dr = dz + ob / 8, *dn = dr + ob / 8;
  double *dmlr = dn + ob / 8, *dmz = dmlr + n_samples;
  WCX_HIP(hipMemcpyAsync(dx, x, xb, hipMemcpyHostToDevice, ctx->stream));
  rc = wcx_predict_normalize_dev(ctx, ref, dx, n_samples, cutoff, ct, cp, dz, dr, dn, dmlr, dmz);
  if (rc) return rc;
  if (ob) {
    WCX_HIP(hipMemcpyAsync(out_z, dz, ob, hipMemcpyDeviceToHost, ctx->stream));
    WCX_HIP(hipMemcpyAsync(out_r, dr, ob, hipMemcpyDeviceToHost, ctx->stream));
    WCX_HIP(hipMemcpyAsync(out_n, dn, ob, hipMemcpyDeviceToHost, ctx->stream));
    WCX_HIP(hipMemcpyAsync(out_mlr, dmlr, (size_t)n_samples * 8, hipMemcpyDeviceToHost, ctx->stream));
    WCX_HIP(hipMemcpyAsync(out_mz, dmz, (size_t)n_samples * 8, hipMemcpyDeviceToHost, ctx->stream));
  }
  WCX_HIP(hipStreamSynchronize(ctx->stream));
  return WCX_OK;
}

}
```

wisecondorx_amd/csrc/wcx_common.h:

```cpp
#pragma once
#include <hip/hip_runtime.h>

#include <cstdarg>
#include <cstdint>
#include <cstdio>
#include <cstring>
#include <map>
#include <string>
#include <vector>

#include "../../include/wcx.h"

void wcx_set_error(const char *fmt, ...);

#define WCX_HIP(call)                                                                  \
  do {                                                                                 \
    hipError_t e__ = (call);                                                           \
    if (e__ != hipSuccess) {                                                           \
      wcx_set_error("%s:%d: %s -> %s", __FILE__, __LINE__, #call, hipGetErrorString(e__)); \
      return WCX_ERR_HIP;                                                              \
    }                                                                                  \
  } while (0)

#define WCX_ARG(cond, msg)                          \
  do {                                              \
    if (!(cond)) {                                  \
      wcx_set_error("bad argument: %s", msg);       \
      return WCX_ERR_ARG;                           \
    }                                               \
  } while (0)

struct KernelTimer {
  hipEvent_t start = nullptr, stop = nullptr;
  bool used = false;
};

struct wcx_ctx {
  int device = 0;
  hipStream_t stream = nullptr;
  bool own_stream = false;
  std::map<std::string, KernelTimer> timers;
  std::string timer_tag;
  int debug_flags = 0;
  int64_t topk_stats[4] = {0, 0, 0, 0};
  unsigned long long *d_stats = nullptr;
  void *d_small = nullptr;
  void *scratch = nullptr;
  size_t scratch_bytes = 0;
  std::vector<double> cbs_trace;
  long long cbs_pairs_listed = 0, cbs_pairs_total = 0;
  long long cbs_shortcuts = 0;
  void *host_scratch = nullptr;
  size_t host_scratch_bytes = 0;
  void *host_scratch2 = nullptr;
  size_t host_scratch2_bytes = 0;
  void *scratch2 = nullptr;
  size_t scratch2_bytes = 0;
  double *d_nullm = nullptr;
  int64_t nullm_bins = 0;
  int nullm_m = 0;
  int32_t *d_nullsrc = nullptr;
  int64_t nullsrc_bins = 0;
  unsigned long long nullsrc_hash = 0;
  std::vector<unsigned char> nullsrc_mask;
  hipStream_t aux_stream = nullptr;
  hipEvent_t ev_main = nullptr, ev_rank = nullptr;
  hipStream_t sweep_stream = nullptr;
  hipEvent_t ev_sweep0 = nullptr, ev_sweep1 = nullptr;
  hipEvent_t ev_after_sweep = nullptr;
  hipStream_t copy_stream = nullptr;
  hipEvent_t ev_cbs_fill = nullptr, ev_cbs_xw = nullptr;
  void *d_rank = nullptr;
  size_t rank_bytes = 0;
  const double *rank_X = nullptr;
  int64_t rank_B = 0;
  std::vector<int32_t> rank_ids;
  struct SelSlot { void *p; size_t bytes; bool used; };
  std::vector<SelSlot> sel_pool;
  bool rank_pending = false;
  void *d_pca = nullptr;
  size_t pca_bytes = 0;
  int64_t pca_B = 0;
  int pca_S = 0;
  std::vector<std::vector<unsigned char>> stage;
  void *sym_state = nullptr;
};
void wcx_sym_state_free(wcx_ctx *ctx);
int wcx_sym_shard_sweep(wcx_ctx *ctx, const double *dXs, int64_t B, int S, const int64_t *chr_cum, int n_chr,
                        int k, int part, int n_parts, const int64_t *row_bounds, int64_t *counts_out);
int wcx_sym_shard_records(wcx_ctx *ctx, void *d_send);
int wcx_sym_shard_finish(wcx_ctx *ctx, const void *d_recv, int64_t n_recv, int32_t *d_out_idx,
                         double *d_out_dist);

struct wcx_ref {
  const int32_t *d_idx = nullptr;
  const double *d_dist = nullptr;
  bool owned = false;
  int64_t B = 0;
  int k = 0;
  int64_t row0 = 0, nrows = 0;
  unsigned long long *d_sel = nullptr;
  size_t sel_bytes = 0;
  std::vector<int64_t> chr_cum;
  int64_t *d_chr_cum = nullptr;
};

int wcx_scratch(wcx_ctx *ctx, size_t bytes, void **out);
int wcx_scratch2(wcx_ctx *ctx, size_t bytes, void **out);
int wcx_upload_small(wcx_ctx *ctx, void *dst_dev, const void *src_host, size_t bytes);
int wcx_transpose_launch(wcx_ctx *ctx, const double *src, int64_t rows, int64_t cols, double *dst);
int wcx_timer_begin(wcx_ctx *ctx, const char *name);
int wcx_timer_end(wcx_ctx *ctx, const char *name);

struct TopkBlock {
  int64_t row0;
  int32_t nrows;
  int32_t pad;
  int64_t cs, ce;
};

int wcx_topk_exact_launch(wcx_ctx *ctx, const double *dXs, int64_t B, int S,
                          const std::vector<TopkBlock> &blocks, int64_t row_begin,
                          int64_t n_rows, int k, int32_t *d_out_idx, double *d_out_dist);
constexpr int WCX_REDO_GRID = 128;
constexpr int WCX_REDO_FAST = 128;
size_t wcx_topk_redo_scratch_bytes(int k, int64_t B);
int wcx_host_scratch(wcx_ctx *ctx, size_t bytes, void **out);
int wcx_aux_kick(wcx_ctx *ctx);
struct WcxRankView { unsigned int *Rg; const double *V; int n_sg; };
struct WcxChrCum { int n_chr; int64_t cum[32]; };
size_t wcx_rank_bytes(int64_t B, int n);
int wcx_rank_rows_launch(const double *d_x, int64_t B, int n, char *base, hipStream_t st, WcxRankView *out);
int wcx_norm_rank_mark_launch(const WcxRankView &rk, const double *copyT, int64_t B, int NS, int n_samples,
                              hipStream_t st);
int wcx_norm_median_rank_launch(const WcxRankView &rk, const int32_t *d_idx, const unsigned long long *d_sel,
                                const double *xT, int64_t B, int k, int ipl, int NS, int n_samples, int64_t ct,
                                const WcxChrCum &chr, double *rT, double *lrT, hipStream_t st);
bool wcx_null_ratios_direct_pays(int64_t B, int64_t n_rows);
void wcx_aux_cancel_if_few_rows(wcx_ctx *ctx, int64_t B, int64_t n_rows);
int wcx_topk_exact_redo_launch(wcx_ctx *ctx, const double *dXs, int64_t B, int S,
                               const TopkBlock *d_blocks, const unsigned int *d_count,
                               const TopkBlock *d_tiles, const unsigned int *d_ntiles,
                               const int32_t *d_rowlist, void *scratch, int64_t row_begin, int k,
                               int32_t *d_out_idx, double *d_out_dist);
bool wcx_screen_supported(int64_t B, int S, int k);
int wcx_topk_screen_launch(wcx_ctx *ctx, const double *dXs, int64_t B, int S,
                           const int64_t *chr_cum, int n_chr,
                           const std::vector<TopkBlock> &exact_blocks, int64_t row_begin,
                           int64_t n_rows, int k, int32_t *d_out_idx, double *d_out_dist);
int wcx_fill_dummy_rows(wcx_ctx *ctx, int32_t *d_idx, double *d_dist, int64_t row_lo,
                        int64_t row_hi, int k);
```

Before: 631.0 billion.

## Batch scattered memsets into one fill kernel and fuse reduction finalize kernels

Adds a multi-buffer fill kernel driven by a table of up to 24 entries, and replaces many separate hipMemsetAsync calls across the screen, CBS, rank and predict paths with a single launch per site. To make the fills happen up front, it gives the second histogram pass its own buffer instead of reusing the first. It also folds the cutoff finalize step into the next partial-sum kernel and the nanmedian decide step into the next histogram kernel, using ping-pong state buffers and a larger small-scratch area. The aim is fewer launches and stream operations; the cost is redundant per-block reductions and more intricate buffer rotation.

```diff
diff --git a/wisecondorx_amd/csrc/api.hip b/wisecondorx_amd/csrc/api.hip
--- a/wisecondorx_amd/csrc/api.hip
+++ b/wisecondorx_amd/csrc/api.hip
@@ -67,6 +67,39 @@
     ctx->scratch2_bytes = bytes;
   }
   *out = ctx->scratch2;
+  return WCX_OK;
+}
+
+namespace {
+__global__ __launch_bounds__(256) void k_fill_many(const WcxFillTable t) {
+  const WcxFillTable::Entry &en = t.e[blockIdx.y];
+  unsigned char *p = reinterpret_cast<unsigned char *>(en.p);
+  const size_t bytes = en.bytes;
+  size_t head = (16 - (reinterpret_cast<uintptr_t>(p) & 15)) & 15;
+  if (head > bytes) head = bytes;
+  const size_t body = (bytes - head) / 16, tail = bytes - head - body * 16;
+  const unsigned int w = en.byte * 0x01010101u;
+  const uint4 v = make_uint4(w, w, w, w);
+  uint4 *q = reinterpret_cast<uint4 *>(p + head);
+  const size_t gid = (size_t)blockIdx.x * 256 + threadIdx.x;
+  for (size_t i = gid; i < body; i += (size_t)gridDim.x * 256) q[i] = v;
+  if (gid < head) p[gid] = (unsigned char)en.byte;
+  if (gid < tail) p[head + body * 16 + gid] = (unsigned char)en.byte;
+}
+}
+
+int wcx_fill_many(const WcxFillTable &t, hipStream_t st) {
+  if (t.overflow) {
+    wcx_set_error("fill table: more than %d entries", WcxFillTable::CAP);
+    return WCX_ERR_ARG;
+  }
+  if (t.n == 0) return WCX_OK;
+  size_t most = 0;
+  for (int i = 0; i < t.n; ++i) most = t.e[i].bytes > most ? t.e[i].bytes : most;
+  size_t gx = (most + 256 * 64 - 1) / (256 * 64);
+  if (gx > 256) gx = 256;
+  k_fill_many<<<dim3((unsigned)gx, (unsigned)t.n), 256, 0, st>>>(t);
+  WCX_HIP(hipGetLastError());
   return WCX_OK;
 }
 
@@ -204,7 +237,7 @@
   }
   WCX_HIP(hipMalloc(reinterpret_cast<void **>(&ctx->d_stats), 256));
   WCX_HIP(hipMemsetAsync(ctx->d_stats, 0, 256, ctx->stream));
-  WCX_HIP(hipMalloc(&ctx->d_small, 8192));
+  WCX_HIP(hipMalloc(&ctx->d_small, 16384));
   *out = ctx;
   return WCX_OK;
 }
diff --git a/wisecondorx_amd/csrc/cbs_seg.hip b/wisecondorx_amd/csrc/cbs_seg.hip
--- a/wisecondorx_amd/csrc/cbs_seg.hip
+++ b/wisecondorx_amd/csrc/cbs_seg.hip
@@ -1389,8 +1389,15 @@
       }
       WCX_ARG(qoff <= qtab_floats, "internal: arc-weight table overflow");
       WCX_HIP(hipMemcpyAsync(djobs, jobs.data(), jobs.size() * sizeof(PermJob), hipMemcpyHostToDevice, st));
-      WCX_HIP(hipMemsetAsync(dbits, 0, jobs.size() * (size_t)nw * 4, st));
-      WCX_HIP(hipMemsetAsync(dcnt, 0, jobs.size() * (size_t)NCH * 4, st));
+      bool nflag_clear = true;
+      {
+        WcxFillTable ft;
+        ft.add(dbits, jobs.size() * (size_t)nw * 4, 0);
+        ft.add(dcnt, jobs.size() * (size_t)NCH * 4, 0);
+        ft.add(dnflag, 4, 0);
+        const int frc = wcx_fill_many(ft, st);
+        if (frc) return frc;
+      }
       {
         int hyb_max_n = 0;
         for (const PermJob &jb : jobs) if (jb.mode == 0) hyb_max_n = std::max(hyb_max_n, jb.n);
@@ -1427,7 +1434,8 @@
             WCX_HIP(hipMemcpyAsync(dj, sj.data() + j0, nj * sizeof(PermJob), hipMemcpyHostToDevice, st));
             joff += nj;
             if (kind <= 1) {
-              WCX_HIP(hipMemsetAsync(dnflag, 0, 4, st));
+              if (!nflag_clear) WCX_HIP(hipMemsetAsync(dnflag, 0, 4, st));
+              nflag_clear = false;
               if (kind == 1)
                 k_cbs_perm_hyb<true><<<dim3((unsigned)std::min(BIG_GRID, p1 - p0), (unsigned)nj), NTP, 0, st>>>(
                     dy, drw, dj, p0, p1, npad_max + 64, dq, dbig, dbits, dcnt, nw, dflags, dnflag);
@@ -1534,9 +1542,14 @@
       unsigned int *dcount = dL + ns;
       if (pruned) {
         WCX_HIP(hipMemcpyAsync(dboff, boff.data(), (size_t)(ns + 1) * 4, hipMemcpyHostToDevice, st));
-        WCX_HIP(hipMemsetAsync(dL, 0, (size_t)(ns + 1) * 4, st));
-        WCX_HIP(hipMemsetAsync(dbbits, 0, (size_t)ns * 8, st));
-        WCX_HIP(hipMemsetAsync(dbij, 0xff, (size_t)ns * 8, st));
+        {
+          WcxFillTable ft;
+          ft.add(dL, (size_t)(ns + 1) * 4, 0);
+          ft.add(dbbits, (size_t)ns * 8, 0);
+          ft.add(dbij, (size_t)ns * 8, 0xff);
+          const int frc = wcx_fill_many(ft, st);
+          if (frc) return frc;
+        }
         std::vector<int> bseg((size_t)total_blocks);
         for (int a = 0; a < ns; ++a) std::fill(bseg.begin() + boff[a], bseg.begin() + boff[a + 1], a);
         WCX_HIP(hipMemcpyAsync(dbseg, bseg.data(), (size_t)total_blocks * 4, hipMemcpyHostToDevice, st));
diff --git a/wisecondorx_amd/csrc/newref_topk_screen.hip b/wisecondorx_amd/csrc/newref_topk_screen.hip
--- a/wisecondorx_amd/csrc/newref_topk_screen.hip
+++ b/wisecondorx_amd/csrc/newref_topk_screen.hip
@@ -1101,13 +1101,15 @@
 
 static float screen_gamma(int NK) { return (float)(16 * NK + 12) * 1.1920929e-7f; }
 
+static void col_stats_clears(WcxFillTable &ft, double *cmean, int S) {
+  ft.add(cmean + S, (size_t)S * 8, 0xff);
+  ft.add(cmean + 2 * (size_t)S, (size_t)S * 8, 0);
+}
 static int col_stats(const double *dXs, int64_t B, int S, double *cmean, ScreenGlobals *glob,
                      const int64_t *chr_cum, int n_chr, ChrTab &tab, hipStream_t st) {
   unsigned long long *cmin = reinterpret_cast<unsigned long long *>(cmean + S);
   unsigned long long *cmax = cmin + S;
   double *psum = cmean + 3 * S, *pcnt = psum + (size_t)S * CSPLIT;
-  WCX_HIP(hipMemsetAsync(cmin, 0xff, (size_t)S * 8, st));
-  WCX_HIP(hipMemsetAsync(cmax, 0, (size_t)S * 8, st));
   k_col_sum<<<dim3((unsigned)S, CSPLIT), NT, 0, st>>>(dXs, B, psum, pcnt, cmin, cmax);
   k_col_stats<<<(unsigned)((S + 63) / 64), 64, 0, st>>>(S, psum, pcnt, cmin, cmax, cmean, glob);
   tab.n_chr = n_chr;
@@ -1248,7 +1250,7 @@
   double *cmean;
   half8 *F, *Fs;
   RowInfo *info, *infs;
-  int *perm2, *rowpos, *rowpos2, *hubhist, *rchr, *rkey, *cellcnt, *cursor, *d_seq, *dett;
+  int *perm2, *rowpos, *rowpos2, *hubhist, *rchr, *rkey, *cellcnt, *cellcnt2, *cursor, *d_seq, *dett;
   unsigned int *rbits, *rfine, *gmask, *tinfo, *pool_head;
   float *tmin, *Dest, *g_state;
   unsigned char *tchr;
@@ -1276,6 +1278,7 @@
     take(rchr, (size_t)B * 4);
     take(rkey, (size_t)B * 4);
     take(cellcnt, (size_t)2 * NCELL * 4);
+    take(cellcnt2, (size_t)2 * NCELL * 4);
     take(cursor, (size_t)2 * NCELL * 4);
     take(gmask, (size_t)(P_s / CT) * 4);
     take(tinfo, (size_t)NTb * 64 * 4);
@@ -1311,13 +1314,29 @@
   const unsigned int *gate2 = use_hub ? d_gate : nullptr;
 
   hipStream_t st = ctx->stream;
-  WCX_HIP(hipMemsetAsync(glob, 0, sizeof(ScreenGlobals), st));
-  WCX_HIP(hipMemsetAsync(t.cnt, 0, (size_t)n_rows * 4, st));
-  WCX_HIP(hipMemsetAsync(t.flags, 0, (size_t)n_rows * 4, st));
-  WCX_HIP(hipMemsetAsync(t.searched, 1, (size_t)n_rows, st));
-  WCX_HIP(hipMemsetAsync(pool_head, 0, 256, st));
-  WCX_HIP(hipMemsetAsync(t.d_nredo, 0, 512, st));
-  WCX_HIP(hipMemsetAsync(ctx->d_stats, 0, 256, st));
+  const int NQb = (int)(NTb / 4);
+  {
+    WcxFillTable ft;
+    ft.add(glob, sizeof(ScreenGlobals), 0);
+    ft.add(t.cnt, (size_t)n_rows * 4, 0);
+    ft.add(t.flags, (size_t)n_rows * 4, 0);
+    ft.add(t.searched, (size_t)n_rows, 1);
+    ft.add(pool_head, 256, 0);
+    ft.add(t.d_nredo, 512, 0);
+    ft.add(ctx->d_stats, 256, 0);
+    col_stats_clears(ft, cmean, S);
+    if (use_hub) ft.add(hubhist, (size_t)HUB_BINS * 4, 0);
+    ft.add(cellcnt, (size_t)2 * NCELL * 4, 0);
+    ft.add(cursor, (size_t)2 * NCELL * 4, 0);
+    ft.add(t.perm, (size_t)PB * 4, 0xff);
+    ft.add(tchr, (size_t)NTb, 0xff);
+    if (sh) ft.add(dett, (size_t)DET_KEYS * n_wg_det * 4, 0);
+    ft.add(d_seq, (size_t)(NQb + 1) * 4, 0);
+    ft.add(cellcnt2, (size_t)2 * NCELL * 4, 0);
+    ft.add(perm2, (size_t)Bpad2 * 4, 0xff);
+    rc = wcx_fill_many(ft, st);
+    if (rc) return rc;
+  }
   rc = wcx_upload_small(ctx, d_blocks, blocks.data(), blocks.size() * sizeof(ScreenBlock));
   if (rc) return rc;
 
@@ -1330,7 +1349,6 @@
   const ChrTab &tab = t.tab;
   const unsigned gb = (unsigned)((B + NT - 1) / NT);
   if (use_hub) {
-    WCX_HIP(hipMemsetAsync(hubhist, 0, (size_t)HUB_BINS * 4, st));
     k_transpose_norm<<<(unsigned)((B + 31) / 32), 256, 0, st>>>(dXs, B, S, Sp, t.Xr, cmean, tab, glob, rbits, rchr,
                                                                 rfine, hubhist);
     k_hub_cut<<<1, 1024, 0, st>>>(hubhist, (int)p.hub_rows, glob);
@@ -1338,15 +1356,10 @@
     k_transpose_norm<<<(unsigned)((B + 31) / 32), 256, 0, st>>>(dXs, B, S, Sp, t.Xr, cmean, tab, glob, rbits, rchr,
                                                                 nullptr, nullptr);
   }
-  WCX_HIP(hipMemsetAsync(cellcnt, 0, (size_t)2 * NCELL * 4, st));
-  WCX_HIP(hipMemsetAsync(cursor, 0, (size_t)2 * NCELL * 4, st));
-  WCX_HIP(hipMemsetAsync(t.perm, 0xff, (size_t)PB * 4, st));
-  WCX_HIP(hipMemsetAsync(tchr, 0xff, (size_t)NTb, st));
   static_assert(2 * SYM_NCELL * SYM_NSUB <= 2 * NCELL, "cell tables");
   k_sym_hist<<<gb, NT, 0, st>>>(rbits, rchr, B, glob, rkey, cellcnt, 1, use_hub ? rfine : nullptr);
   k_sym_scan<<<1, SYM_NCELL, 0, st>>>(cellcnt, cursor, tchr, glob);
   if (sh) {
-    WCX_HIP(hipMemsetAsync(dett, 0, (size_t)DET_KEYS * n_wg_det * 4, st));
     k_det_local<<<gb, NT, 0, st>>>(rkey, B, n_wg_det, dett, detl);
     k_det_scan<<<(unsigned)((DET_KEYS * 64 + NT - 1) / NT), NT, 0, st>>>(dett, n_wg_det, cursor);
     k_det_place<<<gb, NT, 0, st>>>(rkey, B, n_wg_det, dett, detl, t.perm, rowpos);
@@ -1365,7 +1378,6 @@
   const int glist_cap = (int)((Cz / CTG + 64 + 3) / 4 * 4);
   const size_t lds_sym = (size_t)cfg.ring * (size_t)(CTG * NK * 64) * 16 + (size_t)cfg.ring * CTG * 256 +
                          (size_t)glist_cap * 4 + (size_t)4 * 64 * 16;
-  const int NQb = (int)(NTb / 4);
   SymArgs sa;
   int sym_grid = 0;
   {
@@ -1394,7 +1406,6 @@
     }
     rc = wcx_upload_small(ctx, d_desc, descs.data(), descs.size() * sizeof(SymDesc));
     if (rc) return rc;
-    WCX_HIP(hipMemsetAsync(d_seq, 0, (size_t)(NQb + 1) * 4, st));
     sa.F = F; sa.tinfo = tinfo; sa.tmin = tmin; sa.tchr = tchr; sa.glob = glob; sa.sl = t.sl; sa.cnt = t.cnt;
     sa.flags = t.flags; sa.stats = ctx->d_stats; sa.dbg = ctx->debug_flags; sa.cap2 = cap2;
     sa.pool = pool; sa.pool_head = pool_head; sa.pool_ovf = pool_head + 1; sa.pool_cap = pool_cap;
@@ -1471,10 +1482,8 @@
   }
 
   {
-    WCX_HIP(hipMemsetAsync(cellcnt, 0, (size_t)2 * NCELL * 4, st));
-    WCX_HIP(hipMemsetAsync(perm2, 0xff, (size_t)Bpad2 * 4, st));
-    k_row_hist<<<gb, NT, 0, st>>>(rbits, rchr, B, SF, 0, glob, rkey, cellcnt, gate2);
-    k_scan_cells<<<1, 1024, 0, st>>>(cellcnt, cursor, (int)(P_s - n_s), gate2);
+    k_row_hist<<<gb, NT, 0, st>>>(rbits, rchr, B, SF, 0, glob, rkey, cellcnt2, gate2);
+    k_scan_cells<<<1, 1024, 0, st>>>(cellcnt2, cursor, (int)(P_s - n_s), gate2);
     k_scatter<<<gb, NT, 0, st>>>(rkey, B, cursor, perm2, rowpos2, gate2);
     k_group_mask<<<(unsigned)((P_s / CT + NT - 1) / NT), NT, 0, st>>>(perm2, rchr, P_s / CT, gmask, gate2);
     screen_prep(NK, t.Xr, P_s, S, Sp, cmean, perm2, glob, Fs, infs, gate2, st);
@@ -1575,12 +1584,21 @@
   layout(reinterpret_cast<uintptr_t>(scr));
   t.dXs = dXs; t.B = B; t.S = S; t.Sp = Sp; t.k = k; t.cap2 = CAP; t.glob = glob;
   hipStream_t st = ctx->stream;
-  WCX_HIP(hipMemsetAsync(glob, 0, sizeof(ScreenGlobals), st));
-  WCX_HIP(hipMemsetAsync(t.cnt, 0, (size_t)n_seg * n_rows * 4, st));
-  WCX_HIP(hipMemsetAsync(t.flags, 0, (size_t)n_seg * n_rows * 4, st));
-  WCX_HIP(hipMemsetAsync(t.searched, 0, (size_t)n_rows, st));
-  WCX_HIP(hipMemsetAsync(t.d_nredo, 0, 512, st));
-  WCX_HIP(hipMemsetAsync(ctx->d_stats, 0, 256, st));
+  {
+    WcxFillTable ft;
+    ft.add(glob, sizeof(ScreenGlobals), 0);
+    ft.add(t.cnt, (size_t)n_seg * n_rows * 4, 0);
+    ft.add(t.flags, (size_t)n_seg * n_rows * 4, 0);
+    ft.add(t.searched, (size_t)n_rows, 0);
+    ft.add(t.d_nredo, 512, 0);
+    ft.add(ctx->d_stats, 256, 0);
+    col_stats_clears(ft, cmean, S);
+    ft.add(cellcnt, (size_t)2 * NCELL * 4, 0);
+    ft.add(t.perm, (size_t)Bpad * 4, 0xff);
+    if (use_hub1) ft.add(hubhist, (size_t)HUB_BINS * 4, 0);
+    rc = wcx_fill_many(ft, st);
+    if (rc) return rc;
+  }
   rc = wcx_upload_small(ctx, d_blocks, blocks.data(), blocks.size() * sizeof(ScreenBlock));
   if (rc) return rc;
   k_mark<<<(unsigned)blocks.size(), 256, 0, st>>>(t.searched, d_blocks, row_begin);
@@ -1595,10 +1613,7 @@
   {
     const unsigned gb = (unsigned)((B + NT - 1) / NT);
     const unsigned gtn = (unsigned)((B + 31) / 32);
-    WCX_HIP(hipMemsetAsync(cellcnt, 0, (size_t)2 * NCELL * 4, st));
-    WCX_HIP(hipMemsetAsync(t.perm, 0xff, (size_t)Bpad * 4, st));
     if (use_hub1) {
-      WCX_HIP(hipMemsetAsync(hubhist, 0, (size_t)HUB_BINS * 4, st));
       k_transpose_norm<<<gtn, 256, 0, st>>>(dXs, B, S, Sp, t.Xr, cmean, tab, glob, rbits, rchr, rfine, hubhist);
       k_hub_cut<<<1, 1024, 0, st>>>(hubhist, (int)p.hub_rows, glob);
       k_row_hist<<<gb, NT, 0, st>>>(rbits, rchr, B, 0, 0, glob, rkey, cellcnt, nullptr, rfine);
diff --git a/wisecondorx_amd/csrc/null_ratios.hip b/wisecondorx_amd/csrc/null_ratios.hip
--- a/wisecondorx_amd/csrc/null_ratios.hip
+++ b/wisecondorx_amd/csrc/null_ratios.hip
@@ -778,8 +778,11 @@
   unsigned int *R = reinterpret_cast<unsigned int *>(base + L.o_r);
   unsigned int *Rg = reinterpret_cast<unsigned int *>(base + L.o_rg);
   double *V = reinterpret_cast<double *>(base + L.o_v);
-  WCX_HIP(hipMemsetAsync(d_nan, 0, (size_t)n_ids * 4, st));
-  WCX_HIP(hipMemsetAsync(cnt, 0, (size_t)n_ids * RK_NB * 4, st));
+  WcxFillTable ft;
+  ft.add(d_nan, (size_t)n_ids * 4, 0);
+  ft.add(cnt, (size_t)n_ids * RK_NB * 4, 0);
+  const int rc = wcx_fill_many(ft, st);
+  if (rc) return rc;
   const unsigned gb = (unsigned)((B + RK_TILE - 1) / RK_TILE);
   k_rank_splitters<<<(unsigned)n_ids, 1024, 0, st>>>(dXs, B, d_sids, spk, spb);
   k_rank_bucket<<<dim3((unsigned)n_ids, gb), NT, 0, st>>>(dXs, B, d_sids, spk, spb, bkt, cnt, d_nan);
diff --git a/wisecondorx_amd/csrc/predict.hip b/wisecondorx_amd/csrc/predict.hip
--- a/wisecondorx_amd/csrc/predict.hip
+++ b/wisecondorx_amd/csrc/predict.hip
@@ -5,13 +5,50 @@
 
 constexpr int NT = 256;
 constexpr double Z_MASK = 2.3263478740408408;
+
+__device__ __forceinline__ void cut_sum_parts(const double *__restrict__ part_sum,
+                                              const double *__restrict__ part_cnt, int nparts,
+                                              double *sh_s, double *sh_c, double &ts, double &tc) {
+  double s = 0.0, c = 0.0;
+  for (int i = threadIdx.x; i < nparts; i += NT) { s += part_sum[i]; c += part_cnt[i]; }
+  s = wcx::wave_sum(s);
+  c = wcx::wave_sum(c);
+  if ((threadIdx.x & 63) == 0) { sh_s[threadIdx.x >> 6] = s; sh_c[threadIdx.x >> 6] = c; }
+  __syncthreads();
+  ts = 0.0; tc = 0.0;
+  if (threadIdx.x == 0)
+    for (int w = 0; w < NT / 64; ++w) { ts += sh_s[w]; tc += sh_c[w]; }
+}
+
+__device__ __forceinline__ void cut_advance(double *st, int phase, double ts, double tc) {
+  if (phase == 0) {
+    st[2] = tc;
+    st[1] = ts / tc;
+  } else {
+    const double sd = sqrt(ts / st[2]);
+    st[0] = st[1] + 3.0 * sd;
+  }
+}
 
 __global__ __launch_bounds__(NT) void k_cut_partial(const double *__restrict__ d, int64_t n,
                                                     const double *__restrict__ state, int phase,
                                                     double *__restrict__ part_sum,
-                                                    double *__restrict__ part_cnt) {
-  const double cutoff = state[0];
-  const double mean = state[1];
+                                                    double *__restrict__ part_cnt,
+                                                    const double *__restrict__ prev_sum,
+                                                    const double *__restrict__ prev_cnt, int prev_nparts,
+                                                    double *__restrict__ state_out) {
+  __shared__ double sh_s[NT / 64], sh_c[NT / 64];
+  __shared__ double sh_st[3];
+  double ts = 0.0, tc = 0.0;
+  if (prev_nparts > 0) cut_sum_parts(prev_sum, prev_cnt, prev_nparts, sh_s, sh_c, ts, tc);
+  if (threadIdx.x == 0) {
+    sh_st[0] = state[0]; sh_st[1] = state[1]; sh_st[2] = state[2];
+    if (prev_nparts > 0) cut_advance(sh_st, 1 - phase, ts, tc);
+    if (blockIdx.x == 0 && state_out) { state_out[0] = sh_st[0]; state_out[1] = sh_st[1]; state_out[2] = sh_st[2]; }
+  }
+  __syncthreads();
+  const double cutoff = sh_st[0];
+  const double mean = sh_st[1];
   double s = 0.0, c = 0.0;
   const int64_t stride = (int64_t)gridDim.x * NT * 2;
   for (int64_t i = ((int64_t)blockIdx.x * NT + threadIdx.x) * 2; i < n; i += stride) {
@@ -21,7 +58,6 @@
     if (v.x < cutoff) { if (phase == 0) { s += v.x; c += 1.0; } else { double e = v.x - mean; s += e * e; } }
     if (v.y < cutoff) { if (phase == 0) { s += v.y; c += 1.0; } else { double e = v.y - mean; s += e * e; } }
   }
-  __shared__ double sh_s[NT / 64], sh_c[NT / 64];
   s = wcx::wave_sum(s);
   c = wcx::wave_sum(c);
   if ((threadIdx.x & 63) == 0) { sh_s[threadIdx.x >> 6] = s; sh_c[threadIdx.x >> 6] = c; }
@@ -37,39 +73,19 @@
 __global__ __launch_bounds__(NT) void k_cut_final(double *__restrict__ state, int phase,
                                                   const double *__restrict__ part_sum,
                                                   const double *__restrict__ part_cnt, int nparts) {
-  double s = 0.0, c = 0.0;
-  for (int i = threadIdx.x; i < nparts; i += NT) { s += part_sum[i]; c += part_cnt[i]; }
   __shared__ double sh_s[NT / 64], sh_c[NT / 64];
-  s = wcx::wave_sum(s);
-  c = wcx::wave_sum(c);
-  if ((threadIdx.x & 63) == 0) { sh_s[threadIdx.x >> 6] = s; sh_c[threadIdx.x >> 6] = c; }
-  __syncthreads();
-  if (threadIdx.x == 0) {
-    double ts = 0.0, tc = 0.0;
-    for (int w = 0; w < NT / 64; ++w) { ts += sh_s[w]; tc += sh_c[w]; }
-    if (phase == 0) {
-      state[2] = tc;
-      state[1] = ts / tc;
-    } else {
-      const double sd = sqrt(ts / state[2]);
-      state[0] = state[1] + 3.0 * sd;
-    }
-  }
+  double ts, tc;
+  cut_sum_parts(part_sum, part_cnt, nparts, sh_s, sh_c, ts, tc);
+  if (threadIdx.x == 0) cut_advance(state, phase, ts, tc);
 }
 
 __global__ __launch_bounds__(NT) void k_sum_parts(const double *__restrict__ part_sum,
                                                   const double *__restrict__ part_cnt, int nparts,
                                                   double *__restrict__ out) {
-  double s = 0.0, c = 0.0;
-  for (int i = threadIdx.x; i < nparts; i += NT) { s += part_sum[i]; c += part_cnt[i]; }
   __shared__ double sh_s[NT / 64], sh_c[NT / 64];
-  s = wcx::wave_sum(s);
-  c = wcx::wave_sum(c);
-  if ((threadIdx.x & 63) == 0) { sh_s[threadIdx.x >> 6] = s; sh_c[threadIdx.x >> 6] = c; }
-  __syncthreads();
+  double ts, tc;
+  cut_sum_parts(part_sum, part_cnt, nparts, sh_s, sh_c, ts, tc);
   if (threadIdx.x == 0) {
-    double ts = 0.0, tc = 0.0;
-    for (int w = 0; w < NT / 64; ++w) { ts += sh_s[w]; tc += sh_c[w]; }
     out[0] = ts;
     out[1] = tc;
   }
@@ -619,44 +635,74 @@
   }
 }
 
-struct NmState { unsigned long long prefix[2]; long long rank[2]; unsigned long long himask; long long nvalid; };
-
-__global__ __launch_bounds__(256) void k_nm_count(const double *__restrict__ a0,
-                                                  const double *__restrict__ a1, int64_t n,
-                                                  NmState *__restrict__ st) {
-  const double *a = blockIdx.y ? a1 : a0;
-  long long loc = 0;
-  for (int64_t i = (int64_t)blockIdx.x * 256 + threadIdx.x; i < n; i += (int64_t)gridDim.x * 256) {
-    const double x = a[i];
-    loc += (x == x);
-  }
-  loc = (long long)wcx::wave_sum_i((int)loc);
-  if ((threadIdx.x & 63) == 0 && loc) atomicAdd((unsigned long long *)&st[blockIdx.y].nvalid, (unsigned long long)loc);
-}
-
-__global__ void k_nm_init(NmState *__restrict__ st, unsigned int *__restrict__ hist) {
-  const int a = blockIdx.x;
-  if (threadIdx.x == 0) {
-    const long long nv = st[a].nvalid;
-    st[a].rank[0] = nv > 0 ? (nv - 1) / 2 : 0;
-    st[a].rank[1] = nv / 2;
-    st[a].prefix[0] = st[a].prefix[1] = 0;
-    st[a].himask = 0;
-  }
-  for (int i = threadIdx.x; i < 512; i += blockDim.x) hist[a * 512 + i] = 0;
+struct NmState { unsigned long long prefix[2]; long long rank[2]; long long nvalid; };
+
+__device__ __forceinline__ NmState nm_decide(const NmState *__restrict__ prev,
+                                             const unsigned int *__restrict__ h, int shift, bool first) {
+  __shared__ long long wtot[2][4];
+  __shared__ int sh_dg[2];
+  __shared__ long long sh_excl[2];
+  const int d = threadIdx.x, lane = d & 63, w = d >> 6;
+  NmState s;
+  if (first) { s.prefix[0] = s.prefix[1] = 0; s.rank[0] = s.rank[1] = 0; s.nvalid = 0; }
+  else s = *prev;
+  const bool two = s.prefix[1] != s.prefix[0];
+  const long long m0 = h[d], m1 = two ? (long long)h[256 + d] : m0;
+  long long c0 = m0, c1 = m1;
+  for (int off = 1; off < 64; off <<= 1) {
+    const long long u0 = __shfl_up(c0, off), u1 = __shfl_up(c1, off);
+    if (lane >= off) { c0 += u0; c1 += u1; }
+  }
+  if (lane == 63) { wtot[0][w] = c0; wtot[1][w] = c1; }
+  if (d < 2) sh_dg[d] = -1;
+  __syncthreads();
+  long long tot0 = 0;
+  for (int v = 0; v < 4; ++v) {
+    if (v < w) { c0 += wtot[0][v]; c1 += wtot[1][v]; }
+    tot0 += wtot[0][v];
+  }
+  if (first) {
+    s.nvalid = tot0;
+    s.rank[0] = tot0 > 0 ? (tot0 - 1) / 2 : 0;
+    s.rank[1] = tot0 / 2;
+  }
+  if (s.rank[0] >= c0 - m0 && s.rank[0] < c0) { sh_dg[0] = d; sh_excl[0] = c0 - m0; }
+  if (s.rank[1] >= c1 - m1 && s.rank[1] < c1) { sh_dg[1] = d; sh_excl[1] = c1 - m1; }
+  __syncthreads();
+  for (int t = 0; t < 2; ++t)
+    if (sh_dg[t] >= 0) {
+      s.rank[t] -= sh_excl[t];
+      s.prefix[t] |= ((unsigned long long)sh_dg[t]) << shift;
+    }
+  return s;
 }
 
 __global__ __launch_bounds__(256) void k_nm_hist(const double *__restrict__ a0,
                                                  const double *__restrict__ a1, int64_t n, int shift,
-                                                 const NmState *__restrict__ st,
-                                                 unsigned int *__restrict__ hist) {
+                                                 const NmState *__restrict__ st_prev,
+                                                 const unsigned int *__restrict__ h_prev,
+                                                 NmState *__restrict__ st_out,
+                                                 unsigned int *__restrict__ hist,
+                                                 unsigned int *__restrict__ h_next) {
   const int arr = blockIdx.y;
   const double *a = arr ? a1 : a0;
   __shared__ unsigned int lh[2][256];
   lh[0][threadIdx.x] = 0;
   lh[1][threadIdx.x] = 0;
-  __syncthreads();
-  const unsigned long long p0 = st[arr].prefix[0], p1 = st[arr].prefix[1], himask = st[arr].himask;
+  unsigned long long p0 = 0, p1 = 0, himask = 0;
+  if (shift < 56) {
+    const NmState s = nm_decide(st_prev + arr, h_prev + arr * 512, shift + 8, shift == 48);
+    p0 = s.prefix[0];
+    p1 = s.prefix[1];
+    himask = ~0ull << (shift + 8);
+    if (blockIdx.x == 0 && threadIdx.x == 0) st_out[arr] = s;
+  } else {
+    __syncthreads();
+  }
+  if (blockIdx.x == 0) {
+    h_next[arr * 512 + threadIdx.x] = 0;
+    h_next[arr * 512 + 256 + threadIdx.x] = 0;
+  }
   const bool two = p1 != p0;
   for (int64_t i = (int64_t)blockIdx.x * 256 + threadIdx.x; i < n; i += (int64_t)gridDim.x * 256) {
     const double x = a[i];
@@ -672,41 +718,15 @@
   if (two && lh[1][threadIdx.x]) atomicAdd(&hist[arr * 512 + 256 + threadIdx.x], lh[1][threadIdx.x]);
 }
 
-__global__ __launch_bounds__(512) void k_nm_decide(NmState *__restrict__ st,
-                                                    unsigned int *__restrict__ hist, int shift,
-                                                    double *__restrict__ out0,
-                                                    double *__restrict__ out1) {
+__global__ __launch_bounds__(256) void k_nm_final(const NmState *__restrict__ st_prev,
+                                                  const unsigned int *__restrict__ h_prev,
+                                                  double *__restrict__ out0, double *__restrict__ out1) {
   const int a = blockIdx.x;
-  const int t = threadIdx.x >> 8, d = threadIdx.x & 255;
-  const bool two = st[a].prefix[1] != st[a].prefix[0];
-  __shared__ long long cum[2][256];
-  const long long rk = st[a].rank[t];
-  const long long mine = hist[a * 512 + ((t == 1 && two) ? 256 : 0) + d];
-  cum[t][d] = mine;
-  __syncthreads();
-  for (int off = 1; off < 256; off <<= 1) {
-    const long long v = d >= off ? cum[t][d - off] : 0;
-    __syncthreads();
-    cum[t][d] += v;
-    __syncthreads();
-  }
-  const long long incl = cum[t][d], excl = incl - mine;
-  __syncthreads();
-  if (rk >= excl && rk < incl) {
-    st[a].rank[t] = rk - excl;
-    st[a].prefix[t] |= ((unsigned long long)d) << shift;
-  }
-  hist[a * 512 + threadIdx.x] = 0;
-  __syncthreads();
+  const NmState s = nm_decide(st_prev + a, h_prev + a * 512, 0, false);
   if (threadIdx.x == 0) {
-    __threadfence();
-    st[a].himask |= 255ull << shift;
-    if (shift == 0) {
-      double *out = a ? out1 : out0;
-      const long long nv = st[a].nvalid;
-      const double lo = key_f64(st[a].prefix[0]), hi = key_f64(st[a].prefix[1]);
-      out[0] = nv == 0 ? __builtin_nan("") : ((nv & 1) ? lo : (lo + hi) / 2.0);
-    }
+    double *out = a ? out1 : out0;
+    const double lo = key_f64(s.prefix[0]), hi = key_f64(s.prefix[1]);
+    out[0] = s.nvalid == 0 ? __builtin_nan("") : ((s.nvalid & 1) ? lo : (lo + hi) / 2.0);
   }
 }
 
@@ -720,18 +740,17 @@
 
 static int launch_nanmedian_wide(wcx_ctx *ctx, const double *a0, const double *a1, int64_t n,
                                  double *out0, double *out1) {
-  void *scr = ctx->d_small;
+  char *scr = reinterpret_cast<char *>(ctx->d_small);
   NmState *st = reinterpret_cast<NmState *>(scr);
-  unsigned int *hist = reinterpret_cast<unsigned int *>(reinterpret_cast<char *>(scr) + 256);
+  unsigned int *hist = reinterpret_cast<unsigned int *>(scr + 256);
   hipStream_t s = ctx->stream;
-  WCX_HIP(hipMemsetAsync(st, 0, 2 * sizeof(NmState), s));
+  WCX_HIP(hipMemsetAsync(hist, 0, 1024 * 4, s));
   const unsigned g = (unsigned)std::min<int64_t>(256, (n + 255) / 256 > 0 ? (n + 255) / 256 : 1);
-  k_nm_count<<<dim3(g, 2), 256, 0, s>>>(a0, a1, n, st);
-  k_nm_init<<<2, 256, 0, s>>>(st, hist);
-  for (int shift = 56; shift >= 0; shift -= 8) {
-    k_nm_hist<<<dim3(g, 2), 256, 0, s>>>(a0, a1, n, shift, st, hist);
-    k_nm_decide<<<2, 512, 0, s>>>(st, hist, shift, out0, out1);
-  }
+  int j = 0;
+  for (int shift = 56; shift >= 0; shift -= 8, ++j)
+    k_nm_hist<<<dim3(g, 2), 256, 0, s>>>(a0, a1, n, shift, st + 2 * ((j + 1) & 1), hist + 1024 * ((j + 2) % 3),
+                                         st + 2 * (j & 1), hist + 1024 * (j % 3), hist + 1024 * ((j + 1) % 3));
+  k_nm_final<<<2, 256, 0, s>>>(st + 2 * ((j + 1) & 1), hist + 1024 * ((j + 2) % 3), out0, out1);
   WCX_HIP(hipGetLastError());
   return WCX_OK;
 }
@@ -1004,21 +1023,22 @@
   const int64_t n = ref->nrows * (int64_t)ref->k;
   const int nparts = 2048;
   void *scr = nullptr;
-  int rc = wcx_scratch(ctx, (size_t)(2 * nparts + 8) * 8, &scr);
+  int rc = wcx_scratch(ctx, (size_t)(4 * nparts + 8) * 8, &scr);
   if (rc) return rc;
   double *state = reinterpret_cast<double *>(scr);
-  double *ps = state + 8, *pc = ps + nparts;
+  double *parts[2] = {state + 8, state + 8 + 2 * nparts};
   const double init[3] = {HUGE_VAL, 0.0, 0.0};
   rc = wcx_upload_small(ctx, state, init, sizeof(init));
   if (rc) return rc;
   rc = wcx_timer_begin(ctx, "cutoff");
   if (rc) return rc;
-  for (int rep = 0; rep < repeats; ++rep) {
-    for (int phase = 0; phase < 2; ++phase) {
-      k_cut_partial<<<nparts, NT, 0, ctx->stream>>>(ref->d_dist, n, state, phase, ps, pc);
-      k_cut_final<<<1, NT, 0, ctx->stream>>>(state, phase, ps, pc, nparts);
-    }
-  }
+  for (int j = 0; j < 2 * repeats; ++j) {
+    double *ps = parts[j & 1], *pps = parts[(j + 1) & 1];
+    k_cut_partial<<<nparts, NT, 0, ctx->stream>>>(ref->d_dist, n, state + 4 * (j & 1), j & 1, ps, ps + nparts,
+                                                  pps, pps + nparts, j ? nparts : 0,
+                                                  state + 4 * ((j + 1) & 1));
+  }
+  if (repeats > 0) k_cut_final<<<1, NT, 0, ctx->stream>>>(state, 1, parts[1], parts[1] + nparts, nparts);
   WCX_HIP(hipGetLastError());
   rc = wcx_timer_end(ctx, "cutoff");
   if (rc) return rc;
@@ -1105,9 +1125,14 @@
   double *d_st = d_wfin + (BA + BG);
   int *d_fb = reinterpret_cast<int *>(d_st + 8);
   hipStream_t st = ctx->stream;
-  WCX_HIP(hipMemsetAsync(d_out_r, 0, (size_t)n_samples * n_bins * 8, st));
-  WCX_HIP(hipMemsetAsync(d_out_z, 0, (size_t)n_samples * n_bins * 8, st));
-  WCX_HIP(hipMemsetAsync(d_out_w, 0, (size_t)n_samples * n_bins * 8, st));
+  {
+    WcxFillTable ft;
+    ft.add(d_out_r, (size_t)n_samples * n_bins * 8, 0);
+    ft.add(d_out_z, (size_t)n_samples * n_bins * 8, 0);
+    ft.add(d_out_w, (size_t)n_samples * n_bins * 8, 0);
+    rc = wcx_fill_many(ft, st);
+    if (rc) return rc;
+  }
   k_wstats<<<1, 1024, 0, st>>>(d_wA, BA, d_st);
   if (BG) k_wstats<<<1, 1024, 0, st>>>(d_wG, BG, d_st + 3);
   k_wmerge<<<1, 1024, 0, st>>>(d_wA, BA, d_wG, BG, d_st, d_st + 3, d_wfin, d_fb);
@@ -1433,7 +1458,8 @@
   const double init[3] = {cutoff, mean, 0.0};
   rc = wcx_upload_small(ctx, state, init, sizeof(init));
   if (rc) return rc;
-  if (n > 0) k_cut_partial<<<nparts, NT, 0, ctx->stream>>>(ref->d_dist, n, state, phase, ps, pc);
+  if (n > 0) k_cut_partial<<<nparts, NT, 0, ctx->stream>>>(ref->d_dist, n, state, phase, ps, pc, nullptr,
+                                                           nullptr, 0, nullptr);
   else WCX_HIP(hipMemsetAsync(ps, 0, (size_t)2 * nparts * 8, ctx->stream));
   k_sum_parts<<<1, NT, 0, ctx->stream>>>(ps, pc, nparts, state + 8);
   WCX_HIP(hipGetLastError());
diff --git a/wisecondorx_amd/csrc/wcx_common.h b/wisecondorx_amd/csrc/wcx_common.h
--- a/wisecondorx_amd/csrc/wcx_common.h
+++ b/wisecondorx_amd/csrc/wcx_common.h
@@ -108,6 +108,19 @@
 int wcx_scratch(wcx_ctx *ctx, size_t bytes, void **out);
 int wcx_scratch2(wcx_ctx *ctx, size_t bytes, void **out);
 int wcx_upload_small(wcx_ctx *ctx, void *dst_dev, const void *src_host, size_t bytes);
+struct WcxFillTable {
+  static constexpr int CAP = 24;
+  struct Entry { void *p; size_t bytes; unsigned int byte; unsigned int pad; } e[CAP];
+  int n = 0;
+  bool overflow = false;
+  void add(void *p, size_t bytes, int byte) {
+    if (!bytes) return;
+    if (n == CAP) { overflow = true; return; }
+    e[n].p = p; e[n].bytes = bytes; e[n].byte = (unsigned int)byte & 255u; e[n].pad = 0;
+    ++n;
+  }
+};
+int wcx_fill_many(const WcxFillTable &t, hipStream_t st);
 int wcx_transpose_launch(wcx_ctx *ctx, const double *src, int64_t rows, int64_t cols, double *dst);
 int wcx_timer_begin(wcx_ctx *ctx, const char *name);
 int wcx_timer_end(wcx_ctx *ctx, const char *name);
```

Result: no change. 634.4 billion (median of 6 runs) (+0.5%).
